# PhucNguyenAH/tacotron2_subword

Measured on AMD Instinct MI355X. Metric: mel_frames_per_sec_train, higher is better.
Workload: dtype bf16; 1 GPU; BERT_Tacotron2 default hparams (SMA), full training iteration fwd+loss+bwd+clip+Adam, B=64/GPU, 100 phones, 60 sub-word tokens, 400 frames, 80-mel; global_batch=64, frames_per_item=400, parallelism=dp1, torch_ops=loss reductions, cat/transpose copies, persistent_chains=True, recurrent_steps_bf16=True

## Files before the change

include/t2amd.h:

```cpp
#ifndef T2AMD_H
#define T2AMD_H
#include <stddef.h>
#include <stdint.h>

#ifdef __cplusplus
extern "C" {
#endif

#define T2_ATTN_SMA 0
#define T2_ATTN_LSA 1
#define T2_ATTN_DCA 4
#define T2_ATTN_GMM 3
#define T2_ATTN_FWD2 2

enum {
    T2_SITE_PRENET1 = 1, T2_SITE_PRENET2 = 2, T2_SITE_PRENET1_SUB = 3, T2_SITE_PRENET2_SUB = 4,
    T2_SITE_ATT_H = 5, T2_SITE_ATT_C = 6, T2_SITE_ATT_H_SUB = 7, T2_SITE_ATT_C_SUB = 8,
    T2_SITE_DEC_H = 9, T2_SITE_DEC_C = 10, T2_SITE_NOISE = 11, T2_SITE_NOISE_SUB = 12,
    T2_SITE_ENC0 = 16,
    T2_SITE_ENCSUB0 = 20,
    T2_SITE_POSTNET0 = 24
};

const char* t2_last_error(void);
#define T2_ABI_VERSION 4
int t2_version(void);
int t2_chain_status(uint32_t* out_host );
int t2_chain_status_clear(void);
int t2_debug_report_abort(uint32_t code, void* stream);
int t2_debug_occupy(int workgroups, int milliseconds, void* stream);
int t2_chain_claimed(void);
int t2_set_precision(int mode);
int t2_get_precision(void);
int t2_gemm_counts(uint64_t* out_host , int reset);
int t2_set_gemm_split_min_mflop(int mflop);
int t2_set_overlap(int on);
int t2_set_chain(int on);
int t2_get_chain(void);
int t2_set_chain_bwd(int on);
int t2_set_gemm_staging(int on);
int t2_side_join(void* stream);

typedef struct t2_dims {
    int n_mel;
    int prenet_dim;
    int enc_dim;
    int att_rnn_dim;
    int dec_rnn_dim;
    int att_dim;
    int loc_filters;
    int loc_kernel;
    int attention_kind;
    float p_att_dropout, p_dec_dropout, p_prenet_dropout;
    int n_streams;
    float score_mask_value, score_mask_value_sub;
    int score_mask_given;
} t2_dims;

typedef struct t2_attention_weights {
    const float* wq;
    const float* wm;
    const float* v;
    const float* loc_conv;
    const float* loc_dense;
    const float* mlp_b1;
    const float* mlp_w2;
    const float* mlp_b2;
    const float* dca_T;
    const float* dca_bT;
    const float* dca_P;
} t2_attention_weights;
typedef struct t2_lstm_weights { const float *w_ih, *w_hh, *b_ih, *b_hh; } t2_lstm_weights;
typedef struct t2_decoder_weights {
    const float *prenet_w1, *prenet_w2;
    const float *prenet_sub_w1, *prenet_sub_w2;
    t2_lstm_weights att, att_sub;
    t2_attention_weights attn, attn_sub;
    t2_lstm_weights dec;
    const float *proj_w, *proj_b;
    const float *gate_w, *gate_b;
} t2_decoder_weights;

typedef struct t2_decoder_layout {
    size_t total_floats;
    size_t x, p1, p2, p1s, p2s;
    size_t pm, pms;
    size_t prea, preas;
    size_t ga, gas;
    size_t cna, cnas, ca, cas;
    size_t din;
    size_t psel, psels;
    size_t wcum, wcums;
    size_t pred, gd, cnd, cd;
    size_t dout;
    size_t qs, qss;
    size_t qpart;
    size_t w1t;
    size_t w16a, w16as, w16d, wt16a, wt16as, wt16d, din16, dh16;
    size_t gemm_ws; size_t gemm_ws_floats;
    size_t chain; size_t chain_floats;
    size_t usave, usaves;
    size_t locsave, locsaves;
} t2_decoder_layout;

int t2_decoder_layout_query(const t2_dims* dims, int B, int T, int Tin, int Tsub, t2_decoder_layout* out);

typedef struct t2_decoder_fwd_args {
    int B, T, Tin, Tsub;
    const float* memory;
    const float* memory_sub;
    const int32_t* mem_lengths;
    const int32_t* sub_lengths;
    const float* mels;
    float* mel_out;
    float* gate_out;
    float* align;
    float* align_sub;
    float* ws;
    int training;
    int prenet_dropout;
    uint64_t seed;
    int phase;
} t2_decoder_fwd_args;
int t2_decoder_forward(const t2_dims* dims, const t2_decoder_weights* w, const t2_decoder_fwd_args* a, void* stream);

typedef struct t2_lstm_grads { float *w_ih, *w_hh, *b_ih, *b_hh; } t2_lstm_grads;
typedef struct t2_attention_grads { float *wq, *wm, *v, *loc_conv, *loc_dense, *mlp_b1, *mlp_w2, *mlp_b2, *dca_T, *dca_bT, *dca_P; } t2_attention_grads;
typedef struct t2_decoder_grads {
    float *prenet_w1, *prenet_w2, *prenet_sub_w1, *prenet_sub_w2;
    t2_lstm_grads att, att_sub;
    t2_attention_grads attn, attn_sub;
    t2_lstm_grads dec;
    float *proj_w, *proj_b, *gate_w, *gate_b;
} t2_decoder_grads;
typedef struct t2_decoder_bwd_layout {
    size_t total_floats;
    size_t ddout, ddin, dgd, dga, dgas, dctx, dctxs, dq, dqs, dv, dvs, dpm, dpms, carry, carrys;
    size_t carryc, carrycs, dlconv, dlconvs, dldense, dldenses;
    size_t dcd, dca, dcas, partd, parta, dp2, dp2s, dp1, dmel_t, dgate_t, dg16a, dg16d, colsum_ws, gemm_ws, gemm_ws_floats;
    size_t chain, chain_floats;
} t2_decoder_bwd_layout;
int t2_decoder_bwd_layout_query(const t2_dims* dims, int B, int T, int Tin, int Tsub, t2_decoder_bwd_layout* out);
typedef struct t2_decoder_bwd_args {
    int B, T, Tin, Tsub;
    const float* memory; const float* memory_sub;
    const float* align; const float* align_sub;
    const float* d_mel;
    const float* d_gate;
    const float* d_align;
    const float* d_align_sub;
    float* d_memory;
    float* d_memory_sub;
    const float* ws;
    float* bws;
    int training; int prenet_dropout; uint64_t seed;
    int defer_weight_grads;
} t2_decoder_bwd_args;
int t2_decoder_backward(const t2_dims* dims, const t2_decoder_weights* w, const t2_decoder_grads* g,
                        const t2_decoder_bwd_args* a, void* stream);

typedef struct t2_decoder_infer_args {
    int B, Tin, Tsub, max_steps, poll_every;
    float gate_threshold;
    const float* memory; const float* memory_sub;
    const int32_t* mem_lengths; const int32_t* sub_lengths;
    float* mel_out;
    float* gate_out;
    float* align;
    float* align_sub;
    int32_t* stop_index;
    int32_t* done_count;
    float* ws;
    int prenet_dropout; uint64_t seed;
    int* steps_run_host;
} t2_decoder_infer_args;
int t2_decoder_infer(const t2_dims* dims, const t2_decoder_weights* w, const t2_decoder_infer_args* a, void* stream);

int t2_finalize_bct(const float* in_btc, float* out_bct, int B, int T, int C, const int32_t* lengths, float fill, void* stream);
int t2_mask_bt(float* x, int B, int T, const int32_t* lengths, float fill, void* stream);

typedef struct t2_conv_bn_args {
    int B, T, Cin, Cout, K;
    const float* x;
    const float* w; const float* bias;
    const float* gamma; const float* beta;
    float* run_mean; float* run_var;
    int training; float eps; int act; float drop_p; uint64_t seed; uint32_t site;
    const float* residual;
    float* z; float* mean; float* invstd; float* var;
    float* y;
    float* ws; size_t ws_floats;
} t2_conv_bn_args;
int t2_conv_bn_forward(const t2_conv_bn_args* a, void* stream);
typedef struct t2_conv_bn_bwd_args {
    int B, T, Cin, Cout, K;
    const float* x; const float* w; const float* gamma; const float* beta;
    const float* z; const float* mean; const float* invstd;
    int training; float eps; int act; float drop_p; uint64_t seed; uint32_t site;
    const float* dy;
    float* dw; float* dbias; float* dgamma; float* dbeta;
    float* dx; int dx_accumulate;
    float* ws; size_t ws_floats;
} t2_conv_bn_bwd_args;
int t2_conv_bn_backward(const t2_conv_bn_bwd_args* a, void* stream);

int t2_embedding_forward(const int64_t* ids, const float* table, float* out, int rows, int dim, void* stream);
int t2_embedding_backward(const int64_t* ids, const float* dout, float* dtable, int rows, int dim, int vocab, void* stream);

typedef struct t2_lstm_seq_args {
    int nstreams, B, T, H;
    const float* pre[4];
    const float* w_hh[4];
    int reverse[4];
    const int32_t* lengths;
    float* h[4]; long ldh;
    float* c[4];
    float* gates[4];
    float* ws; size_t ws_floats;
} t2_lstm_seq_args;
size_t t2_lstm_seq_chain_ws_floats(int nstreams, int B, int H, int backward);
int t2_lstm_seq_forward(const t2_lstm_seq_args* a, void* stream);
typedef struct t2_lstm_seq_bwd_args {
    int nstreams, B, T, H;
    const float* w_hh[4]; int reverse[4];
    const float* h[4]; long ldh; const float* c[4]; const float* gates[4];
    const float* dh[4]; long lddh;
    float* dpre[4];
    float* dw_hh[4];
    float* ws; size_t ws_floats;
} t2_lstm_seq_bwd_args;
int t2_lstm_seq_backward(const t2_lstm_seq_bwd_args* a, void* stream);

typedef struct t2_gemm_args {
    const float* A; const float* B; float* C; int M, N, K;
    long sam, sak, sbn, sbk, ldc; int batch; long bsA, bsB, bsC;
    float alpha, beta; const float* bias; int act; int crow_mod; long crow_mul;
    float* ws; size_t ws_bytes; int splitk;
} t2_gemm_args;
int t2_gemm_ex(const t2_gemm_args* a, void* stream);
int t2_prof_gemm(const t2_gemm_args* a, int reps, float* ms_total, float* ms_kernel, void* stream);
enum { T2_GEMM_F32_64 = 0, T2_GEMM_F32_128, T2_GEMM_BF16CONV, T2_GEMM_SRC128, T2_GEMM_SRC256, T2_GEMM_SRC256KM };
enum { T2_GEMM_OPERAND_FP32 = 0, T2_GEMM_OPERAND_STAGED, T2_GEMM_OPERAND_CALLER };
typedef struct t2_gemm_plan_opts {
    int conv_a, conv_b, conv_T, conv_C, fp32_only;
    int a16, b16; long lda16, ldb16; int a16_kmajor, b16_kmajor, split16;
} t2_gemm_plan_opts;
typedef struct t2_gemm_plan_info {
    int kernel; const char* name;
    int split;
    int splitk, kchunks;
    int a_src, b_src;
    size_t stage_bytes_a, stage_bytes_b;
} t2_gemm_plan_info;
int t2_gemm_plan(const t2_gemm_args* a, const t2_gemm_plan_opts* opts, t2_gemm_plan_info* out);
int t2_colsum(const float* x, long ld, int M, int N, float* out, float* scratch, void* stream);
int t2_mask_btc(float* x, int B, int T, int C, const int32_t* lengths, float fill, void* stream);

typedef struct t2_adam_tensor { float* p; const float* g; float* m; float* v; long numel; int first_chunk; int pad_; } t2_adam_tensor;
int t2_adam_chunks(long numel);
int t2_adam_step(const t2_adam_tensor* table, int n_tensors, int n_chunks, float* partial, float* norm_out, float max_norm,
                 float lr, float beta1, float beta2, float eps, float weight_decay, int step, void* stream);
int t2_adam_norm(const t2_adam_tensor* table, int n_tensors, int n_chunks, float* partial, float* norm_out, float max_norm, void* stream);

int t2_prof_enable(int max_launches);
int t2_prof_collect(int n_kinds, double* total_ms_host, int* launches_host);

int t2_gemm(const float* A, const float* B, float* C, int M, int N, int K,
            long sam, long sak, long sbn, long sbk, long ldc,
            const float* bias, int act, float alpha, float beta,
            float* ws, size_t ws_bytes, int splitk, void* stream);
int t2_rng_keep_mask(uint64_t seed, uint32_t site, uint32_t n, float p, uint8_t* out, void* stream);
int t2_rng_normal(uint64_t seed, uint32_t site, uint32_t n, float* out, void* stream);

#ifdef __cplusplus
}
#endif
#endif
```

tacotron2_subword_amd/_lib.py:

```python
from __future__ import annotations

import ctypes as C
import os

import torch

_HERE = os.path.dirname(os.path.abspath(__file__))
LIB_PATH = os.environ.get("T2AMD_LIB") or os.path.join(_HERE, "libt2amd.so")

ATTN_SMA, ATTN_LSA, ATTN_FWD2, ATTN_GMM, ATTN_DCA = 0, 1, 2, 3, 4

SITE = dict(PRENET1=1, PRENET2=2, PRENET1_SUB=3, PRENET2_SUB=4, ATT_H=5, ATT_C=6, ATT_H_SUB=7, ATT_C_SUB=8,
            DEC_H=9, DEC_C=10, NOISE=11, NOISE_SUB=12, ENC0=16, ENCSUB0=20, POSTNET0=24)

_fp = C.POINTER(C.c_float)
_ip = C.POINTER(C.c_int32)


class Dims(C.Structure):
    _fields_ = [("n_mel", C.c_int), ("prenet_dim", C.c_int), ("enc_dim", C.c_int), ("att_rnn_dim", C.c_int),
                ("dec_rnn_dim", C.c_int), ("att_dim", C.c_int), ("loc_filters", C.c_int), ("loc_kernel", C.c_int),
                ("attention_kind", C.c_int), ("p_att_dropout", C.c_float), ("p_dec_dropout", C.c_float),
                ("p_prenet_dropout", C.c_float), ("n_streams", C.c_int),
                ("score_mask_value", C.c_float), ("score_mask_value_sub", C.c_float), ("score_mask_given", C.c_int)]


class AttentionWeights(C.Structure):
    _fields_ = [("wq", C.c_void_p), ("wm", C.c_void_p), ("v", C.c_void_p), ("loc_conv", C.c_void_p), ("loc_dense", C.c_void_p),
                ("mlp_b1", C.c_void_p), ("mlp_w2", C.c_void_p), ("mlp_b2", C.c_void_p),
                ("dca_T", C.c_void_p), ("dca_bT", C.c_void_p), ("dca_P", C.c_void_p)]


class LstmWeights(C.Structure):
    _fields_ = [("w_ih", C.c_void_p), ("w_hh", C.c_void_p), ("b_ih", C.c_void_p), ("b_hh", C.c_void_p)]


class DecoderWeights(C.Structure):
    _fields_ = [("prenet_w1", C.c_void_p), ("prenet_w2", C.c_void_p), ("prenet_sub_w1", C.c_void_p), ("prenet_sub_w2", C.c_void_p),
                ("att", LstmWeights), ("att_sub", LstmWeights), ("attn", AttentionWeights), ("attn_sub", AttentionWeights),
                ("dec", LstmWeights), ("proj_w", C.c_void_p), ("proj_b", C.c_void_p), ("gate_w", C.c_void_p), ("gate_b", C.c_void_p)]


_LAYOUT_FIELDS = ["total_floats", "x", "p1", "p2", "p1s", "p2s", "pm", "pms", "prea", "preas", "ga", "gas",
                  "cna", "cnas", "ca", "cas", "din", "psel", "psels", "wcum", "wcums", "pred", "gd", "cnd", "cd",
                  "dout", "qs", "qss", "qpart", "w1t", "w16a", "w16as", "w16d", "wt16a", "wt16as", "wt16d", "din16", "dh16",
                  "gemm_ws", "gemm_ws_floats", "chain", "chain_floats", "usave", "usaves", "locsave", "locsaves"]


class DecoderLayout(C.Structure):
    _fields_ = [(n, C.c_size_t) for n in _LAYOUT_FIELDS]


class DecoderFwdArgs(C.Structure):
    _fields_ = [("B", C.c_int), ("T", C.c_int), ("Tin", C.c_int), ("Tsub", C.c_int),
                ("memory", C.c_void_p), ("memory_sub", C.c_void_p), ("mem_lengths", C.c_void_p), ("sub_lengths", C.c_void_p),
                ("mels", C.c_void_p), ("mel_out", C.c_void_p), ("gate_out", C.c_void_p), ("align", C.c_void_p),
                ("align_sub", C.c_void_p), ("ws", C.c_void_p), ("training", C.c_int), ("prenet_dropout", C.c_int),
                ("seed", C.c_uint64), ("phase", C.c_int)]


class DecoderInferArgs(C.Structure):
    _fields_ = [("B", C.c_int), ("Tin", C.c_int), ("Tsub", C.c_int), ("max_steps", C.c_int), ("poll_every", C.c_int),
                ("gate_threshold", C.c_float),
                ("memory", C.c_void_p), ("memory_sub", C.c_void_p), ("mem_lengths", C.c_void_p), ("sub_lengths", C.c_void_p),
                ("mel_out", C.c_void_p), ("gate_out", C.c_void_p), ("align", C.c_void_p), ("align_sub", C.c_void_p),
                ("stop_index", C.c_void_p), ("done_count", C.c_void_p), ("ws", C.c_void_p),
                ("prenet_dropout", C.c_int), ("seed", C.c_uint64), ("steps_run_host", C.POINTER(C.c_int))]


class LstmGrads(C.Structure):
    _fields_ = LstmWeights._fields_


class AttentionGrads(C.Structure):
    _fields_ = AttentionWeights._fields_


class DecoderGrads(C.Structure):
    _fields_ = [("prenet_w1", C.c_void_p), ("prenet_w2", C.c_void_p), ("prenet_sub_w1", C.c_void_p), ("prenet_sub_w2", C.c_void_p),
                ("att", LstmGrads), ("att_sub", LstmGrads), ("attn", AttentionGrads), ("attn_sub", AttentionGrads),
                ("dec", LstmGrads), ("proj_w", C.c_void_p), ("proj_b", C.c_void_p), ("gate_w", C.c_void_p), ("gate_b", C.c_void_p)]


_BWD_LAYOUT_FIELDS = ["total_floats", "ddout", "ddin", "dgd", "dga", "dgas", "dctx", "dctxs", "dq", "dqs", "dv", "dvs",
                      "dpm", "dpms", "carry", "carrys", "carryc", "carrycs", "dlconv", "dlconvs", "dldense", "dldenses", "dcd", "dca", "dcas", "partd", "parta", "dp2", "dp2s", "dp1",
                      "dmel_t", "dgate_t", "dg16a", "dg16d", "colsum_ws", "gemm_ws", "gemm_ws_floats", "chain", "chain_floats"]


class DecoderBwdLayout(C.Structure):
    _fields_ = [(n, C.c_size_t) for n in _BWD_LAYOUT_FIELDS]


class DecoderBwdArgs(C.Structure):
    _fields_ = [("B", C.c_int), ("T", C.c_int), ("Tin", C.c_int), ("Tsub", C.c_int),
                ("memory", C.c_void_p), ("memory_sub", C.c_void_p), ("align", C.c_void_p), ("align_sub", C.c_void_p),
                ("d_mel", C.c_void_p), ("d_gate", C.c_void_p), ("d_align", C.c_void_p), ("d_align_sub", C.c_void_p),
                ("d_memory", C.c_void_p), ("d_memory_sub", C.c_void_p), ("ws", C.c_void_p), ("bws", C.c_void_p),
                ("training", C.c_int), ("prenet_dropout", C.c_int), ("seed", C.c_uint64), ("defer_weight_grads", C.c_int)]


class ConvBnArgs(C.Structure):
    _fields_ = [("B", C.c_int), ("T", C.c_int), ("Cin", C.c_int), ("Cout", C.c_int), ("K", C.c_int),
                ("x", C.c_void_p), ("w", C.c_void_p), ("bias", C.c_void_p), ("gamma", C.c_void_p), ("beta", C.c_void_p),
                ("run_mean", C.c_void_p), ("run_var", C.c_void_p),
                ("training", C.c_int), ("eps", C.c_float), ("act", C.c_int), ("drop_p", C.c_float), ("seed", C.c_uint64),
                ("site", C.c_uint32), ("residual", C.c_void_p),
                ("z", C.c_void_p), ("mean", C.c_void_p), ("invstd", C.c_void_p), ("var", C.c_void_p), ("y", C.c_void_p),
                ("ws", C.c_void_p), ("ws_floats", C.c_size_t)]


class ConvBnBwdArgs(C.Structure):
    _fields_ = [("B", C.c_int), ("T", C.c_int), ("Cin", C.c_int), ("Cout", C.c_int), ("K", C.c_int),
                ("x", C.c_void_p), ("w", C.c_void_p), ("gamma", C.c_void_p), ("beta", C.c_void_p),
                ("z", C.c_void_p), ("mean", C.c_void_p), ("invstd", C.c_void_p),
                ("training", C.c_int), ("eps", C.c_float), ("act", C.c_int), ("drop_p", C.c_float), ("seed", C.c_uint64),
                ("site", C.c_uint32), ("dy", C.c_void_p),
                ("dw", C.c_void_p), ("dbias", C.c_void_p), ("dgamma", C.c_void_p), ("dbeta", C.c_void_p),
                ("dx", C.c_void_p), ("dx_accumulate", C.c_int), ("ws", C.c_void_p), ("ws_floats", C.c_size_t)]


_P4 = C.c_void_p * 4
_I4 = C.c_int * 4


class LstmSeqArgs(C.Structure):
    _fields_ = [("nstreams", C.c_int), ("B", C.c_int), ("T", C.c_int), ("H", C.c_int),
                ("pre", _P4), ("w_hh", _P4), ("reverse", _I4), ("lengths", C.c_void_p),
                ("h", _P4), ("ldh", C.c_long), ("c", _P4), ("gates", _P4), ("ws", C.c_void_p), ("ws_floats", C.c_size_t)]


class LstmSeqBwdArgs(C.Structure):
    _fields_ = [("nstreams", C.c_int), ("B", C.c_int), ("T", C.c_int), ("H", C.c_int),
                ("w_hh", _P4), ("reverse", _I4), ("h", _P4), ("ldh", C.c_long), ("c", _P4), ("gates", _P4),
                ("dh", _P4), ("lddh", C.c_long), ("dpre", _P4), ("dw_hh", _P4), ("ws", C.c_void_p), ("ws_floats", C.c_size_t)]


class GemmArgs(C.Structure):
    _fields_ = [("A", C.c_void_p), ("B", C.c_void_p), ("C", C.c_void_p), ("M", C.c_int), ("N", C.c_int), ("K", C.c_int),
                ("sam", C.c_long), ("sak", C.c_long), ("sbn", C.c_long), ("sbk", C.c_long), ("ldc", C.c_long),
                ("batch", C.c_int), ("bsA", C.c_long), ("bsB", C.c_long), ("bsC", C.c_long),
                ("alpha", C.c_float), ("beta", C.c_float), ("bias", C.c_void_p), ("act", C.c_int),
                ("crow_mod", C.c_int), ("crow_mul", C.c_long), ("ws", C.c_void_p), ("ws_bytes", C.c_size_t), ("splitk", C.c_int)]


class GemmPlanOpts(C.Structure):
    _fields_ = [("conv_a", C.c_int), ("conv_b", C.c_int), ("conv_T", C.c_int), ("conv_C", C.c_int), ("fp32_only", C.c_int),
                ("a16", C.c_int), ("b16", C.c_int), ("lda16", C.c_long), ("ldb16", C.c_long),
                ("a16_kmajor", C.c_int), ("b16_kmajor", C.c_int), ("split16", C.c_int)]


class GemmPlanInfo(C.Structure):
    _fields_ = [("kernel", C.c_int), ("name", C.c_char_p), ("split", C.c_int), ("splitk", C.c_int), ("kchunks", C.c_int),
                ("a_src", C.c_int), ("b_src", C.c_int), ("stage_bytes_a", C.c_size_t), ("stage_bytes_b", C.c_size_t)]


ABI_VERSION = 4

EXPORTS = ["t2_last_error", "t2_version", "t2_chain_status", "t2_chain_status_clear", "t2_debug_report_abort", "t2_debug_occupy", "t2_chain_claimed", "t2_set_precision", "t2_get_precision", "t2_gemm_counts", "t2_set_gemm_split_min_mflop", "t2_set_overlap", "t2_set_chain", "t2_get_chain", "t2_set_chain_bwd", "t2_set_gemm_staging", "t2_side_join", "t2_decoder_layout_query", "t2_decoder_forward", "t2_decoder_infer",
           "t2_decoder_bwd_layout_query", "t2_decoder_backward", "t2_prof_enable", "t2_prof_collect", "t2_adam_chunks", "t2_adam_step", "t2_adam_norm",
           "t2_conv_bn_forward", "t2_conv_bn_backward", "t2_embedding_forward", "t2_embedding_backward",
           "t2_lstm_seq_forward", "t2_lstm_seq_backward", "t2_lstm_seq_chain_ws_floats", "t2_gemm_ex", "t2_prof_gemm", "t2_gemm_plan", "t2_colsum", "t2_mask_btc",
           "t2_finalize_bct", "t2_mask_bt", "t2_gemm", "t2_rng_keep_mask", "t2_rng_normal"]

_lib = None


def lib() -> C.CDLL:
    global _lib
    if _lib is None:
        if not os.path.exists(LIB_PATH):
            raise RuntimeError(f"{LIB_PATH} is missing: the HIP extension must be built (see __graft_entry__.build); "
                               "there is no CPU fallback for the product path")
        L = C.CDLL(LIB_PATH)
        L.t2_last_error.restype = C.c_char_p
        if L.t2_version() != ABI_VERSION:
            raise RuntimeError(f"{LIB_PATH} speaks ABI version {L.t2_version()}, this binding {ABI_VERSION}: rebuild the library "
                               "(the argument structs differ in size between versions)")
        L.t2_chain_status.argtypes = [C.POINTER(C.c_uint32)]
        L.t2_debug_report_abort.argtypes = [C.c_uint32, C.c_void_p]
        L.t2_debug_occupy.argtypes = [C.c_int, C.c_int, C.c_void_p]
        L.t2_gemm.argtypes = [C.c_void_p, C.c_void_p, C.c_void_p, C.c_int, C.c_int, C.c_int, C.c_long, C.c_long, C.c_long,
                              C.c_long, C.c_long, C.c_void_p, C.c_int, C.c_float, C.c_float, C.c_void_p, C.c_size_t,
                              C.c_int, C.c_void_p]
        L.t2_rng_keep_mask.argtypes = [C.c_uint64, C.c_uint32, C.c_uint32, C.c_float, C.c_void_p, C.c_void_p]
        L.t2_rng_normal.argtypes = [C.c_uint64, C.c_uint32, C.c_uint32, C.c_void_p, C.c_void_p]
        L.t2_decoder_layout_query.argtypes = [C.POINTER(Dims), C.c_int, C.c_int, C.c_int, C.c_int, C.POINTER(DecoderLayout)]
        L.t2_decoder_forward.argtypes = [C.POINTER(Dims), C.POINTER(DecoderWeights), C.POINTER(DecoderFwdArgs), C.c_void_p]
        L.t2_decoder_infer.argtypes = [C.POINTER(Dims), C.POINTER(DecoderWeights), C.POINTER(DecoderInferArgs), C.c_void_p]
        L.t2_decoder_bwd_layout_query.argtypes = [C.POINTER(Dims), C.c_int, C.c_int, C.c_int, C.c_int, C.POINTER(DecoderBwdLayout)]
        L.t2_decoder_backward.argtypes = [C.POINTER(Dims), C.POINTER(DecoderWeights), C.POINTER(DecoderGrads),
                                          C.POINTER(DecoderBwdArgs), C.c_void_p]
        L.t2_conv_bn_forward.argtypes = [C.POINTER(ConvBnArgs), C.c_void_p]
        L.t2_conv_bn_backward.argtypes = [C.POINTER(ConvBnBwdArgs), C.c_void_p]
        L.t2_embedding_forward.argtypes = [C.c_void_p, C.c_void_p, C.c_void_p, C.c_int, C.c_int, C.c_void_p]
        L.t2_embedding_backward.argtypes = [C.c_void_p, C.c_void_p, C.c_void_p, C.c_int, C.c_int, C.c_int, C.c_void_p]
        L.t2_lstm_seq_forward.argtypes = [C.POINTER(LstmSeqArgs), C.c_void_p]
        L.t2_lstm_seq_backward.argtypes = [C.POINTER(LstmSeqBwdArgs), C.c_void_p]
        L.t2_lstm_seq_chain_ws_floats.argtypes, L.t2_lstm_seq_chain_ws_floats.restype = [C.c_int, C.c_int, C.c_int, C.c_int], C.c_size_t
        L.t2_gemm_ex.argtypes = [C.POINTER(GemmArgs), C.c_void_p]
        L.t2_prof_gemm.argtypes = [C.POINTER(GemmArgs), C.c_int, C.POINTER(C.c_float), C.POINTER(C.c_float), C.c_void_p]
        L.t2_gemm_plan.argtypes = [C.POINTER(GemmArgs), C.POINTER(GemmPlanOpts), C.POINTER(GemmPlanInfo)]
        L.t2_colsum.argtypes = [C.c_void_p, C.c_long, C.c_int, C.c_int, C.c_void_p, C.c_void_p, C.c_void_p]
        L.t2_mask_btc.argtypes = [C.c_void_p, C.c_int, C.c_int, C.c_int, C.c_void_p, C.c_float, C.c_void_p]
        L.t2_prof_enable.argtypes = [C.c_int]
        L.t2_gemm_counts.argtypes = [C.POINTER(C.c_uint64), C.c_int]
        L.t2_set_gemm_split_min_mflop.argtypes = [C.c_int]
        L.t2_prof_collect.argtypes = [C.c_int, C.POINTER(C.c_double), C.POINTER(C.c_int)]
        L.t2_finalize_bct.argtypes = [C.c_void_p, C.c_void_p, C.c_int, C.c_int, C.c_int, C.c_void_p, C.c_float, C.c_void_p]
        L.t2_mask_bt.argtypes = [C.c_void_p, C.c_int, C.c_int, C.c_void_p, C.c_float, C.c_void_p]
        _lib = L
    return _lib


def check(rc: int) -> None:
    if rc != 0:
        raise RuntimeError(f"t2amd call failed ({rc}): {lib().t2_last_error().decode()}")


def ptr(t: torch.Tensor | None) -> int | None:
    if t is None:
        return None
    if not t.is_cuda:
        raise RuntimeError("t2amd: tensors must live on the GPU (no CPU fallback in the product path)")
    if not t.is_contiguous():
        raise RuntimeError("t2amd: tensor must be contiguous")
    return t.data_ptr()


def stream() -> int:
    return torch.cuda.current_stream().cuda_stream


def dims_from_hparams(hp, n_streams: int = 2) -> Dims:
    g = (lambda k: hp[k]) if isinstance(hp, dict) else (lambda k: getattr(hp, k))
    kind = {"StepwiseMonotonicAttention": ATTN_SMA, "ForwardAttentionV2": ATTN_FWD2, "GMMAttention": ATTN_GMM,
            "DynamicConvolutionAttention": ATTN_DCA}.get(g("attention"), ATTN_LSA)
    return Dims(int(g("n_mel_channels")) * int(g("n_frames_per_step")), int(g("prenet_dim")), int(g("encoder_embedding_dim")),
                int(g("attention_rnn_dim")), int(g("decoder_rnn_dim")), int(g("attention_dim")),
                int(g("attention_location_n_filters")), int(g("attention_location_kernel_size")), kind,
                float(g("p_attention_dropout")), float(g("p_decoder_dropout")), 0.5, n_streams)


def decoder_weights(P: dict, kind: int, prefix: str = "decoder.", single: bool = False) -> DecoderWeights:
    p = lambda k: ptr(P[prefix + k])
    lstm = lambda n: LstmWeights(p(n + ".weight_ih"), p(n + ".weight_hh"), p(n + ".bias_ih"), p(n + ".bias_hh"))

    def attn(n):
        if kind == ATTN_SMA:
            return AttentionWeights(p(n + ".query_layer.linear_layer.weight"), p(n + ".memory_layer.linear_layer.weight"),
                                    p(n + ".v.weight"), None, None)
        if kind == ATTN_DCA:
            return AttentionWeights(p(n + ".W.weight"), None, p(n + ".v.weight"), p(n + ".F.weight"), p(n + ".U.weight"),
                                    p(n + ".W.bias"), p(n + ".V.weight"), None, p(n + ".T.weight"), p(n + ".T.bias"), p(n + ".P"))
        if kind == ATTN_GMM:
            return AttentionWeights(p(n + ".mlp.0.weight"), None, None, None, None,
                                    p(n + ".mlp.0.bias"), p(n + ".mlp.2.weight"), p(n + ".mlp.2.bias"))
        return AttentionWeights(p(n + ".query_layer.linear_layer.weight"), p(n + ".memory_layer.linear_layer.weight"),
                                p(n + ".v.linear_layer.weight"), p(n + ".location_layer.location_conv.conv.weight"),
                                p(n + ".location_layer.location_dense.linear_layer.weight"))
    none_l, none_a = LstmWeights(None, None, None, None), AttentionWeights()
    return DecoderWeights(p("prenet.layers.0.linear_layer.weight"), p("prenet.layers.1.linear_layer.weight"),
                          None if single else p("prenet_bert.layers.0.linear_layer.weight"),
                          None if single else p("prenet_bert.layers.1.linear_layer.weight"),
                          lstm("attention_rnn"), none_l if single else lstm("attention_rnn_bert"),
                          attn("attention_layer"), none_a if single else attn("attention_layer_bert"),
                          lstm("decoder_rnn"), p("linear_projection.linear_layer.weight"), p("linear_projection.linear_layer.bias"),
                          p("gate_layer.linear_layer.weight"), p("gate_layer.linear_layer.bias"))


DECODER_PARAM_KEYS_SMA = [
    "prenet.layers.0.linear_layer.weight", "prenet.layers.1.linear_layer.weight",
    "prenet_bert.layers.0.linear_layer.weight", "prenet_bert.layers.1.linear_layer.weight",
    "attention_rnn.weight_ih", "attention_rnn.weight_hh", "attention_rnn.bias_ih", "attention_rnn.bias_hh",
    "attention_rnn_bert.weight_ih", "attention_rnn_bert.weight_hh", "attention_rnn_bert.bias_ih", "attention_rnn_bert.bias_hh",
    "attention_layer.query_layer.linear_layer.weight", "attention_layer.memory_layer.linear_layer.weight", "attention_layer.v.weight",
    "attention_layer_bert.query_layer.linear_layer.weight", "attention_layer_bert.memory_layer.linear_layer.weight",
    "attention_layer_bert.v.weight",
    "decoder_rnn.weight_ih", "decoder_rnn.weight_hh", "decoder_rnn.bias_ih", "decoder_rnn.bias_hh",
    "linear_projection.linear_layer.weight", "linear_projection.linear_layer.bias",
    "gate_layer.linear_layer.weight", "gate_layer.linear_layer.bias"]


def _lsa_keys():
    out = []
    for k in DECODER_PARAM_KEYS_SMA:
        if k.endswith(".v.weight"):
            n = k[:-len(".v.weight")]
            out += [n + ".v.linear_layer.weight", n + ".location_layer.location_conv.conv.weight",
                    n + ".location_layer.location_dense.linear_layer.weight"]
        else:
            out.append(k)
    return out


DECODER_PARAM_KEYS_LSA = _lsa_keys()


def _gmm_keys():
    out = []
    for k in DECODER_PARAM_KEYS_SMA:
        if ".query_layer." in k:
            n = k[:k.index(".query_layer.")]
            out += [n + ".mlp.0.weight", n + ".mlp.0.bias", n + ".mlp.2.weight", n + ".mlp.2.bias"]
        elif ".memory_layer." in k or k.endswith(".v.weight"):
            continue
        else:
            out.append(k)
    return out


DECODER_PARAM_KEYS_GMM = _gmm_keys()


def _dca_keys():
    out = []
    for k in DECODER_PARAM_KEYS_SMA:
        if ".query_layer." in k:
            n = k[:k.index(".query_layer.")]
            out += [n + s for s in (".W.weight", ".W.bias", ".V.weight", ".F.weight", ".U.weight", ".T.weight", ".T.bias", ".v.weight")]
        elif ".memory_layer." in k or k.endswith(".v.weight"):
            continue
        else:
            out.append(k)
    return out


DECODER_PARAM_KEYS_DCA = _dca_keys()


def decoder_param_keys(kind: int, single: bool = False):
    keys = {ATTN_SMA: DECODER_PARAM_KEYS_SMA, ATTN_GMM: DECODER_PARAM_KEYS_GMM, ATTN_DCA: DECODER_PARAM_KEYS_DCA}.get(kind, DECODER_PARAM_KEYS_LSA)
    return [k for k in keys if "_bert" not in k] if single else keys


def decoder_grads(G: dict, prefix: str = "decoder.", single: bool = False, kind: int = ATTN_SMA) -> DecoderGrads:
    p = lambda k: ptr(G[prefix + k])
    lstm = lambda n: LstmGrads(p(n + ".weight_ih"), p(n + ".weight_hh"), p(n + ".bias_ih"), p(n + ".bias_hh"))

    def attn(n):
        if kind == ATTN_SMA:
            return AttentionGrads(p(n + ".query_layer.linear_layer.weight"), p(n + ".memory_layer.linear_layer.weight"),
                                  p(n + ".v.weight"), None, None)
        if kind == ATTN_DCA:
            return AttentionGrads(p(n + ".W.weight"), None, p(n + ".v.weight"), p(n + ".F.weight"), p(n + ".U.weight"),
                                  p(n + ".W.bias"), p(n + ".V.weight"), None, p(n + ".T.weight"), p(n + ".T.bias"), None)
        if kind == ATTN_GMM:
            return AttentionGrads(p(n + ".mlp.0.weight"), None, None, None, None,
                                  p(n + ".mlp.0.bias"), p(n + ".mlp.2.weight"), p(n + ".mlp.2.bias"))
        return AttentionGrads(p(n + ".query_layer.linear_layer.weight"), p(n + ".memory_layer.linear_layer.weight"),
                              p(n + ".v.linear_layer.weight"), p(n + ".location_layer.location_conv.conv.weight"),
                              p(n + ".location_layer.location_dense.linear_layer.weight"))
    none_l, none_a = LstmGrads(None, None, None, None), AttentionGrads()
    return DecoderGrads(p("prenet.layers.0.linear_layer.weight"), p("prenet.layers.1.linear_layer.weight"),
                        None if single else p("prenet_bert.layers.0.linear_layer.weight"),
                        None if single else p("prenet_bert.layers.1.linear_layer.weight"),
                        lstm("attention_rnn"), none_l if single else lstm("attention_rnn_bert"),
                        attn("attention_layer"), none_a if single else attn("attention_layer_bert"),
                        lstm("decoder_rnn"), p("linear_projection.linear_layer.weight"), p("linear_projection.linear_layer.bias"),
                        p("gate_layer.linear_layer.weight"), p("gate_layer.linear_layer.bias"))


def decoder_bwd_layout(dims: Dims, B: int, T: int, Tin: int, Tsub: int) -> DecoderBwdLayout:
    L = DecoderBwdLayout()
    check(lib().t2_decoder_bwd_layout_query(C.byref(dims), B, T, Tin, Tsub, C.byref(L)))
    return L


def decoder_layout(dims: Dims, B: int, T: int, Tin: int, Tsub: int) -> DecoderLayout:
    L = DecoderLayout()
    check(lib().t2_decoder_layout_query(C.byref(dims), B, T, Tin, Tsub, C.byref(L)))
    return L


PROF_KINDS = ["att_lstm_fwd", "attention_fwd", "dec_lstm_fwd", "attention_bwd", "att_lstm_bwd_pointwise",
              "att_lstm_bwd_gemm", "dec_lstm_bwd_pointwise", "dec_lstm_bwd_gemm", "chain_a_fwd", "chain_b_fwd", "chain_b_bwd", "chain_a_bwd", "chain_dec"]


def prof_enable(max_launches: int) -> None:
    check(lib().t2_prof_enable(max_launches))


def prof_collect() -> dict:
    n = len(PROF_KINDS)
    ms, cnt = (C.c_double * n)(), (C.c_int * n)()
    check(lib().t2_prof_collect(n, ms, cnt))
    return {k: (ms[i], cnt[i]) for i, k in enumerate(PROF_KINDS)}


def set_chain(on: bool) -> None:
    check(lib().t2_set_chain(int(bool(on))))


def set_chain_bwd(on: bool) -> None:
    check(lib().t2_set_chain_bwd(int(bool(on))))


def get_chain() -> bool:
    return bool(lib().t2_get_chain())


PRECISION_MODES = {"f32": 0, "fp32": 0, "bf16": 1, "bf16x3": 2}


def set_precision(mode: str) -> None:
    check(lib().t2_set_precision(PRECISION_MODES[mode]))


def get_precision() -> str:
    return {0: "f32", 1: "bf16", 2: "bf16x3"}[lib().t2_get_precision()]


def gemm_counts(reset: bool = False):
    out = (C.c_uint64 * 4)()
    check(lib().t2_gemm_counts(out, int(bool(reset))))
    return tuple(int(v) for v in out)


def gemm_plan(args: GemmArgs, **opts) -> dict:
    o, info = GemmPlanOpts(**opts), GemmPlanInfo()
    check(lib().t2_gemm_plan(C.byref(args), C.byref(o), C.byref(info)))
    return dict(kernel=info.kernel, name=info.name.decode(), split=bool(info.split), splitk=info.splitk, kchunks=info.kchunks,
                a_src=info.a_src, b_src=info.b_src, stage_bytes_a=info.stage_bytes_a, stage_bytes_b=info.stage_bytes_b)


def set_gemm_split_min_mflop(mflop: int = -1) -> None:
    check(lib().t2_set_gemm_split_min_mflop(int(mflop)))
```

tacotron2_subword_amd/blocks.py:

```python
from __future__ import annotations

import ctypes as C

import torch

from . import _lib as L

ACT_NONE, ACT_RELU, ACT_TANH = 0, 1, 2
_WS = {}


def _scratch(dev, n_floats: int) -> torch.Tensor:
    key = (dev, torch.cuda.current_stream(dev).cuda_stream if dev.type == "cuda" else 0)
    t = _WS.get(key)
    if t is None or t.numel() < n_floats:
        t = torch.empty(int(n_floats * 1.25) + 1024, dtype=torch.float32, device=dev)
        _WS[key] = t
    return t


def _stage_terms() -> int:
    return 3 if L.get_precision() == "bf16x3" else 1


def gemm_ex(A, Bm, out, M, N, K, sam, sak, sbn, sbk, ldc, *, bias=None, act=0, alpha=1.0, beta=0.0, crow_mod=0, crow_mul=0,
            batch=1, bsA=0, bsB=0, bsC=0, splitk_ws=True):
    ws = _scratch(out.device, (8 << 20) * _stage_terms()) if splitk_ws and beta == 0.0 else None
    a = L.GemmArgs(L.ptr(A), L.ptr(Bm), L.ptr(out), M, N, K, sam, sak, sbn, sbk, ldc, batch, bsA, bsB, bsC, alpha, beta,
                   L.ptr(bias), act, crow_mod, crow_mul, L.ptr(ws), 0 if ws is None else ws.numel() * 4, 0)
    L.check(L.lib().t2_gemm_ex(C.byref(a), L.stream()))
    return out


def colsum(x2d: torch.Tensor) -> torch.Tensor:
    M, N = x2d.shape
    out = torch.empty(N, dtype=torch.float32, device=x2d.device)
    sc = torch.empty(64 * N, dtype=torch.float32, device=x2d.device)
    L.check(L.lib().t2_colsum(L.ptr(x2d), x2d.stride(0), M, N, L.ptr(out), L.ptr(sc), L.stream()))
    return out


class _LinearFn(torch.autograd.Function):

    @staticmethod
    def forward(ctx, x, W, b):
        shape = x.shape
        x2 = x.reshape(-1, shape[-1]).contiguous()
        M, K = x2.shape
        N = W.shape[0]
        y = torch.empty(M, N, dtype=torch.float32, device=x.device)
        gemm_ex(x2, W, y, M, N, K, K, 1, W.stride(0), 1, N, bias=b)
        ctx.save_for_backward(x2, W)
        ctx.has_bias, ctx.shape = b is not None, shape
        return y.view(*shape[:-1], N)

    @staticmethod
    def backward(ctx, dy):
        x2, W = ctx.saved_tensors
        M, K = x2.shape
        N = W.shape[0]
        dy2 = dy.reshape(M, N).contiguous()
        dx = dW = db = None
        if ctx.needs_input_grad[0]:
            dx = torch.empty(M, K, dtype=torch.float32, device=dy.device)
            gemm_ex(dy2, W, dx, M, K, N, N, 1, 1, W.stride(0), K)
            dx = dx.view(ctx.shape)
        if ctx.needs_input_grad[1]:
            dW = torch.empty(N, K, dtype=torch.float32, device=dy.device)
            gemm_ex(dy2, x2, dW, N, K, M, 1, N, 1, K, K)
        if ctx.has_bias and ctx.needs_input_grad[2]:
            db = colsum(dy2)
        return dx, dW, db


def linear(x, W, b=None):
    return _LinearFn.apply(x, W, b)


class _EmbeddingFn(torch.autograd.Function):
    @staticmethod
    def forward(ctx, ids, table):
        ids = ids.contiguous().long()
        rows, D = ids.numel(), table.shape[1]
        out = torch.empty(*ids.shape, D, dtype=torch.float32, device=table.device)
        L.check(L.lib().t2_embedding_forward(L.ptr(ids), L.ptr(table), L.ptr(out), rows, D, L.stream()))
        ctx.save_for_backward(ids)
        ctx.vocab = table.shape[0]
        return out

    @staticmethod
    def backward(ctx, dout):
        (ids,) = ctx.saved_tensors
        dout = dout.contiguous()
        D = dout.shape[-1]
        dtable = torch.empty(ctx.vocab, D, dtype=torch.float32, device=dout.device)
        L.check(L.lib().t2_embedding_backward(L.ptr(ids), L.ptr(dout), L.ptr(dtable), ids.numel(), D, ctx.vocab, L.stream()))
        return None, dtable


def embedding(ids, table):
    return _EmbeddingFn.apply(ids, table)


class _ConvStackFn(torch.autograd.Function):

    @staticmethod
    def forward(ctx, x, cfg, *params):
        x = x.contiguous()
        B, T, _ = x.shape
        n = len(cfg["acts"])
        dev = x.device
        saved, cur = [], x
        for i in range(n):
            w, bias, gamma, beta = params[4 * i:4 * i + 4]
            rm, rv = cfg["buffers"][i]
            Cout, Cin, K = w.shape
            M = B * T
            z = torch.empty(M, Cout, dtype=torch.float32, device=dev)
            y = torch.empty(B, T, Cout, dtype=torch.float32, device=dev)
            st = torch.empty(3, Cout, dtype=torch.float32, device=dev)
            nws = Cout * Cin * K + 4 + 128 * Cout + _stage_terms() * ((M * Cin + Cout * Cin * K) // 2) + 4096
            ws = _scratch(dev, nws)
            res = x if (cfg["residual"] and i == n - 1) else None
            a = L.ConvBnArgs(B, T, Cin, Cout, K, L.ptr(cur), L.ptr(w.detach()), L.ptr(bias.detach()), L.ptr(gamma.detach()),
                             L.ptr(beta.detach()), L.ptr(rm), L.ptr(rv), int(cfg["training"]), 1e-5, cfg["acts"][i],
                             cfg["drop_p"] if cfg["training"] else 0.0, cfg["seed"], cfg["site0"] + i, L.ptr(res),
                             L.ptr(z), L.ptr(st[0]), L.ptr(st[1]), L.ptr(st[2]), L.ptr(y), L.ptr(ws), ws.numel())
            L.check(L.lib().t2_conv_bn_forward(C.byref(a), L.stream()))
            saved.append((cur, z, st))
            cur = y
        ctx.cfg, ctx.saved_acts, ctx.params = cfg, saved, [p.detach() for p in params]
        return cur

    @staticmethod
    def backward(ctx, dy):
        cfg, params = ctx.cfg, ctx.params
        n = len(cfg["acts"])
        dev = dy.device
        dy = dy.contiguous()
        d_res = dy if cfg["residual"] else None
        grads = [None] * (4 * n)
        for i in range(n - 1, -1, -1):
            w, bias, gamma, beta = params[4 * i:4 * i + 4]
            xin, z, st = ctx.saved_acts[i]
            B, T, Cin = xin.shape
            Cout, _, K = w.shape
            M = B * T
            dw, db = torch.empty_like(w), torch.empty_like(bias)
            dg, dbt = torch.empty_like(gamma), torch.empty_like(beta)
            need_dx = i > 0 or ctx.needs_input_grad[0]
            dx = torch.empty(B, T, Cin, dtype=torch.float32, device=dev) if need_dx else None
            nws = M * Cout + Cout * Cin * K + 128 * Cout + 16 + (8 << 20) + _stage_terms() * ((M * (Cout + K * max(Cin, Cout))) // 2) + Cout * Cin * K
            ws = _scratch(dev, nws)
            a = L.ConvBnBwdArgs(B, T, Cin, Cout, K, L.ptr(xin), L.ptr(w), L.ptr(gamma), L.ptr(beta), L.ptr(z), L.ptr(st[0]), L.ptr(st[1]),
                                int(cfg["training"]), 1e-5, cfg["acts"][i], cfg["drop_p"] if cfg["training"] else 0.0, cfg["seed"],
                                cfg["site0"] + i, L.ptr(dy), L.ptr(dw), L.ptr(db), L.ptr(dg), L.ptr(dbt), L.ptr(dx), 0,
                                L.ptr(ws), ws.numel())
            L.check(L.lib().t2_conv_bn_backward(C.byref(a), L.stream()))
            grads[4 * i:4 * i + 4] = [dw, db, dg, dbt]
            dy = dx
        if dy is not None and d_res is not None:
            dy = dy + d_res
        ctx.saved_acts = None
        return (dy, None) + tuple(grads)


def conv_bn_stack(x, layers, acts, *, training, drop_p, seed, site0, residual=False):
    params, buffers = [], []
    for conv, bn in layers:
        params += [conv.weight, conv.bias, bn.weight, bn.bias]
        buffers.append((bn.running_mean, bn.running_var))
        if training:
            bn.num_batches_tracked += 1
    cfg = dict(acts=list(acts), buffers=buffers, training=bool(training), drop_p=float(drop_p), seed=int(seed), site0=int(site0),
               residual=bool(residual))
    return _ConvStackFn.apply(x, cfg, *params)


class _BiLstmFn(torch.autograd.Function):

    @staticmethod
    def forward(ctx, x, lengths, w_ih, w_hh, b_ih, b_hh, w_ih_r, w_hh_r, b_ih_r, b_hh_r):
        B, T, E = x.shape
        H = w_hh.shape[1]
        dev = x.device
        xt = x.transpose(0, 1).contiguous()
        pre = torch.empty(2, T * B, 4 * H, dtype=torch.float32, device=dev)
        bsum = torch.stack((b_ih.detach() + b_hh.detach(), b_ih_r.detach() + b_hh_r.detach()))
        for d, W in enumerate((w_ih, w_ih_r)):
            gemm_ex(xt, W.detach(), pre[d], T * B, 4 * H, E, E, 1, W.stride(0), 1, 4 * H, bias=bsum[d])
        out = torch.empty(T, B, 2 * H, dtype=torch.float32, device=dev)
        cells = torch.empty(2, T, B, H, dtype=torch.float32, device=dev)
        gates = torch.empty(2, T, B, 4 * H, dtype=torch.float32, device=dev)
        a = L.LstmSeqArgs()
        a.nstreams, a.B, a.T, a.H = 2, B, T, H
        a.pre[0], a.pre[1] = pre[0].data_ptr(), pre[1].data_ptr()
        a.w_hh[0], a.w_hh[1] = L.ptr(w_hh.detach()), L.ptr(w_hh_r.detach())
        a.reverse[0], a.reverse[1] = 0, 1
        a.lengths = L.ptr(lengths)
        a.h[0], a.h[1] = out.data_ptr(), out.data_ptr() + 4 * H
        a.ldh = 2 * H
        a.c[0], a.c[1] = cells[0].data_ptr(), cells[1].data_ptr()
        a.gates[0], a.gates[1] = gates[0].data_ptr(), gates[1].data_ptr()
        xws = torch.empty(int(L.lib().t2_lstm_seq_chain_ws_floats(2, B, H, 0)), dtype=torch.float32, device=dev)
        a.ws, a.ws_floats = L.ptr(xws), xws.numel()
        L.check(L.lib().t2_lstm_seq_forward(C.byref(a), L.stream()))
        ctx.save_for_backward(xt, out, cells, gates, w_ih, w_hh, w_ih_r, w_hh_r)
        ctx.dims = (B, T, E, H)
        return out.transpose(0, 1).contiguous()

    @staticmethod
    def backward(ctx, dout):
        xt, out, cells, gates, w_ih, w_hh, w_ih_r, w_hh_r = ctx.saved_tensors
        B, T, E, H = ctx.dims
        dev = dout.device
        dh = dout.transpose(0, 1).contiguous()
        dpre = torch.empty(2, T * B, 4 * H, dtype=torch.float32, device=dev)
        dwhh = torch.empty(2, 4 * H, H, dtype=torch.float32, device=dev)
        nws = max(2 * (B * H + 8 * B * H) + 64, int(L.lib().t2_lstm_seq_chain_ws_floats(2, B, H, 1))) + (8 << 20) * _stage_terms()
        ws = _scratch(dev, nws)
        a = L.LstmSeqBwdArgs()
        a.nstreams, a.B, a.T, a.H = 2, B, T, H
        a.w_hh[0], a.w_hh[1] = L.ptr(w_hh), L.ptr(w_hh_r)
        a.reverse[0], a.reverse[1] = 0, 1
        a.h[0], a.h[1] = out.data_ptr(), out.data_ptr() + 4 * H
        a.ldh = 2 * H
        a.c[0], a.c[1] = cells[0].data_ptr(), cells[1].data_ptr()
        a.gates[0], a.gates[1] = gates[0].data_ptr(), gates[1].data_ptr()
        a.dh[0], a.dh[1] = dh.data_ptr(), dh.data_ptr() + 4 * H
        a.lddh = 2 * H
        a.dpre[0], a.dpre[1] = dpre[0].data_ptr(), dpre[1].data_ptr()
        a.dw_hh[0], a.dw_hh[1] = dwhh[0].data_ptr(), dwhh[1].data_ptr()
        a.ws, a.ws_floats = L.ptr(ws), ws.numel()
        L.check(L.lib().t2_lstm_seq_backward(C.byref(a), L.stream()))
        TB = T * B
        dxt = torch.empty(TB, E, dtype=torch.float32, device=dev)
        res = []
        for d, W in enumerate((w_ih, w_ih_r)):
            gemm_ex(dpre[d], W, dxt, TB, E, 4 * H, 4 * H, 1, 1, W.stride(0), E, beta=float(d))
            dW = torch.empty(4 * H, E, dtype=torch.float32, device=dev)
            gemm_ex(dpre[d], xt, dW, 4 * H, E, TB, 1, 4 * H, 1, E, E)
            db = colsum(dpre[d])
            res.append((dW, dwhh[d], db, db))
        dx = dxt.view(T, B, E).transpose(0, 1).contiguous()
        return (dx, None) + res[0] + res[1]


def bilstm(x, lengths, lstm):
    ln = None if lengths is None else lengths.to(dtype=torch.int32).contiguous()
    return _BiLstmFn.apply(x, ln, lstm.weight_ih_l0, lstm.weight_hh_l0, lstm.bias_ih_l0, lstm.bias_hh_l0,
                           lstm.weight_ih_l0_reverse, lstm.weight_hh_l0_reverse, lstm.bias_ih_l0_reverse, lstm.bias_hh_l0_reverse)
```

tacotron2_subword_amd/csrc/c_api.hip:

```cpp
#include <fcntl.h>
#include <stdarg.h>
#include <stdio.h>
#include <sys/file.h>
#include <unistd.h>
#include <stdlib.h>
#include <string.h>

#include "../../include/t2amd.h"
#include "kernels.h"

static thread_local char g_err[512] = "";

void t2_set_error(const char* fmt, ...) {
    va_list ap;
    va_start(ap, fmt);
    vsnprintf(g_err, sizeof(g_err), fmt, ap);
    va_end(ap);
}

#define T2_TRY(expr)                \
    do {                            \
        int rc_ = (expr);           \
        if (rc_ != 0) return rc_;   \
    } while (0)
// ... 1064 lines not shown
    if (overlap) {
        T2_TRY(side_get(&side)); c.sd = side->s;
        T2_TRY(stream_edge(*side, ne++, c.s, side->s));
    }
    const std::vector<int> bounds = chunk_bounds(z.T, overlap);
    const float* DGd = c.S(BL.dgd);
    unsigned char* const ws8 = reinterpret_cast<unsigned char*>(c.gemm_ws());
    const size_t wt_bytes = ((size_t)4 * z.Hd * z.WD * sizeof(__bf16) + 255) & ~(size_t)255;
    const bool pre16 = get_precision() == 1 && (4 * z.Hd) % 64 == 0 && z.WD % 64 == 0 && c.gemm_ws_bytes() > 2 * wt_bytes;
    if (pre16) T2_TRY(stage_bf16(w->dec.w_ih, false, z.WD, reinterpret_cast<__bf16*>(ws8), z.WD, 4 * z.Hd, overlap ? side->s : c.s));
    const size_t dgt_bytes = ((size_t)4 * z.Hd * BT * sizeof(__bf16) + 255) & ~(size_t)255;
    const size_t dg16_off = pre16 ? wt_bytes : 0;
    const bool share = get_precision() == 1 && BT % 64 == 0 && z.B % 8 == 0 && (4 * z.Hd) % 128 == 0 && z.T > 1 &&
                       c.gemm_ws_bytes() >= dg16_off + dgt_bytes + ((size_t)z.WD * BT * sizeof(__bf16) + 256);
    __bf16* const dg16 = reinterpret_cast<__bf16*>(ws8 + dg16_off);
    bool chunk_cast = share && pre16;
    for (size_t ci = 1; ci < bounds.size(); ++ci) if (((bounds[ci] - bounds[ci - 1]) * z.B) % 64 != 0) chunk_cast = false;
    ChainBwdDesc cbb{};
    const bool chain_b = chain_a && chain_b_bwd_desc(c, &cbb);
    for (size_t ci = bounds.size() - 1; ci > 0; --ci) {
        const int t0 = bounds[ci - 1], t1 = bounds[ci];
        hipStream_t sb = overlap ? side->s : c.s;
        if (chain_b) {
            cbb.t0 = t0; cbb.t1 = t1;
            ProfScope ps(PK_CHAIN_B_BWD, sb);
            T2_TRY(chain_bwd(cbb, c.S(BL.chain), BL.chain_floats, sb));
        } else {
            for (int t = t1 - 1; t >= t0; --t) T2_TRY(dec_bwd_step(c, t));
        }
        GemmDesc dd = matmul_nn(DGd + c.R(t0) * 4 * z.Hd, 4 * z.Hd, w->dec.w_ih, z.WD, c.S(BL.ddin) + c.R(t0) * z.WD, z.WD,
                                (t1 - t0) * z.B, z.WD, 4 * z.Hd);
        dd.ws = c.gemm_ws(); dd.ws_bytes = c.gemm_ws_bytes();
        if (pre16) {
            dd.B16 = reinterpret_cast<const __bf16*>(ws8); dd.ldb16 = 4 * z.Hd;
            dd.ws = reinterpret_cast<float*>(ws8 + wt_bytes); dd.ws_bytes -= wt_bytes;
        }
        if (chunk_cast) {
            T2_TRY(stage_bf16(DGd + c.R(t0) * 4 * z.Hd, true, 4 * z.Hd, dg16 + c.R(t0) * 4 * z.Hd, (t1 - t0) * z.B, 4 * z.Hd, sb));
            dd.A16 = dg16 + c.R(t0) * 4 * z.Hd; dd.lda16 = 4 * z.Hd;
            dd.ws = reinterpret_cast<float*>(ws8 + dg16_off + dgt_bytes); dd.ws_bytes = c.gemm_ws_bytes() - dg16_off - dgt_bytes;
        }
        T2_TRY(gemm(dd, sb));
        if (overlap) T2_TRY(stream_edge(*side, ne++, sb, c.s));
        if (t0 == 0) {
            const float* DG = DGd;
            if (share && !chunk_cast) T2_TRY(stage_bf16(DG, true, 4 * z.Hd, dg16, BT, 4 * z.Hd, sb));
            auto with_dg16 = [&](GemmDesc m, long row0) {
                if (share) {
                    m.A16 = dg16 + row0 * 4 * z.Hd; m.lda16 = 4 * z.Hd; m.a16_kmajor = 1;
                    m.ws = reinterpret_cast<float*>(ws8 + dg16_off + dgt_bytes); m.ws_bytes = c.gemm_ws_bytes() - dg16_off - dgt_bytes;
                }
                return m;
            };
            GemmDesc mih = with_dg16(matmul_tn(c, DG, 4 * z.Hd, c.W(L.din), z.WD, g->dec.w_ih, z.WD, 4 * z.Hd, z.WD, BT), 0);
            if (share && c.use16) { mih.B16 = c.W16(L.din16); mih.ldb16 = z.WD; mih.b16_kmajor = 1; }
            T2_TRY(gemm(mih, sb));
            if (z.T > 1) T2_TRY(gemm(with_dg16(matmul_tn(c, DG + (long)z.B * 4 * z.Hd, 4 * z.Hd, c.W(L.dout), z.WO, g->dec.w_hh, z.Hd, 4 * z.Hd, z.Hd, BT - z.B), z.B), sb));
            else T2_TRY(fill_f32(g->dec.w_hh, 0.f, (size_t)4 * z.Hd * z.Hd, sb));
            if (chain_b) {
                T2_TRY(batch_sum(cbb.st[0].dbias_part, (z.B + 31) / 32, 4 * z.Hd, g->dec.b_ih, sb));
                T2_CHECK_HIP(hipMemcpyAsync(g->dec.b_hh, g->dec.b_ih, (size_t)4 * z.Hd * sizeof(float), hipMemcpyDeviceToDevice, sb));
            } else T2_TRY(colsum(DG, 4 * z.Hd, BT, 4 * z.Hd, g->dec.b_ih, g->dec.b_hh, cws, sb));
        }
        if (chain_a) {
            cab.t0 = t0; cab.t1 = t1;
            ProfScope ps(PK_CHAIN_A_BWD, c.s);
            T2_TRY(chain_bwd(cab, c.S(BL.chain), BL.chain_floats, c.s));
        } else {
            for (int t = t1 - 1; t >= t0; --t) T2_TRY(att_bwd_step(c, t));
        }
    }
    const bool defer = overlap && a->defer_weight_grads != 0;
    hipStream_t ts = c.s;
    if (defer) {
        T2_TRY(stream_edge(*side, ne++, c.s, side->s));
        ts = side->s;
    } else if (overlap) {
        T2_TRY(stream_edge(*side, ne++, side->s, c.s));
    }
    for (int s = 0; s < z.NS; ++s) {
        const t2_lstm_weights& lw = s ? w->att_sub : w->att;
        const t2_lstm_grads& lg = s ? g->att_sub : g->att;
        const t2_attention_weights& aw = s ? w->attn_sub : w->attn;
        const t2_attention_grads& ag = s ? g->attn_sub : g->attn;
        const int hoff = s ? z.Ha + z.E : 0, coff = hoff + z.Ha;
        const int Tin = s ? z.Tsub : z.Tin;
        const float* DG = c.S(s ? BL.dgas : BL.dga);
        const float* DIN = c.W(L.din);
        const float* P1 = c.W(s ? L.p1s : L.p1); const float* P2 = c.W(s ? L.p2s : L.p2);
        float* dP2 = c.S(s ? BL.dp2s : BL.dp2); float* dP1 = c.S(BL.dp1);
        const long ldw = z.P + z.E;
        const size_t dgt_bytes = ((size_t)4 * z.Ha * BT * sizeof(__bf16) + 255) & ~(size_t)255;
        const bool share = get_precision() == 1 && BT % 64 == 0 && z.B % 8 == 0 && (4 * z.Ha) % 128 == 0 && z.T > 1 &&
                           c.gemm_ws_bytes() >= 2 * dgt_bytes;
        __bf16* dg16 = reinterpret_cast<__bf16*>(c.gemm_ws());
        float* const ws_rest = reinterpret_cast<float*>(reinterpret_cast<unsigned char*>(c.gemm_ws()) + dgt_bytes);
        if (share) T2_TRY(stage_bf16(DG, true, 4 * z.Ha, dg16, BT, 4 * z.Ha, ts));
        const __bf16* DIN16 = share && c.use16 ? c.W16(L.din16) : nullptr;
        auto dw_gemm = [&](const float* G, long row0, const float* X, const __bf16* X16, long ldx, float* Y, long ldy, int N, int K) -> int {
            GemmDesc m = matmul_tn(c, G, 4 * z.Ha, X, ldx, Y, ldy, 4 * z.Ha, N, K);
            if (share) {
                m.A16 = dg16 + row0 * 4 * z.Ha; m.lda16 = 4 * z.Ha; m.a16_kmajor = 1;
                if (X16) { m.B16 = X16; m.ldb16 = ldx; m.b16_kmajor = 1; }
                m.ws = ws_rest; m.ws_bytes = c.gemm_ws_bytes() - dgt_bytes;
            }
            return gemm(m, ts);
        };
        T2_TRY(dw_gemm(DG, 0, P2, nullptr, z.P, lg.w_ih, ldw, z.P, BT));
        if (z.T > 1) {
            const float* DG1 = DG + (long)z.B * 4 * z.Ha;
            T2_TRY(dw_gemm(DG1, z.B, DIN + coff, DIN16 ? DIN16 + coff : nullptr, z.WD, lg.w_ih + z.P, ldw, z.E, BT - z.B));
            T2_TRY(dw_gemm(DG1, z.B, DIN + hoff, DIN16 ? DIN16 + hoff : nullptr, z.WD, lg.w_hh, z.Ha, z.Ha, BT - z.B));
        } else {
            GemmDesc zc = matmul_tn(c, DG, 4 * z.Ha, DIN + coff, z.WD, lg.w_ih + z.P, ldw, 4 * z.Ha, z.E, BT);
            zc.alpha = 0.f;
            T2_TRY(gemm(zc, ts));
            T2_TRY(fill_f32(lg.w_hh, 0.f, (size_t)4 * z.Ha * z.Ha, ts));
        }
        if (chain_a) {
            T2_TRY(batch_sum(cab.st[s].dbias_part, (z.B + 31) / 32, 4 * z.Ha, lg.b_ih, ts));
            T2_CHECK_HIP(hipMemcpyAsync(lg.b_hh, lg.b_ih, (size_t)4 * z.Ha * sizeof(float), hipMemcpyDeviceToDevice, ts));
        } else T2_TRY(colsum(DG, 4 * z.Ha, BT, 4 * z.Ha, lg.b_ih, lg.b_hh, cws, ts));
        const float scale = a->prenet_dropout ? 1.0f / (1.0f - dims->p_prenet_dropout) : 1.0f;
        GemmDesc gp = matmul_nn(DG, 4 * z.Ha, lw.w_ih, ldw, dP2, z.P, BT, z.P, 4 * z.Ha);
        gp.ws = c.gemm_ws(); gp.ws_bytes = c.gemm_ws_bytes();
        if (share) { gp.A16 = dg16; gp.lda16 = 4 * z.Ha; gp.ws = ws_rest; gp.ws_bytes -= dgt_bytes; }
        T2_TRY(gemm(gp, ts));
        T2_TRY(relu_drop_bwd(dP2, P2, dP2, scale, (size_t)BT * z.P, ts));
        T2_TRY(gemm(matmul_tn(c, dP2, z.P, P1, z.P, s ? g->prenet_sub_w2 : g->prenet_w2, z.P, z.P, z.P, BT), ts));
        T2_TRY(gemm(matmul_nn(dP2, z.P, s ? w->prenet_sub_w2 : w->prenet_w2, z.P, dP1, z.P, BT, z.P, z.P), ts));
        T2_TRY(relu_drop_bwd(dP1, P1, dP1, scale, (size_t)BT * z.P, ts));
        T2_TRY(gemm(matmul_tn(c, dP1, z.P, c.W(L.x), z.M, s ? g->prenet_sub_w1 : g->prenet_w1, z.M, z.P, z.M, BT), ts));
        const bool lsa_chain = chain_a && cab.kind == CHAIN_LSA;
        const int nsp = lsa_chain ? 2 : attn_bwd_nsplit(*dims, z);
        float* DQ = c.S(s ? BL.dqs : BL.dq);
        if (nsp == 2) T2_TRY(fold_halves(DQ, BT, z.A, ts));
        T2_TRY(gemm(matmul_tn(c, DQ, 2 * z.A, DIN + hoff, z.WD, ag.wq, z.Ha, z.A, z.Ha, BT), ts));
        const bool dcak = dims->attention_kind == T2_ATTN_DCA;
        const bool gmm = dims->attention_kind == T2_ATTN_GMM || dcak;
        if (dcak) {
            T2_REQUIRE(ag.mlp_b1 && ag.mlp_w2 && ag.loc_conv && ag.loc_dense && ag.dca_T && ag.dca_bT && ag.v, "t2_decoder_backward: DCA gradient buffers missing");
            T2_TRY(colsum(DQ, 2 * z.A, BT, z.A, ag.mlp_b1, nullptr, cws, ts));
            const size_t na = dca_acc_floats(z.A);
            float* full = c.gemm_ws();
            T2_REQUIRE(na * sizeof(float) <= c.gemm_ws_bytes(), "t2_decoder_backward: scratch too small");
            T2_TRY(batch_sum(c.S(s ? BL.dldenses : BL.dldense), z.B, (int)na, full, ts));
            auto cp = [&](float* dst, size_t off, size_t n) { return hipMemcpyAsync(dst, full + off, n * sizeof(float), hipMemcpyDeviceToDevice, ts); };
            size_t off = 0;
            T2_CHECK_HIP(cp(ag.v, off, z.A)); off += z.A;
            T2_CHECK_HIP(cp(ag.dca_bT, off, z.A)); off += z.A;
            T2_CHECK_HIP(cp(ag.loc_dense, off, (size_t)z.A * kDcaC)); off += (size_t)z.A * kDcaC;
            T2_CHECK_HIP(cp(ag.dca_T, off, (size_t)z.A * kDcaC)); off += (size_t)z.A * kDcaC;
            T2_CHECK_HIP(cp(ag.loc_conv, off, kDcaC * kDcaK)); off += kDcaC * kDcaK;
            T2_CHECK_HIP(cp(ag.mlp_w2, off, (size_t)kDcaC * kDcaK * z.A));
        } else if (gmm) {
            T2_REQUIRE(ag.mlp_b1 && ag.mlp_w2 && ag.mlp_b2, "t2_decoder_backward: GMM needs mlp_b1 / mlp_w2 / mlp_b2 gradient buffers");
            T2_TRY(colsum(DQ, 2 * z.A, BT, z.A, ag.mlp_b1, nullptr, cws, ts));
            T2_TRY(batch_sum(c.S(s ? BL.dldenses : BL.dldense), z.B, 3 * kGmmK * z.A, ag.mlp_w2, ts));
            float* b2tmp = cws;
            T2_TRY(batch_sum(c.S(s ? BL.dlconvs : BL.dlconv), z.B, 16, b2tmp, ts));
            T2_CHECK_HIP(hipMemcpyAsync(ag.mlp_b2, b2tmp, 3 * kGmmK * sizeof(float), hipMemcpyDeviceToDevice, ts));
        } else {
            T2_TRY(batch_sum(c.S(s ? BL.dvs : BL.dv), nsp * z.B, z.A, ag.v, ts));
        }
        if (dims->attention_kind == T2_ATTN_LSA) {
            T2_REQUIRE(ag.loc_conv && ag.loc_dense, "t2_decoder_backward: LSA needs loc_conv / loc_dense gradient buffers");
            T2_TRY(batch_sum(c.S(s ? BL.dlconvs : BL.dlconv), (lsa_chain ? 2 : 1) * z.B, dims->loc_filters * 2 * dims->loc_kernel, ag.loc_conv, ts));
            T2_TRY(batch_sum(c.S(s ? BL.dldenses : BL.dldense), (lsa_chain ? 2 : 1) * z.B, z.A * dims->loc_filters, ag.loc_dense, ts));
        }
        const float* mem = s ? a->memory_sub : a->memory;
        float* dmem = s ? a->d_memory_sub : a->d_memory;
        if (!gmm) {
            const float* DPM = c.S(s ? BL.dpms : BL.dpm);
            T2_TRY(gemm(matmul_tn(c, DPM, z.A, mem, z.E, ag.wm, z.E, z.A, z.E, z.B * Tin), ts));
            T2_TRY(gemm(matmul_nn(DPM, z.A, aw.wm, z.E, dmem, z.E, z.B * Tin, z.E, z.A), c.s));
        }
        GemmDesc dm = gemm_desc();
        dm.A = s ? a->align_sub : a->align; dm.sam = 1; dm.sak = Tin; dm.bsA = (long)z.T * Tin;
        dm.B = c.S(s ? BL.dctxs : BL.dctx); dm.sbk = (long)z.B * z.E; dm.sbn = 1; dm.bsB = z.E;
        dm.C = dmem; dm.ldc = z.E; dm.bsC = (long)Tin * z.E;
        dm.M = Tin; dm.N = z.E; dm.K = z.T; dm.batch = z.B; dm.beta = gmm ? 0.f : 1.f;
        T2_TRY(gemm(dm, c.s));
    }
    return 0;
}

int t2_decoder_infer(const t2_dims* dims_in, const t2_decoder_weights* w, const t2_decoder_infer_args* a, void* stream) {
    T2_REQUIRE(dims_in && w && a && a->steps_run_host, "null argument");
    T2_TRY(check_dims(*dims_in));
    int max_pos = 0;
    const t2_dims dd = canon_dims(*dims_in, &max_pos);
    const t2_dims* dims = &dd;
    (void)max_pos;
    T2_REQUIRE(a->B >= 1 && a->B <= 256 && a->max_steps >= 1, "bad shape B=%d max_steps=%d", a->B, a->max_steps);
    Dec c{*dims, *w, sizes_of(*dims, a->B, a->max_steps, a->Tin, a->Tsub), {}, a->ws,
          a->memory, a->memory_sub, a->mem_lengths, a->sub_lengths,
          a->mel_out, a->gate_out, a->align, a->align_sub,
          false, a->prenet_dropout != 0, false, a->seed, (hipStream_t)stream};
    c.max_pos = max_pos;
    layout_of(*dims, c.z, &c.L);
    const Sizes& z = c.z; const t2_decoder_layout& L = c.L;
    const int T = z.T;
    int poll = a->poll_every > 0 ? a->poll_every : 16;

    hipLaunchKernelGGL(init_stop_kernel, dim3((z.B + 63) / 64), dim3(64), 0, c.s, a->stop_index, a->done_count, z.B);
    T2_LAUNCH_CHECK();
    T2_TRY(processed_memory(c));
    for (int s = 0; s < z.NS; ++s)
        T2_TRY(permute_rows(s ? w->prenet_sub_w1 : w->prenet_w1, c.P(L.w1t) + (size_t)s * z.M * z.P, z.P, z.M, 1, c.s));
    c.I = infer_shadows(z, L.w16a);
    c.use16 = get_precision() == 1 && z.B <= 128 && c.I.Ka % 256 == 0 && c.I.Kd % 256 == 0;
    if (c.use16) {
        const long ldi = z.P + z.E;
        for (int s = 0; s < z.NS; ++s) {
            const t2_lstm_weights& lw = s ? w->att_sub : w->att;
            __bf16* f = c.P16(c.I.wa[s]);
            T2_TRY(cast_rows_bf16(lw.w_hh, z.Ha, f, c.I.Ka, 4 * z.Ha, z.Ha, c.s));
            T2_TRY(cast_rows_bf16(lw.w_ih + z.P, ldi, f + z.Ha, c.I.Ka, 4 * z.Ha, z.E, c.s));
            T2_TRY(cast_rows_bf16(lw.w_ih, ldi, f + z.Ha + z.E, c.I.Ka, 4 * z.Ha, z.P, c.s));
        }
        T2_TRY(cast_rows_bf16(w->dec.w_ih, z.WD, c.P16(c.I.wd), c.I.Kd, 4 * z.Hd, z.WD, c.s));
        T2_TRY(cast_rows_bf16(w->dec.w_hh, z.Hd, c.P16(c.I.wd) + z.WD, c.I.Kd, 4 * z.Hd, z.Hd, c.s));
        T2_CHECK_HIP(hipMemsetAsync(c.RowA(0, 0), 0, (size_t)2 * 2 * z.B * c.I.Ka * sizeof(__bf16), c.s));
        T2_CHECK_HIP(hipMemsetAsync(c.RowD(0), 0, (size_t)2 * z.B * c.I.Kd * sizeof(__bf16), c.s));
    }
    auto tail = [&](int t, bool proj) -> int {
        StepTailDesc d{};
        d.B = z.B; d.M = z.M; d.P = z.P; d.WO = z.WO; d.NS = z.NS; d.t = t;
        d.do_proj = proj; d.do_prenet = proj ? (t + 1 < T) : 1;
        const int tn = proj ? t + 1 : 0;
        if (proj) {
            d.dout = c.P(L.dout) + c.R(t) * z.WO; d.lddout = z.WO;
            d.proj_w = w->proj_w; d.proj_b = w->proj_b; d.gate_w = w->gate_w; d.gate_b = w->gate_b;
            d.mel_out = a->mel_out + (long)t * z.M; d.ldmel = (long)T * z.M;
            d.gate_out = a->gate_out + t; d.ldgate = T;
            d.thr = a->gate_threshold; d.stop_index = a->stop_index; d.done = a->done_count;
        }
        for (int s = 0; s < z.NS; ++s) {
            d.w1t[s] = c.P(L.w1t) + (size_t)s * z.M * z.P; d.w2[s] = s ? w->prenet_sub_w2 : w->prenet_w2;
            d.p1[s] = c.P(s ? L.p1s : L.p1) + c.R(tn) * z.P; d.p2[s] = c.P(s ? L.p2s : L.p2) + c.R(tn) * z.P;
            d.site1[s] = s ? T2_SITE_PRENET1_SUB : T2_SITE_PRENET1; d.site2[s] = s ? T2_SITE_PRENET2_SUB : T2_SITE_PRENET2;
        }
        d.ldp = z.P;
        if (c.use16) { for (int s = 0; s < z.NS; ++s) d.p2_16[s] = c.RowA(tn & 1, s) + z.Ha + z.E; d.ldp16 = c.I.Ka; }
        d.drop_p = c.prenet_dropout ? dims->p_prenet_dropout : 0.f; d.seed = c.seed;
        d.drop_base = (uint32_t)(c.R(tn) * z.P); d.drop_mstride = (uint32_t)z.P;
        return step_tail(d, c.s);
    };
    int steps = 0;
    StopPoll* pl = nullptr;
    T2_TRY(stop_poll_get(&pl));
    ChainDesc cdec{};
    const bool chain = g_chain && chain_dec_desc(c, *w, *a, &cdec);
    if (chain && a->poll_every <= 0) poll = 32;
    T2_TRY(chain_fwd_ws_clear(c.P(L.chain), L.chain_floats, chain ? CHAIN_WS_DECODE : CHAIN_WS_STATUS, c.s));
    if (!chain) T2_TRY(tail(0, false));
    for (int t = 0; t < T; ++t) {
        if (chain) {
            if (t % poll == 0) {
                cdec.t0 = t; cdec.t1 = std::min(T, t + poll);
                ProfScope ps(PK_CHAIN_DEC, c.s);
                T2_TRY(chain_fwd(cdec, c.P(L.chain), L.chain_floats, c.s));
            }
        } else {
            T2_TRY(att_lstm_step(c, t));
            T2_TRY(attention_step(c, t));
            T2_TRY(dec_lstm_step(c, t));
            T2_TRY(tail(t, true));
        }
        steps = t + 1;
        if (steps % poll == 0 && steps < T) {
            const int k = steps / poll, slot = k & 3;
            T2_CHECK_HIP(hipMemcpyAsync(pl->host + slot, a->done_count, sizeof(int32_t), hipMemcpyDeviceToHost, c.s));
            T2_CHECK_HIP(hipEventRecord(pl->ev[slot], c.s));
            if (k >= 3) {
                const int prev = (k - 2) & 3;
                T2_CHECK_HIP(hipEventSynchronize(pl->ev[prev]));
                if (pl->host[prev] >= z.B) break;
            }
        }
    }
    *a->steps_run_host = steps;
    if (chain) {
        hipLaunchKernelGGL(poison_if_aborted_kernel, dim3(64), dim3(256), 0, c.s, status_words(a->ws, L), CHAIN_STATUS_FWD_ATT + 1,
                           a->mel_out, (size_t)z.B * T * z.M, a->gate_out, (size_t)z.B * T);
        T2_LAUNCH_CHECK();
    }
    return 0;
}


int t2_conv_bn_forward(const t2_conv_bn_args* a, void* stream) {
    T2_REQUIRE(a, "null argument");
    const size_t nw = (size_t)a->Cout * a->Cin * a->K;
    T2_REQUIRE(a->ws_floats >= nw + 128 * (size_t)a->Cout, "t2_conv_bn_forward: workspace too small");
    ConvBnFwd f{};
    f.x = a->x; f.B = a->B; f.T = a->T; f.Cin = a->Cin; f.Cout = a->Cout; f.K = a->K;
    f.w = a->w; f.bias = a->bias; f.gamma = a->gamma; f.beta = a->beta; f.run_mean = a->run_mean; f.run_var = a->run_var;
    f.training = a->training; f.eps = a->eps; f.act = a->act; f.drop_p = a->drop_p; f.seed = a->seed; f.site = a->site;
    f.residual = a->residual; f.z = a->z; f.mean = a->mean; f.invstd = a->invstd; f.var = a->var; f.y = a->y;
    f.wperm = a->ws; f.scratch = a->ws + align4(nw);
    const size_t used = align4(nw) + 128 * (size_t)a->Cout;
    if (a->ws_floats > used) { f.gemm_ws = a->ws + used; f.gemm_ws_bytes = (a->ws_floats - used) * sizeof(float); }
    return conv_bn_fwd(f, (hipStream_t)stream);
}

int t2_conv_bn_backward(const t2_conv_bn_bwd_args* a, void* stream) {
    T2_REQUIRE(a, "null argument");
    const size_t nw = align4((size_t)a->Cout * a->Cin * a->K), ndz = align4((size_t)a->B * a->T * a->Cout), nsc = 128 * (size_t)a->Cout;
    T2_REQUIRE(a->ws_floats >= nw + ndz + nsc, "t2_conv_bn_backward: workspace too small");
    ConvBnBwd f{};
    f.x = a->x; f.B = a->B; f.T = a->T; f.Cin = a->Cin; f.Cout = a->Cout; f.K = a->K;
    f.w = a->w; f.gamma = a->gamma; f.beta = a->beta; f.z = a->z; f.mean = a->mean; f.invstd = a->invstd;
    f.training = a->training; f.eps = a->eps; f.act = a->act; f.drop_p = a->drop_p; f.seed = a->seed; f.site = a->site;
    f.dy = a->dy; f.dw = a->dw; f.dbias = a->dbias; f.dgamma = a->dgamma; f.dbeta = a->dbeta;
    f.dx = a->dx; f.dx_accumulate = a->dx_accumulate;
    f.dz = a->ws; f.wperm = a->ws + ndz; f.scratch = a->ws + ndz + nw;
    f.gemm_ws = a->ws + ndz + nw + nsc; f.gemm_ws_bytes = (a->ws_floats - (ndz + nw + nsc)) * sizeof(float);
    return conv_bn_bwd(f, (hipStream_t)stream);
}

int t2_embedding_forward(const int64_t* ids, const float* table, float* out, int rows, int dim, void* stream) {
    return embedding_fwd(reinterpret_cast<const long*>(ids), table, out, rows, dim, (hipStream_t)stream);
}
int t2_embedding_backward(const int64_t* ids, const float* dout, float* dtable, int rows, int dim, int vocab, void* stream) {
    return embedding_bwd(reinterpret_cast<const long*>(ids), dout, dtable, rows, dim, vocab, (hipStream_t)stream);
}

int t2_lstm_seq_forward(const t2_lstm_seq_args* a, void* stream) {
    T2_REQUIRE(a && a->nstreams >= 1 && a->nstreams <= kMaxLstmStreams, "t2_lstm_seq_forward: bad nstreams");
    T2_REQUIRE(a->H % 64 == 0, "t2_lstm_seq_forward: H=%d must be a multiple of 64", a->H);
    const int B = a->B, T = a->T, H = a->H;
    if (g_chain && a->ws && a->ws_floats >= enc_chain_ws_floats(a->nstreams, B, H, 0) && enc_chain_covers(a->nstreams, B, H)) {
        EncChainDesc d{};
        d.ND = a->nstreams; d.B = B; d.T = T; d.H = H; d.lengths = a->lengths; d.ldh = a->ldh;
        for (int s = 0; s < a->nstreams; ++s) {
            d.pre[s] = a->pre[s]; d.w_hh[s] = a->w_hh[s]; d.reverse[s] = a->reverse[s];
            d.h[s] = a->h[s]; d.c[s] = a->c[s]; d.gates[s] = a->gates[s];
        }
        return enc_chain_fwd(d, a->ws, a->ws_floats, (hipStream_t)stream);
    }
    for (int step = 0; step < T; ++step) {
        LstmStepDesc d{};
        d.nstreams = a->nstreams; d.B = B; d.H = H; d.drop_p = 0.f;
        for (int s = 0; s < a->nstreams; ++s) {
            LstmStream& st = d.st[s];
            const int t = a->reverse[s] ? T - 1 - step : step;
            const int tp = a->reverse[s] ? t + 1 : t - 1;
            st.pre = a->pre[s] + (long)t * B * 4 * H; st.ldpre = 4 * H;
            if (step > 0) {
                st.seg[0] = LstmSeg{a->h[s] + (long)tp * B * a->ldh, a->ldh, a->w_hh[s], (long)H, H};
                st.nseg = 1;
                st.c_prev = a->c[s] + (long)tp * B * H; st.ldc_prev = H;
            }
            st.gates = a->gates[s] + (long)t * B * 4 * H; st.ldgates = 4 * H;
            st.c_out = a->c[s] + (long)t * B * H; st.ldc_out = H;
            st.h_out = a->h[s] + (long)t * B * a->ldh; st.ldh_out = a->ldh;
            st.lengths = a->lengths; st.t = t;
        }
        T2_TRY(lstm_step_fwd(d, (hipStream_t)stream));
    }
    return 0;
}

size_t t2_lstm_seq_chain_ws_floats(int nstreams, int B, int H, int backward) { return enc_chain_ws_floats(nstreams, B, H, backward); }

int t2_lstm_seq_backward(const t2_lstm_seq_bwd_args* a, void* stream) {
    T2_REQUIRE(a && a->nstreams >= 1 && a->nstreams <= kMaxLstmStreams, "t2_lstm_seq_backward: bad nstreams");
    const int B = a->B, T = a->T, H = a->H, ns = a->nstreams;
    const int ks = lstm_bwd_ksplit(4 * H);
    hipStream_t s = (hipStream_t)stream;
    float* dc = a->ws;
    float* part = dc + align4((size_t)ns * B * H);
    float* gws = part + align4((size_t)ns * ks * B * H);
    T2_REQUIRE(a->ws_floats >= (size_t)(gws - a->ws), "t2_lstm_seq_backward: workspace too small");
    const size_t gws_bytes = (a->ws_floats - (size_t)(gws - a->ws)) * sizeof(float);
    const bool chain = g_chain && g_chain_bwd && a->ws_floats >= enc_chain_ws_floats(ns, B, H, 1) && enc_chain_covers(ns, B, H);
    if (chain) {
        EncChainBwdDesc d{};
        d.ND = ns; d.B = B; d.T = T; d.H = H; d.lddh = a->lddh;
        for (int i = 0; i < ns; ++i) {
            d.w_hh[i] = a->w_hh[i]; d.reverse[i] = a->reverse[i]; d.c[i] = a->c[i]; d.gates[i] = a->gates[i];
            d.dh[i] = a->dh[i]; d.dpre[i] = a->dpre[i];
        }
        T2_TRY(enc_chain_bwd(d, a->ws, a->ws_floats, s));
    }
    for (int step = 0; step < (chain ? 0 : T); ++step) {
        LstmBwdPointDesc p{};
        p.nstreams = ns; p.B = B; p.H = H; p.drop_p = 0.f; p.first = step == 0;
        LstmBwdGemmDesc g{};
        g.nstreams = ns; g.B = B; g.H4 = 4 * H; g.KS = ks; g.NC = H;
        for (int i = 0; i < ns; ++i) {
            const int t = a->reverse[i] ? step : T - 1 - step;
            const int tprev = a->reverse[i] ? t + 1 : t - 1;
            const bool has_prev = a->reverse[i] ? (t + 1 < T) : (t > 0);
            LstmBwdStream& st = p.st[i];
            st.dh1 = a->dh[i] + (long)t * B * a->lddh; st.lddh1 = a->lddh;
            st.part = part + (size_t)i * ks * B * H; st.nparts = ks; st.part_stride = (long)B * H; st.ldpart = H; st.part_col = 0;
            st.gates = a->gates[i] + (long)t * B * 4 * H; st.ldgates = 4 * H;
            st.c_new = a->c[i] + (long)t * B * H; st.ldc_new = H;
            if (has_prev) { st.c_prev = a->c[i] + (long)tprev * B * H; st.ldc_prev = H; }
            st.dc_state = dc + (size_t)i * B * H;
            st.dg = a->dpre[i] + (long)t * B * 4 * H; st.lddg = 4 * H;
            g.st[i].dg = st.dg; g.st[i].lddg = 4 * H;
            g.st[i].seg[0] = LstmBwdSeg{a->w_hh[i], (long)H, H}; g.st[i].nseg = 1;
            g.st[i].part = part + (size_t)i * ks * B * H;
        }
        T2_TRY(lstm_bwd_pointwise(p, s));
        if (step + 1 < T) T2_TRY(lstm_bwd_gemm(g, s));
    }
    for (int i = 0; i < ns; ++i) {
        if (T < 2) { T2_TRY(fill_f32(a->dw_hh[i], 0.f, (size_t)4 * H * H, s)); continue; }
        GemmDesc w = gemm_desc();
        const long rowsB = (long)B;
        w.A = a->reverse[i] ? a->dpre[i] : a->dpre[i] + rowsB * 4 * H; w.sam = 1; w.sak = 4 * H;
        w.B = a->reverse[i] ? a->h[i] + rowsB * a->ldh : a->h[i]; w.sbk = a->ldh; w.sbn = 1;
        w.C = a->dw_hh[i]; w.ldc = H; w.M = 4 * H; w.N = H; w.K = (T - 1) * B;
        w.ws = gws; w.ws_bytes = gws_bytes;
        T2_TRY(gemm(w, s));
    }
    return 0;
}

static GemmDesc desc_of(const t2_gemm_args& a) {
    GemmDesc g = gemm_desc();
    g.A = a.A; g.B = a.B; g.C = a.C; g.M = a.M; g.N = a.N; g.K = a.K;
    g.sam = a.sam; g.sak = a.sak; g.sbn = a.sbn; g.sbk = a.sbk; g.ldc = a.ldc;
    g.batch = a.batch > 0 ? a.batch : 1; g.bsA = a.bsA; g.bsB = a.bsB; g.bsC = a.bsC;
    g.alpha = a.alpha; g.beta = a.beta; g.bias1 = a.bias; g.act = a.act;
    g.crow_mod = a.crow_mod; g.crow_mul = a.crow_mul;
    g.ws = a.ws; g.ws_bytes = a.ws_bytes; g.splitk = a.splitk;
    return g;
}
int t2_gemm_ex(const t2_gemm_args* a, void* stream) {
    T2_REQUIRE(a, "null argument");
    return gemm(desc_of(*a), (hipStream_t)stream);
}
int t2_gemm_plan(const t2_gemm_args* a, const t2_gemm_plan_opts* o, t2_gemm_plan_info* out) {
    T2_REQUIRE(a && out, "null argument");
    GemmDesc g = desc_of(*a);
    if (o) {
        g.conv_a = o->conv_a; g.conv_b = o->conv_b; g.conv_T = o->conv_T; g.conv_C = o->conv_C; g.fp32_only = o->fp32_only;
        const __bf16* copy = reinterpret_cast<const __bf16*>(uintptr_t(256));
        if (o->a16) { g.A16 = copy; g.lda16 = o->lda16; g.a16_kmajor = o->a16_kmajor; }
        if (o->b16) { g.B16 = copy; g.ldb16 = o->ldb16; g.b16_kmajor = o->b16_kmajor; }
        g.split16 = o->split16;
    }
    GemmPlan p;
    T2_TRY(gemm_plan(g, &p));
    *out = t2_gemm_plan_info{(int)p.kernel, gemm_plan_name(p), p.split, p.splitk, p.kchunks, (int)p.a.src, (int)p.b.src, p.a.bytes, p.b.bytes};
    return 0;
}
static int time_gemm(const GemmDesc& g, int reps, float* ms, hipStream_t s) {
    hipEvent_t e0, e1;
    T2_CHECK_HIP(hipEventCreate(&e0)); T2_CHECK_HIP(hipEventCreate(&e1));
    int rc = gemm(g, s);
    T2_CHECK_HIP(hipEventRecord(e0, s));
    for (int i = 0; i < reps && rc == 0; ++i) rc = gemm(g, s);
    T2_CHECK_HIP(hipEventRecord(e1, s));
    T2_CHECK_HIP(hipEventSynchronize(e1));
    T2_CHECK_HIP(hipEventElapsedTime(ms, e0, e1));
    *ms /= reps;
    hipEventDestroy(e0); hipEventDestroy(e1);
    return rc;
}
int t2_prof_gemm(const t2_gemm_args* a, int reps, float* ms_total, float* ms_kernel, void* stream) {
    T2_REQUIRE(a && reps > 0 && ms_total && ms_kernel, "t2_prof_gemm: bad arguments");
    T2_REQUIRE(get_precision() != 0 && a->M % 128 == 0 && a->N % 128 == 0 && a->K % 64 == 0 && (a->batch <= 1) && a->ws,
               "t2_prof_gemm: bf16 or split-bf16 mode, whole-tile shapes and scratch only");
    hipStream_t s = (hipStream_t)stream;
    GemmDesc g = desc_of(*a);
    GemmPlan p, q;
    T2_TRY(gemm_plan(g, &p));
    T2_REQUIRE(p.a.src == GemmSrc::staged && p.b.src == GemmSrc::staged, "t2_prof_gemm: refused, gemm() runs this product on kernel %s, which stages no bf16 copies", gemm_plan_name(p));
    T2_TRY(time_gemm(g, reps, ms_total, s));
    unsigned char* w8 = reinterpret_cast<unsigned char*>(a->ws);
    __bf16* a16 = reinterpret_cast<__bf16*>(w8); __bf16* b16 = reinterpret_cast<__bf16*>(w8 + p.a.bytes);
    T2_TRY(stage_planned(g.A, p.a, p.split, a16, s));
    T2_TRY(stage_planned(g.B, p.b, p.split, b16, s));
    g.A16 = a16; g.lda16 = p.a.ld; g.B16 = b16; g.ldb16 = p.b.ld;
    g.a16_kmajor = g.b16_kmajor = p.kernel == GemmKernel::src256km; g.split16 = p.split;
    g.ws = reinterpret_cast<float*>(w8 + p.a.bytes + p.b.bytes); g.ws_bytes = a->ws_bytes - p.a.bytes - p.b.bytes;
    T2_TRY(gemm_plan(g, &q));
    T2_REQUIRE(q.kernel == p.kernel && q.split == p.split && q.a.src == GemmSrc::caller && q.b.src == GemmSrc::caller,
               "t2_prof_gemm: refused, with both copies handed over gemm() would run kernel %s and not read both", gemm_plan_name(q));
    return time_gemm(g, reps, ms_kernel, s);
}
int t2_colsum(const float* x, long ld, int M, int N, float* out, float* scratch, void* stream) {
    return colsum(x, ld, M, N, out, nullptr, scratch, (hipStream_t)stream);
}
int t2_mask_btc(float* x, int B, int T, int C, const int32_t* lengths, float fill, void* stream) {
    T2_REQUIRE(lengths, "t2_mask_btc: lengths is null");
    return mask_btc(x, B, T, C, lengths, fill, (hipStream_t)stream);
}

int t2_prof_enable(int max_launches) {
    if (max_launches <= 0) { g_prof.on = false; return 0; }
    const size_t need = (size_t)max_launches * 2;
    while (g_prof.ev.size() < need) {
        hipEvent_t e;
        T2_CHECK_HIP(hipEventCreate(&e));
        g_prof.ev.push_back(e);
    }
    g_prof.kind.assign(g_prof.ev.size() / 2, 0);
    g_prof.used = 0;
    g_prof.on = true;
    return 0;
}

int t2_prof_collect(int n_kinds, double* total_ms_host, int* launches_host) {
    T2_REQUIRE(n_kinds >= PK_COUNT, "t2_prof_collect: need %d kinds", (int)PK_COUNT);
    g_prof.on = false;
    for (int i = 0; i < n_kinds; ++i) { total_ms_host[i] = 0.0; launches_host[i] = 0; }
    if (g_prof.used == 0) return 0;
    T2_CHECK_HIP(hipDeviceSynchronize());
    for (size_t i = 0; i + 1 < g_prof.used; i += 2) {
        float ms = 0.f;
        T2_CHECK_HIP(hipEventElapsedTime(&ms, g_prof.ev[i], g_prof.ev[i + 1]));
        total_ms_host[g_prof.kind[i / 2]] += ms;
        launches_host[g_prof.kind[i / 2]] += 1;
    }
    g_prof.used = 0;
    return 0;
}

int t2_adam_chunks(long numel) { return adam_chunks(numel); }
int t2_adam_step(const t2_adam_tensor* table, int n_tensors, int n_chunks, float* partial, float* norm_out, float max_norm,
                 float lr, float beta1, float beta2, float eps, float weight_decay, int step, void* stream) {
    static_assert(sizeof(t2_adam_tensor) == sizeof(AdamTensor), "table row layout");
    return adam_step(reinterpret_cast<const AdamTensor*>(table), n_tensors, n_chunks, partial, norm_out, max_norm, lr, beta1, beta2, eps,
                     weight_decay, step, (hipStream_t)stream);
}

int t2_adam_norm(const t2_adam_tensor* table, int n_tensors, int n_chunks, float* partial, float* norm_out, float max_norm, void* stream) {
    return adam_norm(reinterpret_cast<const AdamTensor*>(table), n_tensors, n_chunks, partial, norm_out, max_norm, (hipStream_t)stream);
}

int t2_finalize_bct(const float* in_btc, float* out_bct, int B, int T, int C, const int32_t* lengths, float fill, void* stream) {
    return transpose_btc_to_bct(in_btc, out_bct, B, T, C, lengths, fill, (hipStream_t)stream);
}
int t2_mask_bt(float* x, int B, int T, const int32_t* lengths, float fill, void* stream) {
    T2_REQUIRE(lengths, "t2_mask_bt: lengths is null");
    return mask_bt(x, B, T, lengths, fill, (hipStream_t)stream);
}

int t2_gemm(const float* A, const float* B, float* C, int M, int N, int K, long sam, long sak, long sbn, long sbk, long ldc,
            const float* bias, int act, float alpha, float beta, float* ws, size_t ws_bytes, int splitk, void* stream) {
    GemmDesc g = gemm_desc();
    g.A = A; g.B = B; g.C = C; g.M = M; g.N = N; g.K = K;
    g.sam = sam; g.sak = sak; g.sbn = sbn; g.sbk = sbk; g.ldc = ldc;
    g.bias1 = bias; g.act = act; g.alpha = alpha; g.beta = beta;
    g.ws = ws; g.ws_bytes = ws_bytes; g.splitk = splitk;
    return gemm(g, (hipStream_t)stream);
}
int t2_rng_keep_mask(uint64_t seed, uint32_t site, uint32_t n, float p, uint8_t* out, void* stream) {
    return rng_keep_mask(seed, site, n, p, out, (hipStream_t)stream);
}
int t2_rng_normal(uint64_t seed, uint32_t site, uint32_t n, float* out, void* stream) {
    return rng_normal(seed, site, n, out, (hipStream_t)stream);
}

}
```

tacotron2_subword_amd/csrc/common.h:

```cpp
#pragma once
#include <hip/hip_runtime.h>
#include <stdint.h>
#include <math.h>

namespace t2 {

typedef float f32x4 __attribute__((ext_vector_type(4)));
typedef float f32x16 __attribute__((ext_vector_type(16)));

constexpr int kWave = 64;

__host__ __device__ __forceinline__ uint32_t mix32(uint32_t x) {
    x ^= x >> 16; x *= 0x7feb352du; x ^= x >> 15; x *= 0x846ca68bu; x ^= x >> 16;
    return x;
}
struct RngKey { uint32_t k0, k1; };
__host__ __device__ __forceinline__ RngKey rng_key(uint64_t seed, uint32_t site) {
    RngKey k;
    k.k0 = mix32((uint32_t)seed ^ mix32(site * 0x9E3779B9u + 0x85ebca6bu));
    k.k1 = mix32((uint32_t)(seed >> 32) + site * 0xc2b2ae35u + 0x27d4eb2fu);
    return k;
}
__host__ __device__ __forceinline__ uint32_t rng_u32(RngKey k, uint32_t idx) {
    return mix32((idx ^ k.k0) * 0x9E3779B1u + k.k1);
}
__host__ __device__ __forceinline__ float rng_uniform(RngKey k, uint32_t idx) {
    return (float)(rng_u32(k, idx) >> 8) * (1.0f / 16777216.0f);
}
__host__ __device__ __forceinline__ bool rng_keep(RngKey k, uint32_t idx, float p) {
    return rng_uniform(k, idx) >= p;
}
__device__ __forceinline__ float rng_normal(RngKey k, uint32_t idx) {
    uint32_t a = rng_u32(k, idx);
    uint32_t b = mix32(a ^ 0x68bc21ebu) + k.k0;
    float u1 = ((float)(a >> 8) + 1.0f) * (1.0f / 16777216.0f);
    float u2 = (float)(b >> 8) * (1.0f / 16777216.0f);
    return sqrtf(-2.0f * logf(u1)) * cosf(6.28318530717958647692f * u2);
}

__device__ __forceinline__ float sigmoidf_(float x) { return 1.0f / (1.0f + expf(-x)); }

__device__ __forceinline__ float wave_sum(float v) {
#pragma unroll
    for (int o = 32; o > 0; o >>= 1) v += __shfl_xor(v, o, 64);
    return v;
}
__device__ __forceinline__ float wave_max(float v) {
#pragma unroll
    for (int o = 32; o > 0; o >>= 1) v = fmaxf(v, __shfl_xor(v, o, 64));
    return v;
}

}

void t2_set_error(const char* fmt, ...);
#define T2_CHECK_HIP(expr)                                                                   \
    do {                                                                                     \
        hipError_t e_ = (expr);                                                              \
        if (e_ != hipSuccess) {                                                              \
            t2_set_error("%s:%d: %s -> %s", __FILE__, __LINE__, #expr, hipGetErrorString(e_)); \
            return -2;                                                                       \
        }                                                                                    \
    } while (0)
#define T2_REQUIRE(cond, ...)                                                                \
    do {                                                                                     \
        if (!(cond)) {                                                                       \
            t2_set_error(__VA_ARGS__);                                                       \
            return -1;                                                                       \
        }                                                                                    \
    } while (0)
#define T2_LAUNCH_CHECK() T2_CHECK_HIP(hipGetLastError())
#define T2_TRY_RC(expr)             \
    do {                            \
        int rc__ = (expr);          \
        if (rc__ != 0) return rc__; \
    } while (0)

#include <mutex>
#include <tuple>
#include <vector>
inline int t2_allow_dynamic_lds(const void* fn, size_t smem) {
    if (smem <= 64 * 1024) return 0;
    int dev = 0;
    T2_CHECK_HIP(hipGetDevice(&dev));
    static std::mutex mu;
    static std::vector<std::tuple<int, const void*, size_t>> done;
    std::lock_guard<std::mutex> lock(mu);
    for (auto& e : done)
        if (std::get<0>(e) == dev && std::get<1>(e) == fn) {
            if (std::get<2>(e) >= smem) return 0;
            T2_CHECK_HIP(hipFuncSetAttribute(fn, hipFuncAttributeMaxDynamicSharedMemorySize, (int)smem));
            std::get<2>(e) = smem;
            return 0;
        }
    T2_CHECK_HIP(hipFuncSetAttribute(fn, hipFuncAttributeMaxDynamicSharedMemorySize, (int)smem));
    done.emplace_back(dev, fn, smem);
    return 0;
}
```

tacotron2_subword_amd/csrc/conv.hip:

```cpp
#include "kernels.h"

namespace t2 {

namespace {

inline int grid_for(size_t n, int block = 256, int cap = 8192) {
    size_t g = (n + block - 1) / block;
    return (int)(g < 1 ? 1 : (g > (size_t)cap ? cap : g));
}

__global__ void permute_w_fwd_kernel(const float* __restrict__ w, float* __restrict__ wp, int Co, int Ci, int K) {
    const size_t n = (size_t)Co * Ci * K;
    for (size_t i = blockIdx.x * (size_t)blockDim.x + threadIdx.x; i < n; i += (size_t)gridDim.x * blockDim.x) {
        const int ci = (int)(i % Ci); const size_t r = i / Ci; const int dk = (int)(r % K), co = (int)(r / K);
        wp[i] = w[((size_t)co * Ci + ci) * K + dk];
    }
}
__global__ void permute_w_bwd_kernel(const float* __restrict__ w, float* __restrict__ wt, int Co, int Ci, int K) {
    const size_t n = (size_t)Co * Ci * K;
    for (size_t i = blockIdx.x * (size_t)blockDim.x + threadIdx.x; i < n; i += (size_t)gridDim.x * blockDim.x) {
        const int co = (int)(i % Co); const size_t r = i / Co; const int dk = (int)(r % K), ci = (int)(r / K);
        wt[i] = w[((size_t)co * Ci + ci) * K + (K - 1 - dk)];
    }
}
__global__ void unpermute_dw_kernel(const float* __restrict__ dwp, float* __restrict__ dw, int Co, int Ci, int K) {
    const size_t n = (size_t)Co * Ci * K;
    for (size_t i = blockIdx.x * (size_t)blockDim.x + threadIdx.x; i < n; i += (size_t)gridDim.x * blockDim.x) {
        const int dk = (int)(i % K); const size_t r = i / K; const int ci = (int)(r % Ci), co = (int)(r / Ci);
        dw[i] = dwp[((size_t)co * K + dk) * Ci + ci];
    }
}

struct BnElem {
    const float* z; const float* mean; const float* invstd; const float* gamma; const float* beta;
    int C; int act; float drop_p; RngKey key;
};
__device__ __forceinline__ float act_fwd(float u, int act) {
    return act == ACT_RELU ? fmaxf(u, 0.f) : (act == ACT_TANH ? tanhf(u) : u);
}

template <int MODE>
__global__ void colreduce_stage1_kernel(BnElem e, const float* __restrict__ dy, float* __restrict__ du, int M, int slabs,
                                        float* __restrict__ scratch) {
    const int C = e.C;
    const int c = blockIdx.x * 64 + (threadIdx.x & 63);
    const int sub = threadIdx.x >> 6;
    const int rows = (M + slabs - 1) / slabs;
    const int m0 = blockIdx.y * rows, m1 = min(M, m0 + rows);
    __shared__ float p0[4][64], p1[4][64];
    float a0 = 0.f, a1 = 0.f;
    if (c < C) {
        const float mean = MODE >= 1 ? e.mean[c] : 0.f;
        const float inv = MODE == 2 ? e.invstd[c] : 0.f, ga = MODE == 2 ? e.gamma[c] : 0.f, be = MODE == 2 ? e.beta[c] : 0.f;
        const float scale = e.drop_p > 0.f ? 1.0f / (1.0f - e.drop_p) : 1.0f;
        for (int m = m0 + sub; m < m1; m += 4) {
            const size_t i = (size_t)m * C + c;
            const float z = e.z[i];
            if (MODE == 0) a0 += z;
            else if (MODE == 1) { const float d = z - mean; a0 += d * d; }
            else {
                const float xh = (z - mean) * inv, u = xh * ga + be;
                float g = dy[i];
                if (e.drop_p > 0.f) g = rng_keep(e.key, (uint32_t)i, e.drop_p) ? g * scale : 0.f;
                if (e.act == ACT_RELU) g = u > 0.f ? g : 0.f;
                else if (e.act == ACT_TANH) { const float t = tanhf(u); g *= 1.0f - t * t; }
                du[i] = g;
                a0 += g; a1 += g * xh;
            }
        }
    }
    p0[sub][threadIdx.x & 63] = a0; p1[sub][threadIdx.x & 63] = a1;
    __syncthreads();
    if (sub == 0 && c < C) {
        const int l = threadIdx.x;
        scratch[(size_t)blockIdx.y * C + c] = p0[0][l] + p0[1][l] + p0[2][l] + p0[3][l];
        if (MODE == 2) scratch[(size_t)(slabs + blockIdx.y) * C + c] = p1[0][l] + p1[1][l] + p1[2][l] + p1[3][l];
    }
}
__global__ void colreduce_stage2_kernel(const float* __restrict__ scratch, int C, int slabs, int M, int mode, float eps,
                                        float* out0, float* out1) {
    const int c = blockIdx.x * blockDim.x + threadIdx.x;
    if (c >= C) return;
    auto ordered_sum = [&](const float* __restrict__ p) {
        float acc = 0.f;
        int s = 0;
        for (; s + 16 <= slabs; s += 16) {
            float v[16];
#pragma unroll
            for (int j = 0; j < 16; ++j) v[j] = p[(size_t)(s + j) * C];
#pragma unroll
            for (int j = 0; j < 16; ++j) acc += v[j];
        }
        for (; s < slabs; ++s) acc += p[(size_t)s * C];
        return acc;
    };
    const float s0 = ordered_sum(scratch + c);
    const float s1 = mode == 2 ? ordered_sum(scratch + (size_t)slabs * C + c) : 0.f;
    if (mode == 0) out0[c] = s0 / (float)M;
    else if (mode == 1) { const float var = s0 / (float)M; out0[c] = 1.0f / sqrtf(var + eps); if (out1) out1[c] = var; }
    else { out0[c] = s0; out1[c] = s1; }
}

__global__ void bn_apply_kernel(BnElem e, const float* __restrict__ residual, float* __restrict__ y, size_t n) {
    const float scale = e.drop_p > 0.f ? 1.0f / (1.0f - e.drop_p) : 1.0f;
    for (size_t i = blockIdx.x * (size_t)blockDim.x + threadIdx.x; i < n; i += (size_t)gridDim.x * blockDim.x) {
        const int c = (int)(i % e.C);
        float v = act_fwd((e.z[i] - e.mean[c]) * e.invstd[c] * e.gamma[c] + e.beta[c], e.act);
        if (e.drop_p > 0.f) v = rng_keep(e.key, (uint32_t)i, e.drop_p) ? v * scale : 0.f;
        if (residual) v += residual[i];
        y[i] = v;
    }
}
__global__ void bn_bwd_dz_kernel(BnElem e, const float* __restrict__ du, const float* __restrict__ sdu, const float* __restrict__ sduxh,
                                 int M, int training, float* __restrict__ dz, size_t n) {
    const float invM = 1.0f / (float)M;
    for (size_t i = blockIdx.x * (size_t)blockDim.x + threadIdx.x; i < n; i += (size_t)gridDim.x * blockDim.x) {
        const int c = (int)(i % e.C);
        const float inv = e.invstd[c], ga = e.gamma[c];
        float g = du[i];
        if (training) {
            const float xh = (e.z[i] - e.mean[c]) * inv;
            g = g - sdu[c] * invM - xh * sduxh[c] * invM;
        }
        dz[i] = g * ga * inv;
    }
}
__global__ void bn_running_kernel(const float* mean, const float* var, int C, int M, float momentum, float* rm, float* rv) {
    const int c = blockIdx.x * blockDim.x + threadIdx.x;
    if (c >= C) return;
    const float unb = var[c] * ((float)M / (float)(M > 1 ? M - 1 : 1));
    rm[c] = (1.0f - momentum) * rm[c] + momentum * mean[c];
    rv[c] = (1.0f - momentum) * rv[c] + momentum * unb;
}
__global__ void invstd_from_var_kernel(const float* var, int C, float eps, float* invstd) {
    const int c = blockIdx.x * blockDim.x + threadIdx.x;
    if (c < C) invstd[c] = 1.0f / sqrtf(var[c] + eps);
}

__global__ void embedding_fwd_kernel(const long* __restrict__ ids, const float* __restrict__ table, float* __restrict__ out, int rows, int D) {
    const size_t n = (size_t)rows * (D / 4);
    for (size_t i = blockIdx.x * (size_t)blockDim.x + threadIdx.x; i < n; i += (size_t)gridDim.x * blockDim.x) {
        const int r = (int)(i / (D / 4)), q = (int)(i % (D / 4));
        reinterpret_cast<f32x4*>(out)[i] = reinterpret_cast<const f32x4*>(table + ids[r] * (long)D)[q];
    }
}
__global__ void embedding_bwd_kernel(const long* __restrict__ ids, const float* __restrict__ dout, float* __restrict__ dtable, int rows, int D) {
    const int v = blockIdx.x;
    extern __shared__ int hits[];
    __shared__ int wave_cnt[2][16];
    const int wave = threadIdx.x >> 6, lane = threadIdx.x & 63, nw = blockDim.x >> 6;
    int run = 0;
    long idn = (int)threadIdx.x < rows ? ids[threadIdx.x] : -1;
    for (int r0 = 0, it = 0; r0 < rows; r0 += blockDim.x, ++it) {
        const int r = r0 + threadIdx.x, rn = r + blockDim.x;
        const long id = idn;
        idn = rn < rows ? ids[rn] : -1;
        const bool hit = r < rows && id == v;
        const unsigned long long m = __ballot(hit);
        int* wc = wave_cnt[it & 1];
        if (lane == 0) wc[wave] = __popcll(m);
        __syncthreads();
        int base = run, tot = 0;
        for (int w = 0; w < nw; ++w) { const int cw = wc[w]; if (w < wave) base += cw; tot += cw; }
        if (hit) hits[base + __popcll(m & ((1ull << lane) - 1ull))] = r;
        run += tot;
    }
    __syncthreads();
    const int nhit = run;
    for (int c = threadIdx.x; c < D; c += blockDim.x) {
        float acc = 0.f;
        int h = 0;
        for (; h + 8 <= nhit; h += 8) {
            float x[8];
#pragma unroll
            for (int j = 0; j < 8; ++j) x[j] = dout[(size_t)hits[h + j] * D + c];
#pragma unroll
            for (int j = 0; j < 8; ++j) acc += x[j];
        }
        for (; h < nhit; ++h) acc += dout[(size_t)hits[h] * D + c];
        dtable[(size_t)v * D + c] = acc;
    }
}

template <int MODE>
int colreduce(const BnElem& e, const float* dy, float* du, int M, float eps, float* out0, float* out1, float* scratch, hipStream_t s) {
    const int slabs = M >= 64 * 64 ? 64 : (M >= 64 ? M / 64 : 1);
    hipLaunchKernelGGL(colreduce_stage1_kernel<MODE>, dim3((e.C + 63) / 64, slabs), dim3(256), 0, s, e, dy, du, M, slabs, scratch);
    T2_LAUNCH_CHECK();
    hipLaunchKernelGGL(colreduce_stage2_kernel, dim3((e.C + 255) / 256), dim3(256), 0, s, scratch, e.C, slabs, M, MODE, eps, out0, out1);
    T2_LAUNCH_CHECK();
    return 0;
}

}

int conv_bn_fwd(const ConvBnFwd& a, hipStream_t s) {
    const int M = a.B * a.T;
    T2_REQUIRE(a.Cin % 4 == 0 && a.K % 2 == 1, "conv_bn_fwd: Cin=%d must be a multiple of 4 and the kernel size odd (%d)", a.Cin, a.K);
    T2_REQUIRE((size_t)M * a.Cout < (1ull << 32), "conv_bn_fwd: B*T*Cout too large for 32-bit RNG indices");
    const size_t nw = (size_t)a.Cout * a.Cin * a.K;
    hipLaunchKernelGGL(permute_w_fwd_kernel, dim3(grid_for(nw)), dim3(256), 0, s, a.w, a.wperm, a.Cout, a.Cin, a.K);
    T2_LAUNCH_CHECK();
    GemmDesc g = gemm_desc();
    g.A = a.x; g.conv_a = 1; g.conv_T = a.T; g.conv_C = a.Cin; g.conv_pad = (a.K - 1) / 2;
    g.B = a.wperm; g.sbn = (long)a.K * a.Cin; g.sbk = 1;
    g.C = a.z; g.ldc = a.Cout; g.M = M; g.N = a.Cout; g.K = a.K * a.Cin; g.bias1 = a.bias;
    g.ws = a.gemm_ws; g.ws_bytes = a.gemm_ws_bytes;
    T2_TRY_RC(gemm(g, s));
    BnElem e{a.z, a.mean, a.invstd, a.gamma, a.beta, a.Cout, a.act, a.drop_p, rng_key(a.seed, a.site)};
    if (a.training) {
        T2_TRY_RC(colreduce<0>(e, nullptr, nullptr, M, a.eps, a.mean, nullptr, a.scratch, s));
        T2_TRY_RC(colreduce<1>(e, nullptr, nullptr, M, a.eps, a.invstd, a.var, a.scratch, s));
        if (a.run_mean) {
            hipLaunchKernelGGL(bn_running_kernel, dim3((a.Cout + 255) / 256), dim3(256), 0, s, a.mean, a.var, a.Cout, M, 0.1f, a.run_mean, a.run_var);
            T2_LAUNCH_CHECK();
        }
    } else {
        T2_CHECK_HIP(hipMemcpyAsync(a.mean, a.run_mean, sizeof(float) * a.Cout, hipMemcpyDeviceToDevice, s));
        hipLaunchKernelGGL(invstd_from_var_kernel, dim3((a.Cout + 255) / 256), dim3(256), 0, s, a.run_var, a.Cout, a.eps, a.invstd);
        T2_LAUNCH_CHECK();
    }
    const size_t n = (size_t)M * a.Cout;
    hipLaunchKernelGGL(bn_apply_kernel, dim3(grid_for(n)), dim3(256), 0, s, e, a.residual, a.y, n);
    T2_LAUNCH_CHECK();
    return 0;
}

int conv_bn_bwd(const ConvBnBwd& a, hipStream_t s) {
    const int M = a.B * a.T;
    const size_t n = (size_t)M * a.Cout;
    BnElem e{a.z, a.mean, a.invstd, a.gamma, a.beta, a.Cout, a.act, a.drop_p, rng_key(a.seed, a.site)};
    T2_TRY_RC(colreduce<2>(e, a.dy, a.dz, M, a.eps, a.dbeta, a.dgamma, a.scratch, s));
    hipLaunchKernelGGL(bn_bwd_dz_kernel, dim3(grid_for(n)), dim3(256), 0, s, e, a.dz, a.dbeta, a.dgamma, M, a.training, a.dz, n);
    T2_LAUNCH_CHECK();
    T2_TRY_RC(colsum(a.dz, a.Cout, M, a.Cout, a.dbias, nullptr, a.scratch, s));
    GemmDesc g = gemm_desc();
    g.A = a.dz; g.sam = 1; g.sak = a.Cout;
    g.B = a.x; g.conv_b = 1; g.conv_T = a.T; g.conv_C = a.Cin; g.conv_pad = (a.K - 1) / 2;
    g.C = a.wperm; g.ldc = (long)a.K * a.Cin; g.M = a.Cout; g.N = a.K * a.Cin; g.K = M;
    g.ws = a.gemm_ws; g.ws_bytes = a.gemm_ws_bytes;
    T2_TRY_RC(gemm(g, s));
    const size_t nw = (size_t)a.Cout * a.Cin * a.K;
    hipLaunchKernelGGL(unpermute_dw_kernel, dim3(grid_for(nw)), dim3(256), 0, s, a.wperm, a.dw, a.Cout, a.Cin, a.K);
    T2_LAUNCH_CHECK();
    if (a.dx) {
        T2_REQUIRE(a.Cout % 4 == 0, "conv_bn_bwd: Cout=%d must be a multiple of 4", a.Cout);
        hipLaunchKernelGGL(permute_w_bwd_kernel, dim3(grid_for(nw)), dim3(256), 0, s, a.w, a.wperm, a.Cout, a.Cin, a.K);
        T2_LAUNCH_CHECK();
        GemmDesc h = gemm_desc();
        h.A = a.dz; h.conv_a = 1; h.conv_T = a.T; h.conv_C = a.Cout; h.conv_pad = (a.K - 1) / 2;
        h.B = a.wperm; h.sbn = (long)a.K * a.Cout; h.sbk = 1;
        h.C = a.dx; h.ldc = a.Cin; h.M = M; h.N = a.Cin; h.K = a.K * a.Cout;
        h.beta = a.dx_accumulate ? 1.f : 0.f;
        h.ws = a.gemm_ws; h.ws_bytes = a.gemm_ws_bytes;
        T2_TRY_RC(gemm(h, s));
    }
    return 0;
}

int embedding_fwd(const long* ids, const float* table, float* out, int rows, int D, hipStream_t s) {
    T2_REQUIRE(D % 4 == 0, "embedding: dim %d must be a multiple of 4", D);
    hipLaunchKernelGGL(embedding_fwd_kernel, dim3(grid_for((size_t)rows * (D / 4))), dim3(256), 0, s, ids, table, out, rows, D);
    T2_LAUNCH_CHECK();
    return 0;
}
int embedding_bwd(const long* ids, const float* dout, float* dtable, int rows, int D, int vocab, hipStream_t s) {
    const size_t smem = (size_t)rows * sizeof(int);
    T2_REQUIRE(smem <= 150 * 1024, "embedding_bwd: %d tokens do not fit the LDS hit list", rows);
    T2_TRY_RC(t2_allow_dynamic_lds(reinterpret_cast<const void*>(embedding_bwd_kernel), smem));
    hipLaunchKernelGGL(embedding_bwd_kernel, dim3(vocab), dim3(256), smem, s, ids, dout, dtable, rows, D);
    T2_LAUNCH_CHECK();
    return 0;
}

}
```

tacotron2_subword_amd/csrc/elementwise.hip:

```cpp
#include "kernels.h"

namespace t2 {

namespace {

inline int grid_for(size_t n, int block = 256, int cap = 4096) {
    size_t g = (n + block - 1) / block;
    return (int)(g < 1 ? 1 : (g > (size_t)cap ? cap : g));
}

__global__ void rng_keep_mask_kernel(RngKey k, uint32_t n, float p, uint8_t* out) {
    for (uint32_t i = blockIdx.x * blockDim.x + threadIdx.x; i < n; i += gridDim.x * blockDim.x)
        out[i] = rng_keep(k, i, p) ? 1 : 0;
}
__global__ void rng_normal_kernel(RngKey k, uint32_t n, float* out) {
    for (uint32_t i = blockIdx.x * blockDim.x + threadIdx.x; i < n; i += gridDim.x * blockDim.x)
        out[i] = rng_normal(k, i);
}

__global__ void teacher_inputs_kernel(const float* __restrict__ mel, float* __restrict__ X, int B, int M, int T) {
    __shared__ float tile[32][33];
    const int b = blockIdx.z, t0 = blockIdx.x * 32, m0 = blockIdx.y * 32;
    const int tx = threadIdx.x & 31, ty = threadIdx.x >> 5;
    for (int i = ty; i < 32; i += 8) {
        const int m = m0 + i, ts = t0 + tx - 1;
        float v = 0.f;
        if (m < M && ts >= 0 && ts < T) v = mel[((long)b * M + m) * T + ts];
        tile[i][tx] = v;
    }
    __syncthreads();
    for (int i = ty; i < 32; i += 8) {
        const int t = t0 + i, m = m0 + tx;
        if (t < T && m < M) X[((long)t * B + b) * M + m] = tile[tx][i];
    }
}

__global__ void transpose_btc_kernel(const float* __restrict__ in, float* __restrict__ out, int B, int T, int C,
                                     const int* __restrict__ lengths, float fill) {
    __shared__ float tile[32][33];
    const int b = blockIdx.z, t0 = blockIdx.x * 32, c0 = blockIdx.y * 32;
    const int tx = threadIdx.x & 31, ty = threadIdx.x >> 5;
    for (int i = ty; i < 32; i += 8) {
        const int t = t0 + i, c = c0 + tx;
        tile[i][tx] = (t < T && c < C) ? in[((long)b * T + t) * C + c] : 0.f;
    }
    __syncthreads();
    const int len = lengths ? lengths[b] : T;
    for (int i = ty; i < 32; i += 8) {
        const int c = c0 + i, t = t0 + tx;
        if (c < C && t < T) out[((long)b * C + c) * T + t] = t < len ? tile[tx][i] : fill;
    }
}

__global__ void mask_bt_kernel(float* x, int B, int T, const int* __restrict__ lengths, float fill) {
    const long n = (long)B * T;
    for (long i = blockIdx.x * (long)blockDim.x + threadIdx.x; i < n; i += (long)gridDim.x * blockDim.x) {
        const int b = (int)(i / T), t = (int)(i % T);
        if (t >= lengths[b]) x[i] = fill;
    }
}

__global__ void mask_btc_kernel(float* x, int B, int T, int C, const int* __restrict__ lengths, float fill) {
    const size_t n = (size_t)B * T * C;
    for (size_t i = blockIdx.x * (size_t)blockDim.x + threadIdx.x; i < n; i += (size_t)gridDim.x * blockDim.x) {
        const size_t r = i / C;
        if ((int)(r % T) >= lengths[r / T]) x[i] = fill;
    }
}

__global__ void fill_kernel(float* p, float v, size_t n) {
    for (size_t i = blockIdx.x * (size_t)blockDim.x + threadIdx.x; i < n; i += (size_t)gridDim.x * blockDim.x) p[i] = v;
}

__global__ void permute_rows_kernel(const float* __restrict__ in, float* __restrict__ out, int R1, int R2, int W) {
    const size_t n = (size_t)R1 * R2 * W;
    for (size_t i = blockIdx.x * (size_t)blockDim.x + threadIdx.x; i < n; i += (size_t)gridDim.x * blockDim.x) {
        const int w = (int)(i % W);
        const size_t r = i / W;
        const int r1 = (int)(r % R1), r2 = (int)(r / R1);
        out[i] = in[((size_t)r1 * R2 + r2) * W + w];
    }
}

__global__ void relu_drop_bwd_kernel(const float* __restrict__ dy, const float* __restrict__ y, float* dz, float scale, size_t n) {
    for (size_t i = blockIdx.x * (size_t)blockDim.x + threadIdx.x; i < n; i += (size_t)gridDim.x * blockDim.x)
        dz[i] = y[i] > 0.f ? dy[i] * scale : 0.f;
}

__global__ void colsum_stage1_kernel(const float* __restrict__ X, long ld, int M, int N, int slabs, float* scratch) {
    const int n = blockIdx.x * 64 + (threadIdx.x & 63);
    const int sub = threadIdx.x >> 6;
    const int rows = (M + slabs - 1) / slabs;
    const int m0 = blockIdx.y * rows, m1 = min(M, m0 + rows);
    __shared__ float part[4][64];
    float acc = 0.f;
    if (n < N) for (int m = m0 + sub; m < m1; m += 4) acc += X[(long)m * ld + n];
    part[sub][threadIdx.x & 63] = acc;
    __syncthreads();
    if (sub == 0 && n < N) scratch[(long)blockIdx.y * N + n] = part[0][threadIdx.x] + part[1][threadIdx.x] + part[2][threadIdx.x] + part[3][threadIdx.x];
}
__device__ __forceinline__ float ordered_sum16(const float* __restrict__ p, int count, long stride) {
    float acc = 0.f;
    int s = 0;
    for (; s + 16 <= count; s += 16) {
        float v[16];
#pragma unroll
        for (int j = 0; j < 16; ++j) v[j] = p[(long)(s + j) * stride];
#pragma unroll
        for (int j = 0; j < 16; ++j) acc += v[j];
    }
    for (; s < count; ++s) acc += p[(long)s * stride];
    return acc;
}
__global__ void colsum_stage2_kernel(const float* __restrict__ scratch, int N, int slabs, float* out, float* out2) {
    const int n = blockIdx.x * blockDim.x + threadIdx.x;
    if (n >= N) return;
    const float acc = ordered_sum16(scratch + n, slabs, N);
    out[n] = acc;
    if (out2) out2[n] = acc;
}
__global__ void fold_halves_kernel(float* __restrict__ X, size_t rows, int A) {
    const size_t n = rows * A;
    for (size_t i = blockIdx.x * (size_t)blockDim.x + threadIdx.x; i < n; i += (size_t)gridDim.x * blockDim.x) {
        float* r = X + (i / A) * 2 * A + (i % A);
        r[0] += r[A];
    }
}
__global__ void batch_sum_kernel(const float* __restrict__ X, int B, int n, float* out) {
    const int i = blockIdx.x * blockDim.x + threadIdx.x;
    if (i >= n) return;
    out[i] = ordered_sum16(X + i, B, n);
}

}

int permute_rows(const float* in, float* out, int R1, int R2, int W, hipStream_t s) {
    const size_t n = (size_t)R1 * R2 * W;
    hipLaunchKernelGGL(permute_rows_kernel, dim3(grid_for(n)), dim3(256), 0, s, in, out, R1, R2, W);
    T2_LAUNCH_CHECK();
    return 0;
}
int relu_drop_bwd(const float* dy, const float* y, float* dz, float scale, size_t n, hipStream_t s) {
    hipLaunchKernelGGL(relu_drop_bwd_kernel, dim3(grid_for(n)), dim3(256), 0, s, dy, y, dz, scale, n);
    T2_LAUNCH_CHECK();
    return 0;
}
int colsum(const float* X, long ld, int M, int N, float* out, float* out2, float* scratch, hipStream_t s) {
    const int slabs = M >= 64 * 64 ? 64 : (M >= 64 ? M / 64 : 1);
    hipLaunchKernelGGL(colsum_stage1_kernel, dim3((N + 63) / 64, slabs), dim3(256), 0, s, X, ld, M, N, slabs, scratch);
    T2_LAUNCH_CHECK();
    hipLaunchKernelGGL(colsum_stage2_kernel, dim3((N + 255) / 256), dim3(256), 0, s, scratch, N, slabs, out, out2);
    T2_LAUNCH_CHECK();
    return 0;
}
int fold_halves(float* X, size_t rows, int A, hipStream_t s) {
    hipLaunchKernelGGL(fold_halves_kernel, dim3(grid_for(rows * A)), dim3(256), 0, s, X, rows, A);
    T2_LAUNCH_CHECK();
    return 0;
}
int batch_sum(const float* X, int B, int n, float* out, hipStream_t s) {
    hipLaunchKernelGGL(batch_sum_kernel, dim3((n + 255) / 256), dim3(256), 0, s, X, B, n, out);
    T2_LAUNCH_CHECK();
    return 0;
}

int rng_keep_mask(uint64_t seed, uint32_t site, uint32_t n, float p, uint8_t* out, hipStream_t s) {
    hipLaunchKernelGGL(rng_keep_mask_kernel, dim3(grid_for(n)), dim3(256), 0, s, rng_key(seed, site), n, p, out);
    T2_LAUNCH_CHECK();
    return 0;
}
int rng_normal(uint64_t seed, uint32_t site, uint32_t n, float* out, hipStream_t s) {
    hipLaunchKernelGGL(rng_normal_kernel, dim3(grid_for(n)), dim3(256), 0, s, rng_key(seed, site), n, out);
    T2_LAUNCH_CHECK();
    return 0;
}
int teacher_inputs(const float* mel, float* X, int B, int M, int T, hipStream_t s) {
    dim3 grid((T + 31) / 32, (M + 31) / 32, B);
    hipLaunchKernelGGL(teacher_inputs_kernel, grid, dim3(256), 0, s, mel, X, B, M, T);
    T2_LAUNCH_CHECK();
    return 0;
}
int transpose_btc_to_bct(const float* in, float* out, int B, int T, int C, const int* lengths, float fill, hipStream_t s) {
    dim3 grid((T + 31) / 32, (C + 31) / 32, B);
    hipLaunchKernelGGL(transpose_btc_kernel, grid, dim3(256), 0, s, in, out, B, T, C, lengths, fill);
    T2_LAUNCH_CHECK();
    return 0;
}
int mask_bt(float* x, int B, int T, const int* lengths, float fill, hipStream_t s) {
    hipLaunchKernelGGL(mask_bt_kernel, dim3(grid_for((size_t)B * T)), dim3(256), 0, s, x, B, T, lengths, fill);
    T2_LAUNCH_CHECK();
    return 0;
}
int mask_btc(float* x, int B, int T, int C, const int* lengths, float fill, hipStream_t s) {
    hipLaunchKernelGGL(mask_btc_kernel, dim3(grid_for((size_t)B * T * C)), dim3(256), 0, s, x, B, T, C, lengths, fill);
    T2_LAUNCH_CHECK();
    return 0;
}
int fill_f32(float* p, float v, size_t n, hipStream_t s) {
    hipLaunchKernelGGL(fill_kernel, dim3(grid_for(n)), dim3(256), 0, s, p, v, n);
    T2_LAUNCH_CHECK();
    return 0;
}

}
```

tacotron2_subword_amd/csrc/gemm.hip:

```cpp
#include "kernels.h"
#include <cstdlib>
#include <algorithm>
#include <type_traits>

namespace t2 {

static int g_precision = 0;
static int env_int(const char* name, int dflt) { const char* v = getenv(name); return v && *v ? atoi(v) : dflt; }
static int g_stage = env_int("T2_GEMM_STAGE", 1);
void set_gemm_staging(int on) { g_stage = on != 0; }
constexpr int kStageMin = 256;
constexpr int kSplitMinMflopDefault = 2147;
static double g_split_min_flop = 1e6 * kSplitMinMflopDefault;
void set_gemm_split_min_mflop(int mflop) { g_split_min_flop = 1e6 * (mflop < 0 ? kSplitMinMflopDefault : mflop); }
void set_precision(int p) { g_precision = p; }
int get_precision() { return g_precision; }
static uint64_t g_counts[4] = {0, 0, 0, 0};
void gemm_counts(uint64_t* out, int reset) {
    for (int i = 0; i < 4; ++i) { out[i] = g_counts[i]; if (reset) g_counts[i] = 0; }
}

namespace {

constexpr int BK = 16;
// ... 905 lines not shown
    using I0 = std::integral_constant<int, 0>; using I1 = std::integral_constant<int, 1>; using I2 = std::integral_constant<int, 2>;

    stage(0, 0); stage(2, 0); stage(3, 0); stage(1, 0); stage(0, 1); stage(2, 1);
    T2_G256_WAIT(8);
    __builtin_amdgcn_s_barrier();
    if (wr == 1) __builtin_amdgcn_s_barrier();
    int kt = 0;
    for (; kt + 2 < nkt2; kt += 2) { ktile(I0{}, I0{}, kt); ktile(I1{}, I0{}, kt + 1); }
    ktile(I0{}, I1{}, kt);
    ktile(I1{}, I2{}, kt + 1);
    if (wr == 0) __builtin_amdgcn_s_barrier();
#undef T2_G256_WAIT

    const RngKey key = rng_key(d.seed, d.site);
    float* ws = d.splitk > 1 ? d.ws + (long)split * (long)d.M * d.N : nullptr;
    float* stg = reinterpret_cast<float*>(smem16) + wave * 4096;
    const bool vec_ok = ws || ((reinterpret_cast<uintptr_t>(d.C) & 15) == 0 && d.ldc % 4 == 0);
    const float inv_keep = d.drop_p > 0.f ? 1.0f / (1.0f - d.drop_p) : 1.0f;
    const int c4 = (lane & 15) * 4, n = n0 + (KM ? (wc >> 1) * 128 + (c4 >> 5) * 64 + (wc & 1) * 32 + (c4 & 31) : wc * 64 + c4);
    f32x4 bias = {0.f, 0.f, 0.f, 0.f};
    if (!ws) {
#pragma unroll
        for (int c = 0; c < 4; ++c) bias[c] = (d.bias1 ? d.bias1[n + c] : 0.f) + (d.bias2 ? d.bias2[n + c] : 0.f);
    }
    __syncthreads();
#pragma unroll
    for (int p = 0; p < 2; ++p) {
#pragma unroll
        for (int ii = 0; ii < 2; ++ii)
#pragma unroll
            for (int j = 0; j < 2; ++j)
#pragma unroll
                for (int e = 0; e < 16; ++e) stg[(ii * 32 + (e & 3) + 8 * (e >> 2) + 4 * hk) * 64 + j * 32 + r] = acc[2 * p + ii][j][e];
        __syncthreads();
        for (int it = 0; it < 16; ++it) {
            const int row = it * 4 + (lane >> 4);
            const int m = m0 + wr * 128 + p * 64 + row;
            f32x4 v = *reinterpret_cast<const f32x4*>(stg + row * 64 + c4);
            if (ws) { *reinterpret_cast<f32x4*>(ws + (long)m * d.N + n) = v; continue; }
            const uint32_t ibase = d.drop_base + (uint32_t)m * d.drop_mstride + (uint32_t)n;
#pragma unroll
            for (int c = 0; c < 4; ++c) {
                float x = apply_act(d.alpha * v[c] + bias[c], d.act);
                if (d.drop_p > 0.f) x = rng_keep(key, ibase + c, d.drop_p) ? x * inv_keep : 0.f;
                v[c] = x;
            }
            const long mo = d.crow_mod ? (long)(m % d.crow_mod) * d.crow_mul + m / d.crow_mod : (long)m;
            float* pc = d.C + mo * d.ldc + n;
            if (vec_ok) {
                if (d.beta != 0.f) v += d.beta * *reinterpret_cast<const f32x4*>(pc);
                *reinterpret_cast<f32x4*>(pc) = v;
            } else {
#pragma unroll
                for (int c = 0; c < 4; ++c) pc[c] = d.beta != 0.f ? v[c] + d.beta * pc[c] : v[c];
            }
        }
        if (p == 0) __syncthreads();
    }
}

template <bool CONV_A, bool KM, bool CONV_B>
int launch_bf16src256(const GemmK& g, const __bf16* pa, long lda, const __bf16* pb, long ldb, dim3 grid, hipStream_t s) {
    constexpr size_t smem = 128 * 1024;
    T2_TRY_RC(t2_allow_dynamic_lds(reinterpret_cast<const void*>(gemm_bf16src256_kernel<CONV_A, KM, CONV_B>), smem));
    GemmK gk = g;
    gk.xcd_swizzle = (grid.x * grid.y) % 8 == 0 && grid.y >= 4;
    hipLaunchKernelGGL((gemm_bf16src256_kernel<CONV_A, KM, CONV_B>), grid, dim3(512), smem, s, gk, pa, lda, pb, ldb);
    T2_LAUNCH_CHECK();
    return 0;
}

__global__ void stage_kc_kernel(const float* __restrict__ src, long ld, __bf16* __restrict__ dst, int rows, int K) {
    const int k8 = K >> 3;
    const long total = (long)rows * k8;
    for (long t = blockIdx.x * (long)blockDim.x + threadIdx.x; t < total; t += (long)gridDim.x * blockDim.x) {
        const long row = t / k8; const int s = (int)(t - row * k8);
        const float* p = src + row * ld + s * 8;
        const f32x4 lo = *reinterpret_cast<const f32x4*>(p), hi = *reinterpret_cast<const f32x4*>(p + 4);
        *reinterpret_cast<bf16x8*>(dst + row * (long)K + s * 8) = pack8(lo, hi);
    }
}
__global__ __launch_bounds__(256) void stage_mc_kernel(const float* __restrict__ src, long ld, __bf16* __restrict__ dst, int rows, int K) {
    __shared__ float tile[64][65];
    const int r0 = blockIdx.x * 64, k0 = blockIdx.y * 64;
#pragma unroll
    for (int i = 0; i < 4; ++i) {
        const int k = (threadIdx.x >> 4) + 16 * i, r4 = (threadIdx.x & 15) * 4;
        const f32x4 v = *reinterpret_cast<const f32x4*>(src + (long)(k0 + k) * ld + r0 + r4);
#pragma unroll
        for (int j = 0; j < 4; ++j) tile[k][r4 + j] = v[j];
    }
    __syncthreads();
#pragma unroll
    for (int i = 0; i < 2; ++i) {
        const int kg = threadIdx.x & 7, row = (threadIdx.x >> 3) + 32 * i;
        bf16x8 o;
#pragma unroll
        for (int j = 0; j < 8; ++j) o[j] = (__bf16)tile[kg * 8 + j][row];
        *reinterpret_cast<bf16x8*>(dst + (long)(r0 + row) * K + k0 + kg * 8) = o;
    }
}

int stage_operand(const float* src, bool kc, long ld, __bf16* dst, int rows, int K, hipStream_t s) {
    if (kc) {
        long blocks = ((long)rows * (K >> 3) + 255) / 256;
        if (blocks > 8192) blocks = 8192;
        hipLaunchKernelGGL(stage_kc_kernel, dim3((unsigned)blocks), dim3(256), 0, s, src, ld, dst, rows, K);
    } else {
        hipLaunchKernelGGL(stage_mc_kernel, dim3(rows / 64, K / 64), dim3(256), 0, s, src, ld, dst, rows, K);
    }
    T2_LAUNCH_CHECK();
    return 0;
}

__device__ __forceinline__ void split8(const f32x4& lo4, const f32x4& hi4, bf16x8& h, bf16x8& l) {
#pragma unroll
    for (int j = 0; j < 8; ++j) {
        const float x = j < 4 ? lo4[j] : hi4[j - 4];
        const __bf16 xh = (__bf16)x;
        h[j] = xh; l[j] = (__bf16)(x - (float)xh);
    }
}
__global__ void stage_split_kc_kernel(const float* __restrict__ src, long ld, __bf16* __restrict__ dst, int rows, int K, int lo_slot, int row_group) {
    const int k8 = K >> 3;
    const long total = (long)rows * k8;
    for (long t = blockIdx.x * (long)blockDim.x + threadIdx.x; t < total; t += (long)gridDim.x * blockDim.x) {
        const long row = t / k8; const int k = (int)(t - row * k8) * 8;
        const float* p = src + row * ld + k;
        bf16x8 h, l;
        split8(*reinterpret_cast<const f32x4*>(p), *reinterpret_cast<const f32x4*>(p + 4), h, l);
        long o, step;
        if (row_group) { o = ((row / row_group) * 3 * row_group + row % row_group) * (long)K + k; step = (long)row_group * K; }
        else { o = row * 3 * (long)K + (k >> 6) * 192 + (k & 63); step = 64; }
#pragma unroll
        for (int slot = 0; slot < 3; ++slot) *reinterpret_cast<bf16x8*>(dst + o + slot * step) = slot == lo_slot ? l : h;
    }
}
__global__ __launch_bounds__(256) void stage_split_mc_kernel(const float* __restrict__ src, long ld, __bf16* __restrict__ dst, int rows, int K, int lo_slot) {
    __shared__ float tile[64][65];
    const int r0 = blockIdx.x * 64, k0 = blockIdx.y * 64;
#pragma unroll
    for (int i = 0; i < 4; ++i) {
        const int k = (threadIdx.x >> 4) + 16 * i, r4 = (threadIdx.x & 15) * 4;
        const f32x4 v = *reinterpret_cast<const f32x4*>(src + (long)(k0 + k) * ld + r0 + r4);
#pragma unroll
        for (int j = 0; j < 4; ++j) tile[k][r4 + j] = v[j];
    }
    __syncthreads();
#pragma unroll
    for (int i = 0; i < 2; ++i) {
        const int kg = threadIdx.x & 7, row = (threadIdx.x >> 3) + 32 * i;
        f32x4 a, b;
#pragma unroll
        for (int j = 0; j < 4; ++j) { a[j] = tile[kg * 8 + j][row]; b[j] = tile[kg * 8 + 4 + j][row]; }
        bf16x8 h, l;
        split8(a, b, h, l);
        __bf16* o = dst + (long)(r0 + row) * 3 * K + 3 * (long)k0 + kg * 8;
#pragma unroll
        for (int slot = 0; slot < 3; ++slot) *reinterpret_cast<bf16x8*>(o + slot * 64) = slot == lo_slot ? l : h;
    }
}
int stage_split_operand(const float* src, bool kc, long ld, __bf16* dst, int rows, int K, int lo_slot, int row_group, hipStream_t s) {
    if (kc) {
        long blocks = ((long)rows * (K >> 3) + 255) / 256;
        if (blocks > 8192) blocks = 8192;
        hipLaunchKernelGGL(stage_split_kc_kernel, dim3((unsigned)blocks), dim3(256), 0, s, src, ld, dst, rows, K, lo_slot, row_group);
    } else {
        hipLaunchKernelGGL(stage_split_mc_kernel, dim3(rows / 64, K / 64), dim3(256), 0, s, src, ld, dst, rows, K, lo_slot);
    }
    T2_LAUNCH_CHECK();
    return 0;
}

inline bool aligned16(const void* p) { return (reinterpret_cast<uintptr_t>(p) & 15) == 0; }
inline size_t round256(size_t n) { return (n + 255) & ~(size_t)255; }

int check_gemm(const GemmDesc& d) {
    T2_REQUIRE(d.M > 0 && d.N > 0 && d.K > 0 && d.batch > 0, "gemm: bad shape M=%d N=%d K=%d batch=%d", d.M, d.N, d.K, d.batch);
    if (d.conv_a || d.conv_b) {
        T2_REQUIRE(d.conv_T > 0 && d.conv_C > 0 && d.conv_C % 4 == 0 && !(d.conv_a && d.conv_b), "gemm: bad implicit-conv operand (T=%d C=%d)", d.conv_T, d.conv_C);
        T2_REQUIRE(d.batch == 1, "gemm: implicit-conv operands need batch == 1");
        if (d.conv_a) T2_REQUIRE(d.K % d.conv_C == 0 && aligned16(d.A), "gemm: conv A operand: K=%d C=%d", d.K, d.conv_C);
        if (d.conv_b) T2_REQUIRE(d.N % d.conv_C == 0 && aligned16(d.B), "gemm: conv B operand: N=%d C=%d", d.N, d.conv_C);
    }
    T2_REQUIRE(d.conv_a || d.sam == 1 || d.sak == 1, "gemm: A needs one unit stride (sam=%ld sak=%ld)", d.sam, d.sak);
    T2_REQUIRE(d.conv_b || d.sbn == 1 || d.sbk == 1, "gemm: B needs one unit stride (sbn=%ld sbk=%ld)", d.sbn, d.sbk);
    T2_REQUIRE(d.drop_p == 0.f || (d.batch == 1 && (long)d.M * d.N < (1l << 32)), "gemm: dropout epilogue needs batch==1 and M*N < 2^32");
    return 0;
}

int choose_splitk(const GemmDesc& d, bool tile256, long tiles, int kch, size_t ws_bytes) {
    if (!(d.ws && d.beta == 0.f)) return 1;
    int sp = 1;
    if (tile256) {
        const int nkt = kch / 4;
        if (d.splitk > 0) sp = std::min(d.splitk, std::max(1, nkt / 2));
        else if (tiles < 512) {
            double best = 0.0;
            for (int c = 1; c <= 16; ++c) {
                if (c > 1 && nkt / c < 16) break;
                const long wgs = tiles * c, rounds = (wgs + 255) / 256;
                const double eff = (double)wgs / (256.0 * rounds);
                if (eff > best * 1.05) { best = eff; sp = c; }
            }
        }
    } else if (d.splitk > 0) sp = d.splitk;
    else if (tiles < 512 && kch >= 64) sp = std::min((int)((1024 + tiles - 1) / tiles), kch / 16);
    const size_t per = (size_t)d.batch * d.M * d.N * sizeof(float);
    if ((size_t)sp * per > ws_bytes) sp = (int)(ws_bytes / per);
    return std::max(sp, 1);
}

int run_gemm(const GemmDesc& d, const GemmPlan& p, hipStream_t s) {
    GemmK g{};
    g.d = d;
    g.kchunks = p.kchunks; g.avec = p.avec; g.bvec = p.bvec;
    if (d.conv_a) { g.d.sam = 0; g.d.sak = 1; }
    if (d.conv_b) { g.d.sbk = 0; g.d.sbn = 1; }
    if (d.drop_mstride == 0) g.d.drop_mstride = (uint32_t)d.N;
    g.d.K = p.K; g.d.conv_C = p.conv_C; g.d.splitk = p.splitk;
    const size_t staged = p.a.bytes + p.b.bytes;
    if (staged) { g.d.ws = reinterpret_cast<float*>(reinterpret_cast<unsigned char*>(d.ws) + staged); g.d.ws_bytes = d.ws_bytes - staged; }
    const int tile = p.kernel == GemmKernel::f32_64 ? 64 : p.kernel >= GemmKernel::src256 ? 256 : 128;
    const dim3 grid((d.N + tile - 1) / tile, (d.M + tile - 1) / tile, d.batch * p.splitk);
    if (gemm_reads_bf16_copies(p.kernel)) {
        __bf16* a16 = reinterpret_cast<__bf16*>(d.ws), * b16 = reinterpret_cast<__bf16*>(reinterpret_cast<unsigned char*>(d.ws) + p.a.bytes);
        if (p.a.src == GemmSrc::staged) T2_TRY_RC(stage_planned(d.A, p.a, p.split, a16, s));
        if (p.b.src == GemmSrc::staged) T2_TRY_RC(stage_planned(d.B, p.b, p.split, b16, s));
        const __bf16* pa = p.a.src == GemmSrc::caller ? d.A16 : a16, * pb = p.b.src == GemmSrc::caller ? d.B16 : b16;
        if (p.kernel == GemmKernel::src256km && d.conv_b) T2_TRY_RC((launch_bf16src256<false, true, true>(g, pa, p.a.ld, pb, p.b.ld, grid, s)));
        else if (p.kernel == GemmKernel::src256km) T2_TRY_RC((launch_bf16src256<false, true, false>(g, pa, p.a.ld, pb, p.b.ld, grid, s)));
        else if (p.kernel == GemmKernel::src256 && d.conv_a) T2_TRY_RC((launch_bf16src256<true, false, false>(g, pa, p.a.ld, pb, p.b.ld, grid, s)));
        else if (p.kernel == GemmKernel::src256) T2_TRY_RC((launch_bf16src256<false, false, false>(g, pa, p.a.ld, pb, p.b.ld, grid, s)));
        else if (d.conv_a) T2_TRY_RC((launch_bf16src<true, 2, 2, 2, 2, 2>(g, pa, p.a.ld, pb, p.b.ld, grid, s)));
        else T2_TRY_RC((launch_bf16src<false, 2, 2, 2, 2, 2>(g, pa, p.a.ld, pb, p.b.ld, grid, s)));
    } else {
        using Kernel = void (*)(GemmK);
        static const Kernel bf16conv[] = {gemm_bf16_kernel<true, true>, gemm_bf16_kernel<true, false>, gemm_bf16_kernel<false, true>, gemm_bf16_kernel<false, false>};
        static const Kernel f32_64[] = {gemm_kernel<64, 64, true, true>, gemm_kernel<64, 64, true, false>, gemm_kernel<64, 64, false, true>, gemm_kernel<64, 64, false, false>};
        static const Kernel f32_128[] = {gemm_kernel<128, 128, true, true>, gemm_kernel<128, 128, true, false>, gemm_kernel<128, 128, false, true>, gemm_kernel<128, 128, false, false>};
        const bool conv16 = p.kernel == GemmKernel::bf16conv;
        const size_t smem = conv16 ? (size_t)4 * 128 * PK16 * sizeof(__bf16) : 0;
        const Kernel kernel = (conv16 ? bf16conv : p.kernel == GemmKernel::f32_64 ? f32_64 : f32_128)[(g.d.sak == 1 ? 0 : 2) + (g.d.sbk == 1 ? 0 : 1)];
        hipLaunchKernelGGL(kernel, grid, dim3(256), smem, s, g);
    }
    T2_LAUNCH_CHECK();
    if (p.splitk > 1) {
        const long total = (long)d.batch * d.M * d.N;
        int blocks = (int)((total + 255) / 256);
        if (blocks > 2048) blocks = 2048;
        hipLaunchKernelGGL(splitk_reduce_kernel, dim3(blocks), dim3(256), 0, s, g.d);
        T2_LAUNCH_CHECK();
    }
    return 0;
}

}

int stage_bf16(const float* src, bool kc, long ld, __bf16* dst, int rows, int K, hipStream_t s) {
    T2_REQUIRE(rows > 0 && K > 0 && rows % 64 == 0 && K % 64 == 0 && ld % 4 == 0 && aligned16(src) && aligned16(dst),
               "stage_bf16: rows=%d K=%d ld=%ld must be whole 64-tiles of 16-byte aligned rows", rows, K, ld);
    return stage_operand(src, kc, ld, dst, rows, K, s);
}

int stage_split_bf16(const float* src, bool kc, long ld, __bf16* dst, int rows, int K, int lo_slot, int row_group, hipStream_t s) {
    T2_REQUIRE(rows > 0 && K > 0 && rows % 64 == 0 && K % 64 == 0 && ld % 4 == 0 && aligned16(src) && aligned16(dst) &&
               (lo_slot == 1 || lo_slot == 2) && row_group >= 0 && (!row_group || (kc && rows % row_group == 0)),
               "stage_split_bf16: rows=%d K=%d ld=%ld must be whole 64-tiles of 16-byte aligned rows", rows, K, ld);
    return stage_split_operand(src, kc, ld, dst, rows, K, lo_slot, row_group, s);
}

int stage_planned(const float* src, const GemmOperandPlan& o, bool split, __bf16* dst, hipStream_t s) {
    return split ? stage_split_operand(src, o.kc, o.ld_src, dst, o.rows, o.K, o.lo_slot, o.row_group, s)
                 : stage_operand(src, o.kc, o.ld_src, dst, o.rows, o.K, s);
}

const char* gemm_plan_name(const GemmPlan& p) {
    static const char* const names[] = {"f32_64", "f32_128", "bf16conv", "src128", "src256", "src256km", "x3src128", "x3src256", "x3src256km"};
    return names[(int)p.kernel + (p.split ? 3 : 0)];
}

GemmPlan plan_gemm(const GemmDesc& d) {
    GemmPlan p{};
    const bool conv_any = d.conv_a || d.conv_b;
    const bool akc = d.conv_a || d.sak == 1, bkc = !d.conv_b && d.sbk == 1;
    const long lda = d.conv_a ? d.conv_C : akc ? d.sam : d.sak;
    const long ldb = d.conv_b ? d.conv_C : bkc ? d.sbn : d.sbk;
    p.avec = aligned16(d.A) && d.bsA % 4 == 0 && lda % 4 == 0;
    p.bvec = aligned16(d.B) && d.bsB % 4 == 0 && ldb % 4 == 0;
    p.K = d.K; p.conv_C = d.conv_C;

    const bool large = !d.fp32_only && d.M >= 64 && d.N >= 64 && d.K >= 64 && (!conv_any || d.conv_C % 8 == 0);
    const bool use_bf16 = g_precision == 1 && large;
    const bool want_split = g_precision == 2 && large && 2.0 * d.M * d.N * d.K >= g_split_min_flop;
    const int kmul = want_split ? 3 : 1;
    const bool copies = g_precision != 2 || (want_split && d.split16);
    bool a_caller = copies && d.A16, b_caller = copies && d.B16;
    static const int g_t256 = env_int("T2_GEMM_256", 1);
    const bool shape256 = g_t256 && d.M % 256 == 0 && d.N % 256 == 0 && d.K >= 128;
    const long ld_km = std::max(std::max((long)d.M, a_caller && d.a16_kmajor ? d.lda16 : 0l), std::max((long)(d.conv_b ? d.conv_C : d.N), b_caller && d.b16_kmajor ? d.ldb16 : 0l));
    const bool km = shape256 && !akc && !bkc && !d.conv_a && (!d.conv_b || d.conv_C % 256 == 0) && (long)d.K * kmul * ld_km * 2 < (1l << 31);
    a_caller = a_caller && (d.a16_kmajor != 0) == km;
    b_caller = b_caller && (d.b16_kmajor != 0) == km;
    const bool conv_ok = !conv_any || (d.conv_a && d.conv_C % 64 == 0 && !a_caller && !b_caller) || (d.conv_b && km && (!want_split || d.K % d.conv_T == 0));
    bool staged = false;
    size_t ws_bytes = d.ws_bytes;
    if ((use_bf16 || want_split) && g_stage && conv_ok && d.batch == 1 && d.M % 128 == 0 && d.N % 128 == 0 && d.K % 64 == 0) {
        const size_t a_elems = d.conv_a ? (size_t)d.M * d.conv_C : (size_t)d.M * d.K;
        const size_t b_elems = d.conv_b ? (size_t)d.K * d.conv_C : (size_t)d.N * d.K;
        const size_t need_a = a_caller ? 0 : round256(kmul * a_elems * sizeof(__bf16));
        const size_t need_b = b_caller ? 0 : round256(kmul * b_elems * sizeof(__bf16));
        const bool big = (a_caller || d.N >= kStageMin) && (b_caller || d.M >= kStageMin);
        const bool ok_src = (a_caller ? aligned16(d.A16) && d.lda16 % 8 == 0 : p.avec != 0) && (b_caller ? aligned16(d.B16) && d.ldb16 % 8 == 0 : p.bvec != 0);
        if (big && ok_src && (need_a + need_b == 0 || (d.ws && aligned16(d.ws) && d.ws_bytes >= need_a + need_b))) {
            staged = true;
            p.a.bytes = need_a; p.b.bytes = need_b;
            ws_bytes -= need_a + need_b;
        }
    }
    p.split = want_split && staged;
    if (p.split) { p.K = 3 * d.K; if (d.conv_a) p.conv_C = 3 * d.conv_C; }
    const int kch = (p.K + BK - 1) / BK;
    int splitk;
    if (staged) {
        const bool use256 = shape256 && (!d.conv_a || (long)d.M * p.conv_C * 2 < (1l << 31));
        p.kernel = !use256 ? GemmKernel::src128 : km ? GemmKernel::src256km : GemmKernel::src256;
        const int lo_grp = !p.split ? 0 : d.conv_b ? d.K : 64;
        const int lo = p.split ? 1 : 0;
        if (a_caller) p.a = {GemmSrc::caller, d.lda16};
        else if (d.conv_a) p.a = {GemmSrc::staged, p.conv_C, true, lda, d.M, d.conv_C, lo, 0, p.a.bytes};
        else if (km) p.a = {GemmSrc::staged, d.M, true, lda, d.K, d.M, lo, lo_grp, p.a.bytes};
        else p.a = {GemmSrc::staged, p.K, akc, lda, d.M, d.K, lo, 0, p.a.bytes};
        if (b_caller) p.b = {GemmSrc::caller, d.ldb16};
        else if (d.conv_b) p.b = {GemmSrc::staged, d.conv_C, true, ldb, d.K, d.conv_C, 2 * lo, lo_grp, p.b.bytes};
        else if (km) p.b = {GemmSrc::staged, d.N, true, ldb, d.K, d.N, 2 * lo, lo_grp, p.b.bytes};
        else p.b = {GemmSrc::staged, p.K, bkc, ldb, d.N, d.K, 2 * lo, 0, p.b.bytes};
        splitk = use256 ? choose_splitk(d, true, (long)(d.M / 256) * (d.N / 256), kch, ws_bytes) : choose_splitk(d, false, (long)(d.M / 128) * (d.N / 128), kch, ws_bytes);
    } else {
        const bool can_split = d.ws && d.beta == 0.f && kch >= 64;
        const long tiles128 = (long)((d.M + 127) / 128) * ((d.N + 127) / 128) * d.batch;
        const bool small = !use_bf16 && ((d.M <= 64 || d.N <= 64) || (tiles128 < 256 && !can_split));
        p.kernel = use_bf16 ? GemmKernel::bf16conv : small ? GemmKernel::f32_64 : GemmKernel::f32_128;
        splitk = choose_splitk(d, false, small ? (long)((d.M + 63) / 64) * ((d.N + 63) / 64) * d.batch : tiles128, kch, ws_bytes);
    }
    const int round = p.kernel >= GemmKernel::bf16conv ? 3 : 0;
    p.kchunks = ((kch + splitk - 1) / splitk + round) & ~round;
    p.splitk = (kch + p.kchunks - 1) / p.kchunks;
    if (p.kernel >= GemmKernel::src256 && p.splitk > 1 && kch - (p.splitk - 1) * p.kchunks < 8) {
        p.kchunks = ((kch + p.splitk - 2) / (p.splitk - 1) + 3) & ~3;
        p.splitk = (kch + p.kchunks - 1) / p.kchunks;
    }
    return p;
}

int gemm_plan(const GemmDesc& d, GemmPlan* out) {
    T2_TRY_RC(check_gemm(d));
    *out = plan_gemm(d);
    T2_REQUIRE((long)d.batch * out->splitk <= 65535, "gemm: batch*splitk too large (%d*%d)", d.batch, out->splitk);
    return 0;
}

int gemm(const GemmDesc& d, hipStream_t s) {
    GemmPlan p;
    T2_TRY_RC(gemm_plan(d, &p));
    static const int g_log = env_int("T2_GEMM_LOG", 0);
    if (g_log)
        fprintf(stderr, "t2gemm M=%d N=%d K=%d batch=%d %s%s kernel=%s splitk=%d stageA=%d stageB=%d convA=%d convB=%d beta=%g\n", d.M, d.N, d.K, d.batch,
                d.conv_a || d.sak == 1 ? "A[m][k]" : "A[k][m]", !d.conv_b && d.sbk == 1 ? " B[n][k]" : " B[k][n]", gemm_plan_name(p),
                p.splitk, p.a.src == GemmSrc::staged, p.b.src == GemmSrc::staged, d.conv_a, d.conv_b, (double)d.beta);
    ++g_counts[p.split ? 3 : gemm_reads_bf16_copies(p.kernel) ? 2 : p.kernel == GemmKernel::bf16conv ? 1 : 0];
    return run_gemm(d, p, s);
}

}
```

tacotron2_subword_amd/csrc/kernels.h:

```cpp
#pragma once
#include "common.h"

namespace t2 {

enum Act : int { ACT_NONE = 0, ACT_RELU = 1, ACT_TANH = 2 };

struct GemmDesc {
    const float* A; const float* B; float* C;
    int M, N, K;
    long sam, sak;
    long sbn, sbk;
    long ldc;
    int batch; long bsA, bsB, bsC;
    float alpha, beta;
    const float* bias1; const float* bias2;
    int act;
    float drop_p; uint64_t seed; uint32_t site;
    uint32_t drop_base, drop_mstride;
    float* ws; size_t ws_bytes;
    int splitk;
    int conv_a, conv_b, conv_T, conv_C, conv_pad;
    int fp32_only;
    const __bf16* A16; long lda16;
    const __bf16* B16; long ldb16;
    int a16_kmajor, b16_kmajor;
    int split16;
    int crow_mod; long crow_mul;
};
inline GemmDesc gemm_desc() {
    GemmDesc d{}; d.batch = 1; d.alpha = 1.f; d.beta = 0.f; d.act = ACT_NONE; d.drop_p = 0.f; return d;
}
int gemm(const GemmDesc& d, hipStream_t s);

enum class GemmKernel : int {
    f32_64, f32_128,
    bf16conv,
    src128,
    src256,
    src256km
};
inline bool gemm_reads_bf16_copies(GemmKernel k) { return k >= GemmKernel::src128; }
enum class GemmSrc : int { fp32, staged, caller };
struct GemmOperandPlan {
    GemmSrc src;
    long ld;
    bool kc; long ld_src; int rows, K, lo_slot, row_group;
    size_t bytes;
};
struct GemmPlan {
    GemmKernel kernel;
    bool split;
    int splitk, kchunks;
    int K, conv_C;
    GemmOperandPlan a, b;
    int avec, bvec;
};
GemmPlan plan_gemm(const GemmDesc& d);
int gemm_plan(const GemmDesc& d, GemmPlan* out);
const char* gemm_plan_name(const GemmPlan& p);
int stage_planned(const float* src, const GemmOperandPlan& o, bool split, __bf16* dst, hipStream_t s);
int stage_bf16(const float* src, bool kc, long ld, __bf16* dst, int rows, int K, hipStream_t s);
int stage_split_bf16(const float* src, bool kc, long ld, __bf16* dst, int rows, int K, int lo_slot, int row_group, hipStream_t s);
void set_precision(int p);
int get_precision();
void gemm_counts(uint64_t* out, int reset);
void set_gemm_split_min_mflop(int mflop);
void set_gemm_staging(int on);

constexpr int kMaxSeg = 6;
struct LstmSeg { const float* x; long ldx; const float* w; long ldw; int k; };
struct LstmStream {
    LstmSeg seg[kMaxSeg]; int nseg;
    const float* pre; long ldpre;
    const float* bias1; const float* bias2;
    const float* c_prev; long ldc_prev;
    float* gates; long ldgates;
    float* c_new; long ldc_new;
    float* h_out; long ldh_out;
    float* h_out2; long ldh_out2;
    float* c_out; long ldc_out;
    uint32_t site_h, site_c; uint32_t idx_base, idx_bstride;
    const int* lengths; int t;
    const float* wq; int A; float* qpart;
    const __bf16* x16; long ldx16; const __bf16* w16; long ldw16; int k16;
    __bf16* h16_out; long ldh16;
    __bf16* h16_out2; long ldh16_2;
};
constexpr int kMaxLstmStreams = 4;
struct LstmStepDesc { LstmStream st[kMaxLstmStreams]; int nstreams; int B, H; float drop_p; uint64_t seed; };
int lstm_step_fwd(const LstmStepDesc& d, hipStream_t s);

struct LstmBwdStream {
    const float* dh1; long lddh1;
    const float* dh2; long lddh2;
    const float* part; int nparts; long part_stride; long ldpart; int part_col;
    const float* dq; long lddq; const float* wq; int A;
    int dq_parts;
    const float* gates; long ldgates;
    const float* c_new; long ldc_new;
    const float* c_prev; long ldc_prev;
    float* dc_state;
    float* dg; long lddg;
    __bf16* dg16;
    uint32_t site_h, site_c, idx_base, idx_bstride;
};
struct LstmBwdPointDesc { LstmBwdStream st[kMaxLstmStreams]; int nstreams; int B, H; float drop_p; uint64_t seed; int first; };
int lstm_bwd_pointwise(const LstmBwdPointDesc& d, hipStream_t s);

struct LstmBwdSeg { const float* w; long ldw; int ncols; };
struct LstmBwdGemmStream {
    const float* dg; long lddg; LstmBwdSeg seg[3]; int nseg; float* part;
    const __bf16* dg16; const __bf16* wt16;
};
struct LstmBwdGemmDesc { LstmBwdGemmStream st[kMaxLstmStreams]; int nstreams; int B, H4, KS, NC; };
int lstm_bwd_gemm(const LstmBwdGemmDesc& d, hipStream_t s);
int lstm_bwd_ksplit(int H4);
int cast_rows_bf16(const float* src, long ld_src, __bf16* dst, long ld_dst, int R, int C, hipStream_t s);
int cast_transpose_bf16(const float* src, long ld_src, __bf16* dst, long ld_dst, int R, int C, hipStream_t s);

constexpr int kDcaC = 8, kDcaK = 21, kDcaP = 11, kDcaPad = (kDcaK - 1) / 2;
struct DcaWeights {
    const float* bW;
    const float* V;
    const float* F;
    const float* U;
    const float* T; const float* bT;
    const float* v;
    const float* P;
};
struct AttnStream {
    const float* query; long ldq;
    const float* qpart; int nparts;
    float* q_out; long ldq_out;
    const float* pm;
    const float* memory;
    const int* lengths;
    const float* a_prev; long lda_prev;
    float* a_out; long lda_out;
    float* p_out; long ldp_out;
    const float* wcum_prev; long ldwcum_prev;
    float* wcum_out; long ldwcum_out;
    float* ctx1; long ldctx1;
    float* ctx2; long ldctx2;
    __bf16* ctx16; long ldctx16;
    __bf16* ctx16b; long ldctx16b;
    const float* v;
    const float* loc_conv; const float* loc_dense;
    uint32_t site_noise; uint32_t idx_base, idx_bstride;
    int Tin;
    const float* gmm_b1; const float* gmm_w2; const float* gmm_b2;
    const float* mu_prev; float* mu_out;
    DcaWeights dca;
    float mask_value;
};
constexpr int kGmmK = 5, kGmmPad = 8;
struct AttnStepDesc {
    AttnStream st[2]; int nstreams; int B, A, E; int kind;
    int F, Kc; float noise_std; uint64_t seed; int first;
    int lsa_pa;
    int max_pos;
};
int attention_step_fwd(const AttnStepDesc& d, hipStream_t s);

struct AttnBwdStream {
    const float* dctx[3]; long lddctx[3];
    const float* part; int nparts; long part_stride; long ldpart; int part_col;
    const float* dalign; long lddalign;
    const float* q; long ldq;
    const float* pm; const float* memory;
    const float* p; long ldp;
    const float* a_prev; long lda_prev;
    const float* v;
    float* carry;
    float* carry_out;
    float* dctx_out; long lddctx_out;
    float* dq_out; long lddq_out;
    float* dv_acc;
    float* dpm_acc;
    int Tin;
    const float* w; long ldw;
    const float* wcum_prev; long ldwcum_prev;
    const float* loc_conv; const float* loc_dense;
    float* carry_cum;
    float* dconv_acc; float* ddense_acc;
    const float* gmm_w2; const float* gmm_b2;
    const float* mu; long ldmu;
    float* mu_carry;
    float* dw2_acc; float* db2_acc;
    DcaWeights dca;
    float* dca_acc;
};
__host__ __device__ inline size_t dca_acc_floats(int A) { return (size_t)2 * A + 2 * (size_t)A * kDcaC + kDcaC * kDcaK + (size_t)kDcaC * kDcaK * A; }
struct AttnBwdDesc { AttnBwdStream st[2]; int nstreams; int B, A, E; int first; int kind, F, Kc; int nsplit; };
int attention_step_bwd(const AttnBwdDesc& d, hipStream_t s);


enum ChainKind : int { CHAIN_LSTM = 0, CHAIN_SMA = 1, CHAIN_LSA = 2 };
struct ChainStream {
    const __bf16* w16; long ldw16;
    const float* pre;
    const float* wq;
    float* gates; float* c_new; float* c_out;
    float* h_out; long ldh;
    __bf16* h16_out; long ldh16;
    int coff, ctx2off;
    const float* pm; const float* memory; const int* lengths; int Tin;
    float* align; float* psel; float* wcum; float* qs;
    const float* v; const float* loc_conv; const float* loc_dense;
    float* usave; float* locsave;
    uint32_t site_h, site_c, site_noise;
    float mask_value;
};
struct ChainDesc {
    ChainStream st[2]; int NS, B, T, t0, t1;
    int H, E, A, WD, WO;
    float* din; __bf16* din16; float* dout;
    int kind, F, Kc, max_pos;
    float drop_p, noise_std; uint64_t seed;
    unsigned char* X; float* Q; unsigned* cnt; unsigned* err; unsigned q_bytes;
    int UT, RT, CS;
    int dec, P, M, Hd;
    const float* bias1[2]; const float* bias2[2];
    float* att_c[2];
    const __bf16* wd16; long ldwd;
    const float* dbias1; const float* dbias2; float* dec_c;
    const float* proj_w; const float* proj_b; const float* gate_w; const float* gate_b;
    const float* pw1[2]; const float* pw2[2];
    float* mel_out; long ldmel; float* gate_out; long ldgate;
    float thr; int32_t* stop_index; int32_t* done;
    float pdrop; uint32_t psite1[2], psite2[2];
    unsigned char* XD; unsigned char* XM;
    int lds_Tin, lds_Jp, lds_Jm; int Jp[2], Jm[2];
};
bool chain_plan(ChainDesc& d);
constexpr int kCntShards = 16;
enum ChainStatus : int { CHAIN_STATUS_FWD_ATT = 0, CHAIN_STATUS_FWD_LSTM = 1, CHAIN_STATUS_BWD_LSTM = 2, CHAIN_STATUS_BWD_ATT = 3 };
enum ChainWsClear : int { CHAIN_WS_STATUS = 0, CHAIN_WS_TEACHER = 1, CHAIN_WS_DECODE = 2 };
size_t chain_fwd_ws_floats(int NS, int B, int Ha, int E, int P, int Hd, int A);
int chain_fwd_ws_clear(float* ws, size_t ws_floats, ChainWsClear what, hipStream_t s);
int chain_fwd(ChainDesc d, float* ws, size_t ws_floats, hipStream_t s);
int chain_device_cus();
unsigned* chain_sticky_words();
bool chain_device_claim();

struct ChainBwdStream {
    const __bf16* wt16; long ldwt;
    const float* dh1; long lddh1;
    const float* gates; const float* c_new; const float* c_out;
    float* dg;
    float* dc_state;
    float* dbias_part;
    uint32_t site_h, site_c;
    const float* dctx_a; long lddctx_a;
    const float* dctx_b; long lddctx_b;
    const float* dalign;
    const float* qs;
    const float* pm; const float* memory; int Tin;
    const float* psel; const float* align;
    const float* v; const float* wq;
    float* dctx_out;
    float* dq_out;
    float* dv_acc;
    float* dpm_acc;
    const float* wcum;
    const float* usave; const float* locsave;
    const float* loc_conv; const float* loc_dense;
    float* dconv_acc; float* ddense_acc;
    const __bf16* wdt16;
};
struct ChainBwdDesc {
    ChainBwdStream st[2]; int NS, B, T, t0, t1, H, kind;
    int E, A, F, Kc;
    float drop_p; uint64_t seed;
    unsigned char* X; unsigned char* PB; unsigned* err; unsigned pb_bytes;
    unsigned char* PBC; unsigned pbc_bytes; float* DQX; float* CARRYX;
    int lds_Tc;
};
bool chain_bwd_plan(ChainBwdDesc& d);
size_t chain_bwd_ws_floats(int kind, int NS, int B, int Ha, int E, int A, int F, int Kc, int Hd);
int chain_bwd(ChainBwdDesc d, float* ws, size_t ws_floats, hipStream_t s);

struct EncChainDesc {
    int ND, B, T, H;
    const float* pre[2];
    const float* w_hh[2];
    int reverse[2];
    const int* lengths;
    float* h[2]; long ldh;
    float* c[2]; float* gates[2];
    float* X; unsigned* cnt; unsigned* err;
};
struct EncChainBwdDesc {
    int ND, B, T, H;
    const float* w_hh[2]; int reverse[2];
    const float* c[2]; const float* gates[2];
    const float* dh[2]; long lddh;
    float* dpre[2];
    float* X; float* PB; unsigned* cnt; unsigned* err;
};
bool enc_chain_covers(int ND, int B, int H);
size_t enc_chain_ws_floats(int ND, int B, int H, int backward);
int enc_chain_fwd(EncChainDesc d, float* ws, size_t ws_floats, hipStream_t s);
int enc_chain_bwd(EncChainBwdDesc d, float* ws, size_t ws_floats, hipStream_t s);

struct StepTailDesc {
    int B, M, P, WO, NS, t;
    int do_proj, do_prenet;
    const float* dout; long lddout;
    const float* proj_w; const float* proj_b; const float* gate_w; const float* gate_b;
    float* mel_out; long ldmel; float* gate_out; long ldgate;
    float thr; int32_t* stop_index; int32_t* done;
    const float* x_in; long ldx_in;
    const float* w1t[2]; const float* w2[2];
    float* p1[2]; float* p2[2]; long ldp;
    __bf16* p2_16[2]; long ldp16;
    float drop_p; uint64_t seed; uint32_t site1[2], site2[2]; uint32_t drop_base, drop_mstride;
};
int step_tail(const StepTailDesc& d, hipStream_t s);

struct ConvBnFwd {
    const float* x; int B, T, Cin, Cout, K;
    const float* w; const float* bias;
    const float* gamma; const float* beta; float* run_mean; float* run_var;
    int training; float eps; int act; float drop_p; uint64_t seed; uint32_t site;
    const float* residual;
    float* z; float* mean; float* invstd; float* var;
    float* y;
    float* wperm; float* scratch;
    float* gemm_ws; size_t gemm_ws_bytes;
};
int conv_bn_fwd(const ConvBnFwd& a, hipStream_t s);
struct ConvBnBwd {
    const float* x; int B, T, Cin, Cout, K;
    const float* w; const float* gamma; const float* beta;
    const float* z; const float* mean; const float* invstd;
    int training; float eps; int act; float drop_p; uint64_t seed; uint32_t site;
    const float* dy;
    float* dz;
    float* dw; float* dbias; float* dgamma; float* dbeta;
    float* dx; int dx_accumulate;
    float* wperm; float* scratch; float* gemm_ws; size_t gemm_ws_bytes;
};
int conv_bn_bwd(const ConvBnBwd& a, hipStream_t s);
int embedding_fwd(const long* ids, const float* table, float* out, int rows, int D, hipStream_t s);
int embedding_bwd(const long* ids, const float* dout, float* dtable, int rows, int D, int vocab, hipStream_t s);

struct AdamTensor { float* p; const float* g; float* m; float* v; long numel; int first_chunk; int pad_; };
int adam_chunks(long numel);
int adam_norm(const AdamTensor* table_dev, int n_tensors, int n_chunks, float* partial, float* norm_out, float max_norm, hipStream_t s);
int adam_step(const AdamTensor* table_dev, int n_tensors, int n_chunks, float* partial, float* norm_out, float max_norm,
              float lr, float b1, float b2, float eps, float wd, int step, hipStream_t s);

int rng_keep_mask(uint64_t seed, uint32_t site, uint32_t n, float p, uint8_t* out, hipStream_t s);
int rng_normal(uint64_t seed, uint32_t site, uint32_t n, float* out, hipStream_t s);
int teacher_inputs(const float* mel, float* X, int B, int M, int T, hipStream_t s);
int transpose_btc_to_bct(const float* in, float* out, int B, int T, int C, const int* lengths, float fill, hipStream_t s);
int mask_bt(float* x, int B, int T, const int* lengths, float fill, hipStream_t s);
int mask_btc(float* x, int B, int T, int C, const int* lengths, float fill, hipStream_t s);
int fill_f32(float* p, float v, size_t n, hipStream_t s);
int permute_rows(const float* in, float* out, int R1, int R2, int W, hipStream_t s);
int relu_drop_bwd(const float* dy, const float* y, float* dz, float scale, size_t n, hipStream_t s);
int colsum(const float* X, long ld, int M, int N, float* out, float* out2, float* scratch, hipStream_t s);
int fold_halves(float* X, size_t rows, int A, hipStream_t s);
int batch_sum(const float* X, int B, int n, float* out, hipStream_t s);

}
```

Baseline: 978,400 mel-frames/s.

## Hand off bf16 activations between conv-BN layers and vectorise column reductions

Conv-BN layers can now emit a bf16 copy of their output, which the next layer's GEMM reads directly instead of restaging the fp32 activation. Backward reuses the saved bf16 inputs, writes the weights in permuted bf16 and gives dz a bf16 copy, so the GEMMs can skip their staging kernels. Column-sum and BN column reductions are rewritten with 16-byte vector loads and multiple rows kept in flight. The cost is extra bf16 activation buffers held for backward, plus a more complex planning check that the GEMM route stays the same.

After: 1.002 million mel-frames/s (median of 6 runs). 1.02x the previous value.

```diff
diff --git a/include/t2amd.h b/include/t2amd.h
--- a/include/t2amd.h
+++ b/include/t2amd.h
@@ -190,6 +190,7 @@
     float* z; float* mean; float* invstd; float* var;
     float* y;
     float* ws; size_t ws_floats;
+    const void* x16; void* y16; int handoff;
 } t2_conv_bn_args;
 int t2_conv_bn_forward(const t2_conv_bn_args* a, void* stream);
 typedef struct t2_conv_bn_bwd_args {
@@ -201,6 +202,7 @@
     float* dw; float* dbias; float* dgamma; float* dbeta;
     float* dx; int dx_accumulate;
     float* ws; size_t ws_floats;
+    const void* x16; int handoff;
 } t2_conv_bn_bwd_args;
 int t2_conv_bn_backward(const t2_conv_bn_bwd_args* a, void* stream);
 
@@ -253,6 +255,7 @@
     size_t stage_bytes_a, stage_bytes_b;
 } t2_gemm_plan_info;
 int t2_gemm_plan(const t2_gemm_args* a, const t2_gemm_plan_opts* opts, t2_gemm_plan_info* out);
+int t2_conv_handoff_plan(const t2_gemm_args* a, const t2_gemm_plan_opts* opts, int* taken, t2_gemm_plan_info* out);
 int t2_colsum(const float* x, long ld, int M, int N, float* out, float* scratch, void* stream);
 int t2_mask_btc(float* x, int B, int T, int C, const int32_t* lengths, float fill, void* stream);
 
diff --git a/tacotron2_subword_amd/_lib.py b/tacotron2_subword_amd/_lib.py
--- a/tacotron2_subword_amd/_lib.py
+++ b/tacotron2_subword_amd/_lib.py
@@ -106,7 +106,8 @@
                 ("training", C.c_int), ("eps", C.c_float), ("act", C.c_int), ("drop_p", C.c_float), ("seed", C.c_uint64),
                 ("site", C.c_uint32), ("residual", C.c_void_p),
                 ("z", C.c_void_p), ("mean", C.c_void_p), ("invstd", C.c_void_p), ("var", C.c_void_p), ("y", C.c_void_p),
-                ("ws", C.c_void_p), ("ws_floats", C.c_size_t)]
+                ("ws", C.c_void_p), ("ws_floats", C.c_size_t),
+                ("x16", C.c_void_p), ("y16", C.c_void_p), ("handoff", C.c_int)]
 
 
 class ConvBnBwdArgs(C.Structure):
@@ -116,7 +117,8 @@
                 ("training", C.c_int), ("eps", C.c_float), ("act", C.c_int), ("drop_p", C.c_float), ("seed", C.c_uint64),
                 ("site", C.c_uint32), ("dy", C.c_void_p),
                 ("dw", C.c_void_p), ("dbias", C.c_void_p), ("dgamma", C.c_void_p), ("dbeta", C.c_void_p),
-                ("dx", C.c_void_p), ("dx_accumulate", C.c_int), ("ws", C.c_void_p), ("ws_floats", C.c_size_t)]
+                ("dx", C.c_void_p), ("dx_accumulate", C.c_int), ("ws", C.c_void_p), ("ws_floats", C.c_size_t),
+                ("x16", C.c_void_p), ("handoff", C.c_int)]
 
 
 _P4 = C.c_void_p * 4
@@ -159,7 +161,7 @@
 EXPORTS = ["t2_last_error", "t2_version", "t2_chain_status", "t2_chain_status_clear", "t2_debug_report_abort", "t2_debug_occupy", "t2_chain_claimed", "t2_set_precision", "t2_get_precision", "t2_gemm_counts", "t2_set_gemm_split_min_mflop", "t2_set_overlap", "t2_set_chain", "t2_get_chain", "t2_set_chain_bwd", "t2_set_gemm_staging", "t2_side_join", "t2_decoder_layout_query", "t2_decoder_forward", "t2_decoder_infer",
            "t2_decoder_bwd_layout_query", "t2_decoder_backward", "t2_prof_enable", "t2_prof_collect", "t2_adam_chunks", "t2_adam_step", "t2_adam_norm",
            "t2_conv_bn_forward", "t2_conv_bn_backward", "t2_embedding_forward", "t2_embedding_backward",
-           "t2_lstm_seq_forward", "t2_lstm_seq_backward", "t2_lstm_seq_chain_ws_floats", "t2_gemm_ex", "t2_prof_gemm", "t2_gemm_plan", "t2_colsum", "t2_mask_btc",
+           "t2_lstm_seq_forward", "t2_lstm_seq_backward", "t2_lstm_seq_chain_ws_floats", "t2_gemm_ex", "t2_prof_gemm", "t2_gemm_plan", "t2_conv_handoff_plan", "t2_colsum", "t2_mask_btc",
            "t2_finalize_bct", "t2_mask_bt", "t2_gemm", "t2_rng_keep_mask", "t2_rng_normal"]
 
 _lib = None
@@ -200,6 +202,7 @@
         L.t2_gemm_ex.argtypes = [C.POINTER(GemmArgs), C.c_void_p]
         L.t2_prof_gemm.argtypes = [C.POINTER(GemmArgs), C.c_int, C.POINTER(C.c_float), C.POINTER(C.c_float), C.c_void_p]
         L.t2_gemm_plan.argtypes = [C.POINTER(GemmArgs), C.POINTER(GemmPlanOpts), C.POINTER(GemmPlanInfo)]
+        L.t2_conv_handoff_plan.argtypes = [C.POINTER(GemmArgs), C.POINTER(GemmPlanOpts), C.POINTER(C.c_int), C.POINTER(GemmPlanInfo)]
         L.t2_colsum.argtypes = [C.c_void_p, C.c_long, C.c_int, C.c_int, C.c_void_p, C.c_void_p, C.c_void_p]
         L.t2_mask_btc.argtypes = [C.c_void_p, C.c_int, C.c_int, C.c_int, C.c_void_p, C.c_float, C.c_void_p]
         L.t2_prof_enable.argtypes = [C.c_int]
@@ -423,5 +426,12 @@
                 a_src=info.a_src, b_src=info.b_src, stage_bytes_a=info.stage_bytes_a, stage_bytes_b=info.stage_bytes_b)
 
 
+def conv_handoff_plan(args: GemmArgs, **opts) -> dict:
+    o, info, taken = GemmPlanOpts(**opts), GemmPlanInfo(), C.c_int(0)
+    check(lib().t2_conv_handoff_plan(C.byref(args), C.byref(o), C.byref(taken), C.byref(info)))
+    return dict(taken=bool(taken.value), kernel=info.kernel, name=info.name.decode(), split=bool(info.split), splitk=info.splitk,
+                kchunks=info.kchunks, a_src=info.a_src, b_src=info.b_src, stage_bytes_a=info.stage_bytes_a, stage_bytes_b=info.stage_bytes_b)
+
+
 def set_gemm_split_min_mflop(mflop: int = -1) -> None:
     check(lib().t2_set_gemm_split_min_mflop(int(mflop)))
diff --git a/tacotron2_subword_amd/blocks.py b/tacotron2_subword_amd/blocks.py
--- a/tacotron2_subword_amd/blocks.py
+++ b/tacotron2_subword_amd/blocks.py
@@ -7,6 +7,7 @@
 from . import _lib as L
 
 ACT_NONE, ACT_RELU, ACT_TANH = 0, 1, 2
+CONV_HANDOFF = True
 _WS = {}
 
 
@@ -110,7 +111,8 @@
         B, T, _ = x.shape
         n = len(cfg["acts"])
         dev = x.device
-        saved, cur = [], x
+        saved, cur, cur16 = [], x, None
+        handoff = CONV_HANDOFF and L.get_precision() == "bf16"
         for i in range(n):
             w, bias, gamma, beta = params[4 * i:4 * i + 4]
             rm, rv = cfg["buffers"][i]
@@ -122,14 +124,16 @@
             nws = Cout * Cin * K + 4 + 128 * Cout + _stage_terms() * ((M * Cin + Cout * Cin * K) // 2) + 4096
             ws = _scratch(dev, nws)
             res = x if (cfg["residual"] and i == n - 1) else None
+            y16 = torch.empty(B, T, Cout, dtype=torch.bfloat16, device=dev) if handoff and i + 1 < n else None
             a = L.ConvBnArgs(B, T, Cin, Cout, K, L.ptr(cur), L.ptr(w.detach()), L.ptr(bias.detach()), L.ptr(gamma.detach()),
                              L.ptr(beta.detach()), L.ptr(rm), L.ptr(rv), int(cfg["training"]), 1e-5, cfg["acts"][i],
                              cfg["drop_p"] if cfg["training"] else 0.0, cfg["seed"], cfg["site0"] + i, L.ptr(res),
-                             L.ptr(z), L.ptr(st[0]), L.ptr(st[1]), L.ptr(st[2]), L.ptr(y), L.ptr(ws), ws.numel())
+                             L.ptr(z), L.ptr(st[0]), L.ptr(st[1]), L.ptr(st[2]), L.ptr(y), L.ptr(ws), ws.numel(),
+                             L.ptr(cur16), L.ptr(y16), int(handoff))
             L.check(L.lib().t2_conv_bn_forward(C.byref(a), L.stream()))
-            saved.append((cur, z, st))
-            cur = y
-        ctx.cfg, ctx.saved_acts, ctx.params = cfg, saved, [p.detach() for p in params]
+            saved.append((cur, z, st, cur16))
+            cur, cur16 = y, y16
+        ctx.cfg, ctx.saved_acts, ctx.params, ctx.handoff = cfg, saved, [p.detach() for p in params], handoff
         return cur
 
     @staticmethod
@@ -142,7 +146,7 @@
         grads = [None] * (4 * n)
         for i in range(n - 1, -1, -1):
             w, bias, gamma, beta = params[4 * i:4 * i + 4]
-            xin, z, st = ctx.saved_acts[i]
+            xin, z, st, xin16 = ctx.saved_acts[i]
             B, T, Cin = xin.shape
             Cout, _, K = w.shape
             M = B * T
@@ -155,7 +159,7 @@
             a = L.ConvBnBwdArgs(B, T, Cin, Cout, K, L.ptr(xin), L.ptr(w), L.ptr(gamma), L.ptr(beta), L.ptr(z), L.ptr(st[0]), L.ptr(st[1]),
                                 int(cfg["training"]), 1e-5, cfg["acts"][i], cfg["drop_p"] if cfg["training"] else 0.0, cfg["seed"],
                                 cfg["site0"] + i, L.ptr(dy), L.ptr(dw), L.ptr(db), L.ptr(dg), L.ptr(dbt), L.ptr(dx), 0,
-                                L.ptr(ws), ws.numel())
+                                L.ptr(ws), ws.numel(), L.ptr(xin16), int(ctx.handoff and L.get_precision() == "bf16"))
             L.check(L.lib().t2_conv_bn_backward(C.byref(a), L.stream()))
             grads[4 * i:4 * i + 4] = [dw, db, dg, dbt]
             dy = dx
diff --git a/tacotron2_subword_amd/csrc/c_api.hip b/tacotron2_subword_amd/csrc/c_api.hip
--- a/tacotron2_subword_amd/csrc/c_api.hip
+++ b/tacotron2_subword_amd/csrc/c_api.hip
@@ -1390,6 +1390,7 @@
     f.wperm = a->ws; f.scratch = a->ws + align4(nw);
     const size_t used = align4(nw) + 128 * (size_t)a->Cout;
     if (a->ws_floats > used) { f.gemm_ws = a->ws + used; f.gemm_ws_bytes = (a->ws_floats - used) * sizeof(float); }
+    f.handoff = a->handoff; f.x16 = static_cast<const __bf16*>(a->x16); f.y16 = static_cast<__bf16*>(a->y16);
     return conv_bn_fwd(f, (hipStream_t)stream);
 }
 
@@ -1405,6 +1406,7 @@
     f.dx = a->dx; f.dx_accumulate = a->dx_accumulate;
     f.dz = a->ws; f.wperm = a->ws + ndz; f.scratch = a->ws + ndz + nw;
     f.gemm_ws = a->ws + ndz + nw + nsc; f.gemm_ws_bytes = (a->ws_floats - (ndz + nw + nsc)) * sizeof(float);
+    f.handoff = a->handoff; f.x16 = static_cast<const __bf16*>(a->x16);
     return conv_bn_bwd(f, (hipStream_t)stream);
 }
 
@@ -1524,9 +1526,8 @@
     T2_REQUIRE(a, "null argument");
     return gemm(desc_of(*a), (hipStream_t)stream);
 }
-int t2_gemm_plan(const t2_gemm_args* a, const t2_gemm_plan_opts* o, t2_gemm_plan_info* out) {
-    T2_REQUIRE(a && out, "null argument");
-    GemmDesc g = desc_of(*a);
+static GemmDesc desc_of(const t2_gemm_args& a, const t2_gemm_plan_opts* o) {
+    GemmDesc g = desc_of(a);
     if (o) {
         g.conv_a = o->conv_a; g.conv_b = o->conv_b; g.conv_T = o->conv_T; g.conv_C = o->conv_C; g.fp32_only = o->fp32_only;
         const __bf16* copy = reinterpret_cast<const __bf16*>(uintptr_t(256));
@@ -1534,9 +1535,27 @@
         if (o->b16) { g.B16 = copy; g.ldb16 = o->ldb16; g.b16_kmajor = o->b16_kmajor; }
         g.split16 = o->split16;
     }
+    return g;
+}
+static t2_gemm_plan_info info_of(const GemmPlan& p) {
+    return t2_gemm_plan_info{(int)p.kernel, gemm_plan_name(p), p.split, p.splitk, p.kchunks, (int)p.a.src, (int)p.b.src, p.a.bytes, p.b.bytes};
+}
+int t2_gemm_plan(const t2_gemm_args* a, const t2_gemm_plan_opts* o, t2_gemm_plan_info* out) {
+    T2_REQUIRE(a && out, "null argument");
     GemmPlan p;
-    T2_TRY(gemm_plan(g, &p));
-    *out = t2_gemm_plan_info{(int)p.kernel, gemm_plan_name(p), p.split, p.splitk, p.kchunks, (int)p.a.src, (int)p.b.src, p.a.bytes, p.b.bytes};
+    T2_TRY(gemm_plan(desc_of(*a, o), &p));
+    *out = info_of(p);
+    return 0;
+}
+int t2_conv_handoff_plan(const t2_gemm_args* a, const t2_gemm_plan_opts* o, int* taken, t2_gemm_plan_info* out) {
+    T2_REQUIRE(a && taken && out, "null argument");
+    const GemmDesc offered = desc_of(*a, o);
+    GemmDesc plain = offered;
+    plain.A16 = plain.B16 = nullptr; plain.a16_kmajor = plain.b16_kmajor = 0; plain.lda16 = plain.ldb16 = 0;
+    GemmPlan p;
+    T2_TRY(gemm_plan(plain, &p));
+    *taken = gemm_handoff(plain, offered, &p);
+    *out = info_of(p);
     return 0;
 }
 static int time_gemm(const GemmDesc& g, int reps, float* ms, hipStream_t s) {
diff --git a/tacotron2_subword_amd/csrc/common.h b/tacotron2_subword_amd/csrc/common.h
--- a/tacotron2_subword_amd/csrc/common.h
+++ b/tacotron2_subword_amd/csrc/common.h
@@ -51,6 +51,57 @@
     return v;
 }
 
+constexpr int kColLanes = 32;
+constexpr int kColThreads = 4 * kColLanes;
+
+template <int V> struct ColVec { float v[V]; };
+template <int V> __device__ __forceinline__ ColVec<V> load_cols(const float* p) {
+    static_assert(V == 1 || V == 4, "one column or one 16-byte group per lane");
+    ColVec<V> r;
+    if constexpr (V == 4) {
+        const f32x4 t = *reinterpret_cast<const f32x4*>(p);
+        r.v[0] = t.x; r.v[1] = t.y; r.v[2] = t.z; r.v[3] = t.w;
+    } else r.v[0] = *p;
+    return r;
+}
+template <int V> __device__ __forceinline__ void store_cols(float* p, const ColVec<V>& r) {
+    if constexpr (V == 4) { f32x4 t; t.x = r.v[0]; t.y = r.v[1]; t.z = r.v[2]; t.w = r.v[3]; *reinterpret_cast<f32x4*>(p) = t; }
+    else *p = r.v[0];
+}
+template <int R, class Row, class Load, class Use>
+__device__ __forceinline__ void rows_in_flight(int m, const int m1, Load load, Use use) {
+    int left = m < m1 ? (m1 - m + 3) / 4 : 0;
+    Row a[R], b[R];
+    auto request = [&](Row (&x)[R], int mm) {
+#pragma unroll
+        for (int j = 0; j < R; ++j) x[j] = load(mm + 4 * j);
+    };
+    auto consume = [&](const Row (&x)[R]) {
+#pragma unroll
+        for (int j = 0; j < R; ++j) use(m + 4 * j, x[j]);
+        m += 4 * R;
+        left -= R;
+    };
+    if (left >= R) request(a, m);
+    while (left >= R) {
+        if (left >= 2 * R) request(b, m + 4 * R);
+        consume(a);
+        if (left < R) break;
+        if (left >= 2 * R) request(a, m + 4 * R);
+        consume(b);
+    }
+    if (left > 0) {
+#pragma unroll
+        for (int j = 0; j < R; ++j) a[j] = load(m + 4 * (j < left ? j : left - 1));
+#pragma unroll
+        for (int j = 0; j < R; ++j) if (j < left) use(m + 4 * j, a[j]);
+    }
+}
+__host__ __device__ inline int col_slabs(int M) { return M >= 64 * 64 ? 64 : (M >= 64 ? M / 64 : 1); }
+inline bool cols_vectorisable(const void* p, long ld, int N) {
+    return N % 4 == 0 && ld % 4 == 0 && (reinterpret_cast<uintptr_t>(p) & 15) == 0;
+}
+
 }
 
 void t2_set_error(const char* fmt, ...);
diff --git a/tacotron2_subword_amd/csrc/conv.hip b/tacotron2_subword_amd/csrc/conv.hip
--- a/tacotron2_subword_amd/csrc/conv.hip
+++ b/tacotron2_subword_amd/csrc/conv.hip
@@ -9,18 +9,20 @@
     return (int)(g < 1 ? 1 : (g > (size_t)cap ? cap : g));
 }
 
-__global__ void permute_w_fwd_kernel(const float* __restrict__ w, float* __restrict__ wp, int Co, int Ci, int K) {
+template <class OUT>
+__global__ void permute_w_fwd_kernel(const float* __restrict__ w, OUT* __restrict__ wp, int Co, int Ci, int K) {
     const size_t n = (size_t)Co * Ci * K;
     for (size_t i = blockIdx.x * (size_t)blockDim.x + threadIdx.x; i < n; i += (size_t)gridDim.x * blockDim.x) {
         const int ci = (int)(i % Ci); const size_t r = i / Ci; const int dk = (int)(r % K), co = (int)(r / K);
-        wp[i] = w[((size_t)co * Ci + ci) * K + dk];
-    }
-}
-__global__ void permute_w_bwd_kernel(const float* __restrict__ w, float* __restrict__ wt, int Co, int Ci, int K) {
+        wp[i] = (OUT)w[((size_t)co * Ci + ci) * K + dk];
+    }
+}
+template <class OUT>
+__global__ void permute_w_bwd_kernel(const float* __restrict__ w, OUT* __restrict__ wt, int Co, int Ci, int K) {
     const size_t n = (size_t)Co * Ci * K;
     for (size_t i = blockIdx.x * (size_t)blockDim.x + threadIdx.x; i < n; i += (size_t)gridDim.x * blockDim.x) {
         const int co = (int)(i % Co); const size_t r = i / Co; const int dk = (int)(r % K), ci = (int)(r / K);
-        wt[i] = w[((size_t)co * Ci + ci) * K + (K - 1 - dk)];
+        wt[i] = (OUT)w[((size_t)co * Ci + ci) * K + (K - 1 - dk)];
     }
 }
 __global__ void unpermute_dw_kernel(const float* __restrict__ dwp, float* __restrict__ dw, int Co, int Ci, int K) {
@@ -39,42 +41,70 @@
     return act == ACT_RELU ? fmaxf(u, 0.f) : (act == ACT_TANH ? tanhf(u) : u);
 }
 
+struct BnCol { float mean, inv, ga, be; };
 template <int MODE>
-__global__ void colreduce_stage1_kernel(BnElem e, const float* __restrict__ dy, float* __restrict__ du, int M, int slabs,
-                                        float* __restrict__ scratch) {
+__device__ __forceinline__ float colreduce_term(const BnElem& e, const BnCol& k, float scale, float z, float g, uint32_t i,
+                                                float& a0, float& a1) {
+#pragma clang fp contract(off)
+    if (MODE == 0) a0 += z;
+    else if (MODE == 1) { const float d = z - k.mean; a0 = fmaf(d, d, a0); }
+    else {
+        const float xh = (z - k.mean) * k.inv, u = fmaf(xh, k.ga, k.be);
+        if (e.drop_p > 0.f) g = rng_keep(e.key, i, e.drop_p) ? g * scale : 0.f;
+        if (e.act == ACT_RELU) g = u > 0.f ? g : 0.f;
+        else if (e.act == ACT_TANH) { const float t = tanhf(u); g *= fmaf(-t, t, 1.0f); }
+        const float gx = g * xh;
+        a0 += g; a1 += gx;
+    }
+    return g;
+}
+template <int MODE, int V>
+__global__ void __launch_bounds__(kColThreads) colreduce_stage1_kernel(BnElem e, const float* __restrict__ dy, float* __restrict__ du,
+                                                                       int M, int slabs, float* __restrict__ scratch) {
+    constexpr int R = MODE == 2 ? 8 : 16;
     const int C = e.C;
-    const int c = blockIdx.x * 64 + (threadIdx.x & 63);
-    const int sub = threadIdx.x >> 6;
+    const int lane = threadIdx.x % kColLanes, sub = threadIdx.x / kColLanes;
+    const int c = (blockIdx.x * kColLanes + lane) * V;
     const int rows = (M + slabs - 1) / slabs;
     const int m0 = blockIdx.y * rows, m1 = min(M, m0 + rows);
-    __shared__ float p0[4][64], p1[4][64];
-    float a0 = 0.f, a1 = 0.f;
+    __shared__ float p0[4][kColLanes * V], p1[4][kColLanes * V];
+    float a0[V] = {}, a1[V] = {};
     if (c < C) {
-        const float mean = MODE >= 1 ? e.mean[c] : 0.f;
-        const float inv = MODE == 2 ? e.invstd[c] : 0.f, ga = MODE == 2 ? e.gamma[c] : 0.f, be = MODE == 2 ? e.beta[c] : 0.f;
+        BnCol col[V];
+#pragma unroll
+        for (int k = 0; k < V; ++k) {
+            col[k].mean = MODE >= 1 ? e.mean[c + k] : 0.f;
+            col[k].inv = MODE == 2 ? e.invstd[c + k] : 0.f; col[k].ga = MODE == 2 ? e.gamma[c + k] : 0.f; col[k].be = MODE == 2 ? e.beta[c + k] : 0.f;
+        }
         const float scale = e.drop_p > 0.f ? 1.0f / (1.0f - e.drop_p) : 1.0f;
-        for (int m = m0 + sub; m < m1; m += 4) {
-            const size_t i = (size_t)m * C + c;
-            const float z = e.z[i];
-            if (MODE == 0) a0 += z;
-            else if (MODE == 1) { const float d = z - mean; a0 += d * d; }
-            else {
-                const float xh = (z - mean) * inv, u = xh * ga + be;
-                float g = dy[i];
-                if (e.drop_p > 0.f) g = rng_keep(e.key, (uint32_t)i, e.drop_p) ? g * scale : 0.f;
-                if (e.act == ACT_RELU) g = u > 0.f ? g : 0.f;
-                else if (e.act == ACT_TANH) { const float t = tanhf(u); g *= 1.0f - t * t; }
-                du[i] = g;
-                a0 += g; a1 += g * xh;
-            }
-        }
-    }
-    p0[sub][threadIdx.x & 63] = a0; p1[sub][threadIdx.x & 63] = a1;
+        struct Row { ColVec<V> z, g; };
+        rows_in_flight<R, Row>(m0 + sub, m1,
+            [&](int m) {
+                const size_t i = (size_t)m * C + c;
+                Row r;
+                r.z = load_cols<V>(e.z + i);
+                if (MODE == 2) r.g = load_cols<V>(dy + i);
+                return r;
+            },
+            [&](int m, const Row& r) {
+                const size_t i = (size_t)m * C + c;
+                ColVec<V> g;
+#pragma unroll
+                for (int k = 0; k < V; ++k)
+                    g.v[k] = colreduce_term<MODE>(e, col[k], scale, r.z.v[k], MODE == 2 ? r.g.v[k] : 0.f, (uint32_t)(i + k), a0[k], a1[k]);
+                if (MODE == 2) store_cols<V>(du + i, g);
+            });
+    }
+#pragma unroll
+    for (int k = 0; k < V; ++k) { p0[sub][lane * V + k] = a0[k]; p1[sub][lane * V + k] = a1[k]; }
     __syncthreads();
     if (sub == 0 && c < C) {
-        const int l = threadIdx.x;
-        scratch[(size_t)blockIdx.y * C + c] = p0[0][l] + p0[1][l] + p0[2][l] + p0[3][l];
-        if (MODE == 2) scratch[(size_t)(slabs + blockIdx.y) * C + c] = p1[0][l] + p1[1][l] + p1[2][l] + p1[3][l];
+#pragma unroll
+        for (int k = 0; k < V; ++k) {
+            const int l = lane * V + k;
+            scratch[(size_t)blockIdx.y * C + c + k] = p0[0][l] + p0[1][l] + p0[2][l] + p0[3][l];
+            if (MODE == 2) scratch[(size_t)(slabs + blockIdx.y) * C + c + k] = p1[0][l] + p1[1][l] + p1[2][l] + p1[3][l];
+        }
     }
 }
 __global__ void colreduce_stage2_kernel(const float* __restrict__ scratch, int C, int slabs, int M, int mode, float eps,
@@ -101,28 +131,69 @@
     else { out0[c] = s0; out1[c] = s1; }
 }
 
-__global__ void bn_apply_kernel(BnElem e, const float* __restrict__ residual, float* __restrict__ y, size_t n) {
+typedef __bf16 bf16x4 __attribute__((ext_vector_type(4)));
+template <int V> __device__ __forceinline__ void store_cols16(__bf16* p, const ColVec<V>& r) {
+    if constexpr (V == 4) { bf16x4 t; t[0] = (__bf16)r.v[0]; t[1] = (__bf16)r.v[1]; t[2] = (__bf16)r.v[2]; t[3] = (__bf16)r.v[3]; *reinterpret_cast<bf16x4*>(p) = t; }
+    else *p = (__bf16)r.v[0];
+}
+__device__ __forceinline__ float bn_apply_term(const BnElem& e, float scale, float z, float mean, float inv, float ga, float be, uint32_t i) {
+#pragma clang fp contract(off)
+    float v = act_fwd(fmaf((z - mean) * inv, ga, be), e.act);
+    if (e.drop_p > 0.f) v = rng_keep(e.key, i, e.drop_p) ? v * scale : 0.f;
+    return v;
+}
+template <int V>
+__global__ void bn_apply_kernel(BnElem e, const float* __restrict__ residual, float* __restrict__ y, __bf16* __restrict__ y16, size_t n) {
     const float scale = e.drop_p > 0.f ? 1.0f / (1.0f - e.drop_p) : 1.0f;
-    for (size_t i = blockIdx.x * (size_t)blockDim.x + threadIdx.x; i < n; i += (size_t)gridDim.x * blockDim.x) {
-        const int c = (int)(i % e.C);
-        float v = act_fwd((e.z[i] - e.mean[c]) * e.invstd[c] * e.gamma[c] + e.beta[c], e.act);
-        if (e.drop_p > 0.f) v = rng_keep(e.key, (uint32_t)i, e.drop_p) ? v * scale : 0.f;
-        if (residual) v += residual[i];
-        y[i] = v;
-    }
-}
-__global__ void bn_bwd_dz_kernel(BnElem e, const float* __restrict__ du, const float* __restrict__ sdu, const float* __restrict__ sduxh,
-                                 int M, int training, float* __restrict__ dz, size_t n) {
+    const size_t stride = (size_t)gridDim.x * blockDim.x * V;
+    size_t i = (blockIdx.x * (size_t)blockDim.x + threadIdx.x) * V;
+    int c = (int)(i % e.C);
+    const int cstep = (int)(stride % e.C);
+    for (; i < n; i += stride) {
+        const ColVec<V> z = load_cols<V>(e.z + i), mean = load_cols<V>(e.mean + c), inv = load_cols<V>(e.invstd + c),
+                        ga = load_cols<V>(e.gamma + c), be = load_cols<V>(e.beta + c);
+        ColVec<V> v;
+#pragma unroll
+        for (int k = 0; k < V; ++k) v.v[k] = bn_apply_term(e, scale, z.v[k], mean.v[k], inv.v[k], ga.v[k], be.v[k], (uint32_t)(i + k));
+        if (residual) {
+            const ColVec<V> r = load_cols<V>(residual + i);
+#pragma unroll
+            for (int k = 0; k < V; ++k) v.v[k] += r.v[k];
+        }
+        store_cols<V>(y + i, v);
+        if (y16) store_cols16<V>(y16 + i, v);
+        c += cstep;
+        if (c >= e.C) c -= e.C;
+    }
+}
+__device__ __forceinline__ float bn_bwd_dz_term(float g, float z, float mean, float inv, float ga, float sdu, float sduxh, float invM, int training) {
+#pragma clang fp contract(off)
+    if (training) {
+        const float xh = (z - mean) * inv;
+        g = fmaf(-invM, sdu, g);
+        g = fmaf(-invM, xh * sduxh, g);
+    }
+    return g * ga * inv;
+}
+template <int V>
+__global__ void bn_bwd_dz_kernel(BnElem e, const float* du, const float* __restrict__ sdu, const float* __restrict__ sduxh,
+                                 int M, int training, float* dz, __bf16* __restrict__ dz16, size_t n) {
     const float invM = 1.0f / (float)M;
-    for (size_t i = blockIdx.x * (size_t)blockDim.x + threadIdx.x; i < n; i += (size_t)gridDim.x * blockDim.x) {
-        const int c = (int)(i % e.C);
-        const float inv = e.invstd[c], ga = e.gamma[c];
-        float g = du[i];
-        if (training) {
-            const float xh = (e.z[i] - e.mean[c]) * inv;
-            g = g - sdu[c] * invM - xh * sduxh[c] * invM;
-        }
-        dz[i] = g * ga * inv;
+    const size_t stride = (size_t)gridDim.x * blockDim.x * V;
+    size_t i = (blockIdx.x * (size_t)blockDim.x + threadIdx.x) * V;
+    int c = (int)(i % e.C);
+    const int cstep = (int)(stride % e.C);
+    for (; i < n; i += stride) {
+        const ColVec<V> g = load_cols<V>(du + i), inv = load_cols<V>(e.invstd + c), ga = load_cols<V>(e.gamma + c);
+        ColVec<V> z{}, mean{}, s0{}, s1{};
+        if (training) { z = load_cols<V>(e.z + i); mean = load_cols<V>(e.mean + c); s0 = load_cols<V>(sdu + c); s1 = load_cols<V>(sduxh + c); }
+        ColVec<V> o;
+#pragma unroll
+        for (int k = 0; k < V; ++k) o.v[k] = bn_bwd_dz_term(g.v[k], z.v[k], mean.v[k], inv.v[k], ga.v[k], s0.v[k], s1.v[k], invM, training);
+        store_cols<V>(dz + i, o);
+        if (dz16) store_cols16<V>(dz16 + i, o);
+        c += cstep;
+        if (c >= e.C) c -= e.C;
     }
 }
 __global__ void bn_running_kernel(const float* mean, const float* var, int C, int M, float momentum, float* rm, float* rv) {
@@ -182,10 +253,22 @@
     }
 }
 
+bool bn_vectorisable(const BnElem& e, const void* p, const void* q) {
+    for (const void* a : {(const void*)e.z, (const void*)e.mean, (const void*)e.invstd, (const void*)e.gamma, (const void*)e.beta, p, q})
+        if (!cols_vectorisable(a, e.C, e.C)) return false;
+    return true;
+}
+inline bool aligned8(const void* p) { return (reinterpret_cast<uintptr_t>(p) & 7) == 0; }
+inline size_t round256(size_t n) { return (n + 255) & ~(size_t)255; }
+inline bool same_route(const GemmPlan& p, const GemmPlan& q) { return p.kernel == q.kernel && p.split == q.split && p.splitk == q.splitk && p.kchunks == q.kchunks; }
+
 template <int MODE>
 int colreduce(const BnElem& e, const float* dy, float* du, int M, float eps, float* out0, float* out1, float* scratch, hipStream_t s) {
-    const int slabs = M >= 64 * 64 ? 64 : (M >= 64 ? M / 64 : 1);
-    hipLaunchKernelGGL(colreduce_stage1_kernel<MODE>, dim3((e.C + 63) / 64, slabs), dim3(256), 0, s, e, dy, du, M, slabs, scratch);
+    const int slabs = col_slabs(M);
+    if (cols_vectorisable(e.z, e.C, e.C) && cols_vectorisable(dy, e.C, e.C) && cols_vectorisable(du, e.C, e.C))
+        hipLaunchKernelGGL((colreduce_stage1_kernel<MODE, 4>), dim3((e.C + 4 * kColLanes - 1) / (4 * kColLanes), slabs), dim3(kColThreads), 0, s, e, dy, du, M, slabs, scratch);
+    else
+        hipLaunchKernelGGL((colreduce_stage1_kernel<MODE, 1>), dim3((e.C + kColLanes - 1) / kColLanes, slabs), dim3(kColThreads), 0, s, e, dy, du, M, slabs, scratch);
     T2_LAUNCH_CHECK();
     hipLaunchKernelGGL(colreduce_stage2_kernel, dim3((e.C + 255) / 256), dim3(256), 0, s, scratch, e.C, slabs, M, MODE, eps, out0, out1);
     T2_LAUNCH_CHECK();
@@ -199,13 +282,20 @@
     T2_REQUIRE(a.Cin % 4 == 0 && a.K % 2 == 1, "conv_bn_fwd: Cin=%d must be a multiple of 4 and the kernel size odd (%d)", a.Cin, a.K);
     T2_REQUIRE((size_t)M * a.Cout < (1ull << 32), "conv_bn_fwd: B*T*Cout too large for 32-bit RNG indices");
     const size_t nw = (size_t)a.Cout * a.Cin * a.K;
-    hipLaunchKernelGGL(permute_w_fwd_kernel, dim3(grid_for(nw)), dim3(256), 0, s, a.w, a.wperm, a.Cout, a.Cin, a.K);
-    T2_LAUNCH_CHECK();
     GemmDesc g = gemm_desc();
     g.A = a.x; g.conv_a = 1; g.conv_T = a.T; g.conv_C = a.Cin; g.conv_pad = (a.K - 1) / 2;
     g.B = a.wperm; g.sbn = (long)a.K * a.Cin; g.sbk = 1;
     g.C = a.z; g.ldc = a.Cout; g.M = M; g.N = a.Cout; g.K = a.K * a.Cin; g.bias1 = a.bias;
     g.ws = a.gemm_ws; g.ws_bytes = a.gemm_ws_bytes;
+    GemmDesc g16 = g;
+    g16.A16 = a.x16; g16.lda16 = a.Cin;
+    g16.B16 = reinterpret_cast<const __bf16*>(a.wperm); g16.ldb16 = (long)a.K * a.Cin;
+    if (a.handoff && gemm_handoff(g, g16)) {
+        g = g16;
+        hipLaunchKernelGGL(permute_w_fwd_kernel<__bf16>, dim3(grid_for(nw)), dim3(256), 0, s, a.w, reinterpret_cast<__bf16*>(a.wperm), a.Cout, a.Cin, a.K);
+    } else
+        hipLaunchKernelGGL(permute_w_fwd_kernel<float>, dim3(grid_for(nw)), dim3(256), 0, s, a.w, a.wperm, a.Cout, a.Cin, a.K);
+    T2_LAUNCH_CHECK();
     T2_TRY_RC(gemm(g, s));
     BnElem e{a.z, a.mean, a.invstd, a.gamma, a.beta, a.Cout, a.act, a.drop_p, rng_key(a.seed, a.site)};
     if (a.training) {
@@ -221,7 +311,10 @@
         T2_LAUNCH_CHECK();
     }
     const size_t n = (size_t)M * a.Cout;
-    hipLaunchKernelGGL(bn_apply_kernel, dim3(grid_for(n)), dim3(256), 0, s, e, a.residual, a.y, n);
+    if (bn_vectorisable(e, a.residual, a.y) && aligned8(a.y16))
+        hipLaunchKernelGGL(bn_apply_kernel<4>, dim3(grid_for(n / 4)), dim3(256), 0, s, e, a.residual, a.y, a.y16, n);
+    else
+        hipLaunchKernelGGL(bn_apply_kernel<1>, dim3(grid_for(n)), dim3(256), 0, s, e, a.residual, a.y, a.y16, n);
     T2_LAUNCH_CHECK();
     return 0;
 }
@@ -230,29 +323,55 @@
     const int M = a.B * a.T;
     const size_t n = (size_t)M * a.Cout;
     BnElem e{a.z, a.mean, a.invstd, a.gamma, a.beta, a.Cout, a.act, a.drop_p, rng_key(a.seed, a.site)};
-    T2_TRY_RC(colreduce<2>(e, a.dy, a.dz, M, a.eps, a.dbeta, a.dgamma, a.scratch, s));
-    hipLaunchKernelGGL(bn_bwd_dz_kernel, dim3(grid_for(n)), dim3(256), 0, s, e, a.dz, a.dbeta, a.dgamma, M, a.training, a.dz, n);
-    T2_LAUNCH_CHECK();
-    T2_TRY_RC(colsum(a.dz, a.Cout, M, a.Cout, a.dbias, nullptr, a.scratch, s));
     GemmDesc g = gemm_desc();
     g.A = a.dz; g.sam = 1; g.sak = a.Cout;
     g.B = a.x; g.conv_b = 1; g.conv_T = a.T; g.conv_C = a.Cin; g.conv_pad = (a.K - 1) / 2;
     g.C = a.wperm; g.ldc = (long)a.K * a.Cin; g.M = a.Cout; g.N = a.K * a.Cin; g.K = M;
     g.ws = a.gemm_ws; g.ws_bytes = a.gemm_ws_bytes;
+    GemmDesc h = gemm_desc();
+    h.A = a.dz; h.conv_a = 1; h.conv_T = a.T; h.conv_C = a.Cout; h.conv_pad = (a.K - 1) / 2;
+    h.B = a.wperm; h.sbn = (long)a.K * a.Cout; h.sbk = 1;
+    h.C = a.dx; h.ldc = a.Cin; h.M = M; h.N = a.Cin; h.K = a.K * a.Cout;
+    h.beta = a.dx_accumulate ? 1.f : 0.f;
+    h.ws = a.gemm_ws; h.ws_bytes = a.gemm_ws_bytes;
+    if (a.dx) T2_REQUIRE(a.Cout % 4 == 0, "conv_bn_bwd: Cout=%d must be a multiple of 4", a.Cout);
+    __bf16* dz16 = nullptr;
+    bool w16 = false;
+    const size_t dz16_bytes = round256(n * sizeof(__bf16));
+    if (a.handoff && a.gemm_ws && (reinterpret_cast<uintptr_t>(a.gemm_ws) & 15) == 0 && a.gemm_ws_bytes >= dz16_bytes) {
+        float* behind = a.gemm_ws + dz16_bytes / sizeof(float);
+        GemmDesc g16 = g, h16 = h;
+        g16.ws = h16.ws = behind; g16.ws_bytes = h16.ws_bytes = a.gemm_ws_bytes - dz16_bytes;
+        g16.A16 = h16.A16 = reinterpret_cast<const __bf16*>(a.gemm_ws);
+        g16.lda16 = a.Cout; g16.a16_kmajor = 1; h16.lda16 = a.Cout;
+        g16.B16 = a.x16; g16.ldb16 = a.Cin; g16.b16_kmajor = 1;
+        h16.B16 = reinterpret_cast<const __bf16*>(a.wperm); h16.ldb16 = (long)a.K * a.Cout;
+        const bool tw = gemm_handoff(g, g16);
+        bool tx = a.dx && gemm_handoff(h, h16);
+        if (tx && !tw) {
+            GemmDesc gb = g;
+            gb.ws = behind; gb.ws_bytes = g16.ws_bytes;
+            if (same_route(plan_gemm(g), plan_gemm(gb))) g = gb; else tx = false;
+        }
+        if (tw) g = g16;
+        if (tx) { h = h16; w16 = true; }
+        if (tw || tx) dz16 = reinterpret_cast<__bf16*>(a.gemm_ws);
+    }
+    T2_TRY_RC(colreduce<2>(e, a.dy, a.dz, M, a.eps, a.dbeta, a.dgamma, a.scratch, s));
+    if (bn_vectorisable(e, a.dz, a.dbeta) && cols_vectorisable(a.dgamma, e.C, e.C))
+        hipLaunchKernelGGL(bn_bwd_dz_kernel<4>, dim3(grid_for(n / 4)), dim3(256), 0, s, e, a.dz, a.dbeta, a.dgamma, M, a.training, a.dz, dz16, n);
+    else
+        hipLaunchKernelGGL(bn_bwd_dz_kernel<1>, dim3(grid_for(n)), dim3(256), 0, s, e, a.dz, a.dbeta, a.dgamma, M, a.training, a.dz, dz16, n);
+    T2_LAUNCH_CHECK();
+    T2_TRY_RC(colsum(a.dz, a.Cout, M, a.Cout, a.dbias, nullptr, a.scratch, s));
     T2_TRY_RC(gemm(g, s));
     const size_t nw = (size_t)a.Cout * a.Cin * a.K;
     hipLaunchKernelGGL(unpermute_dw_kernel, dim3(grid_for(nw)), dim3(256), 0, s, a.wperm, a.dw, a.Cout, a.Cin, a.K);
     T2_LAUNCH_CHECK();
     if (a.dx) {
-        T2_REQUIRE(a.Cout % 4 == 0, "conv_bn_bwd: Cout=%d must be a multiple of 4", a.Cout);
-        hipLaunchKernelGGL(permute_w_bwd_kernel, dim3(grid_for(nw)), dim3(256), 0, s, a.w, a.wperm, a.Cout, a.Cin, a.K);
+        if (w16) hipLaunchKernelGGL(permute_w_bwd_kernel<__bf16>, dim3(grid_for(nw)), dim3(256), 0, s, a.w, reinterpret_cast<__bf16*>(a.wperm), a.Cout, a.Cin, a.K);
+        else hipLaunchKernelGGL(permute_w_bwd_kernel<float>, dim3(grid_for(nw)), dim3(256), 0, s, a.w, a.wperm, a.Cout, a.Cin, a.K);
         T2_LAUNCH_CHECK();
-        GemmDesc h = gemm_desc();
-        h.A = a.dz; h.conv_a = 1; h.conv_T = a.T; h.conv_C = a.Cout; h.conv_pad = (a.K - 1) / 2;
-        h.B = a.wperm; h.sbn = (long)a.K * a.Cout; h.sbk = 1;
-        h.C = a.dx; h.ldc = a.Cin; h.M = M; h.N = a.Cin; h.K = a.K * a.Cout;
-        h.beta = a.dx_accumulate ? 1.f : 0.f;
-        h.ws = a.gemm_ws; h.ws_bytes = a.gemm_ws_bytes;
         T2_TRY_RC(gemm(h, s));
     }
     return 0;
diff --git a/tacotron2_subword_amd/csrc/elementwise.hip b/tacotron2_subword_amd/csrc/elementwise.hip
--- a/tacotron2_subword_amd/csrc/elementwise.hip
+++ b/tacotron2_subword_amd/csrc/elementwise.hip
@@ -87,17 +87,31 @@
         dz[i] = y[i] > 0.f ? dy[i] * scale : 0.f;
 }
 
-__global__ void colsum_stage1_kernel(const float* __restrict__ X, long ld, int M, int N, int slabs, float* scratch) {
-    const int n = blockIdx.x * 64 + (threadIdx.x & 63);
-    const int sub = threadIdx.x >> 6;
+template <int V>
+__global__ void __launch_bounds__(kColThreads) colsum_stage1_kernel(const float* __restrict__ X, long ld, int M, int N, int slabs,
+                                                                    float* __restrict__ scratch) {
+    const int lane = threadIdx.x % kColLanes, sub = threadIdx.x / kColLanes;
+    const int n = (blockIdx.x * kColLanes + lane) * V;
     const int rows = (M + slabs - 1) / slabs;
     const int m0 = blockIdx.y * rows, m1 = min(M, m0 + rows);
-    __shared__ float part[4][64];
-    float acc = 0.f;
-    if (n < N) for (int m = m0 + sub; m < m1; m += 4) acc += X[(long)m * ld + n];
-    part[sub][threadIdx.x & 63] = acc;
+    __shared__ float part[4][kColLanes * V];
+    ColVec<V> acc{};
+    if (n < N)
+        rows_in_flight<16, ColVec<V>>(m0 + sub, m1, [&](int m) { return load_cols<V>(X + (long)m * ld + n); },
+                                      [&](int, const ColVec<V>& x) {
+#pragma unroll
+                                          for (int k = 0; k < V; ++k) acc.v[k] += x.v[k];
+                                      });
+#pragma unroll
+    for (int k = 0; k < V; ++k) part[sub][lane * V + k] = acc.v[k];
     __syncthreads();
-    if (sub == 0 && n < N) scratch[(long)blockIdx.y * N + n] = part[0][threadIdx.x] + part[1][threadIdx.x] + part[2][threadIdx.x] + part[3][threadIdx.x];
+    if (sub == 0 && n < N) {
+#pragma unroll
+        for (int k = 0; k < V; ++k) {
+            const int l = lane * V + k;
+            scratch[(long)blockIdx.y * N + n + k] = part[0][l] + part[1][l] + part[2][l] + part[3][l];
+        }
+    }
 }
 __device__ __forceinline__ float ordered_sum16(const float* __restrict__ p, int count, long stride) {
     float acc = 0.f;
@@ -146,8 +160,11 @@
     return 0;
 }
 int colsum(const float* X, long ld, int M, int N, float* out, float* out2, float* scratch, hipStream_t s) {
-    const int slabs = M >= 64 * 64 ? 64 : (M >= 64 ? M / 64 : 1);
-    hipLaunchKernelGGL(colsum_stage1_kernel, dim3((N + 63) / 64, slabs), dim3(256), 0, s, X, ld, M, N, slabs, scratch);
+    const int slabs = col_slabs(M);
+    if (cols_vectorisable(X, ld, N))
+        hipLaunchKernelGGL(colsum_stage1_kernel<4>, dim3((N + 4 * kColLanes - 1) / (4 * kColLanes), slabs), dim3(kColThreads), 0, s, X, ld, M, N, slabs, scratch);
+    else
+        hipLaunchKernelGGL(colsum_stage1_kernel<1>, dim3((N + kColLanes - 1) / kColLanes, slabs), dim3(kColThreads), 0, s, X, ld, M, N, slabs, scratch);
     T2_LAUNCH_CHECK();
     hipLaunchKernelGGL(colsum_stage2_kernel, dim3((N + 255) / 256), dim3(256), 0, s, scratch, N, slabs, out, out2);
     T2_LAUNCH_CHECK();
diff --git a/tacotron2_subword_amd/csrc/gemm.hip b/tacotron2_subword_amd/csrc/gemm.hip
--- a/tacotron2_subword_amd/csrc/gemm.hip
+++ b/tacotron2_subword_amd/csrc/gemm.hip
@@ -1231,7 +1231,9 @@
     const bool km = shape256 && !akc && !bkc && !d.conv_a && (!d.conv_b || d.conv_C % 256 == 0) && (long)d.K * kmul * ld_km * 2 < (1l << 31);
     a_caller = a_caller && (d.a16_kmajor != 0) == km;
     b_caller = b_caller && (d.b16_kmajor != 0) == km;
-    const bool conv_ok = !conv_any || (d.conv_a && d.conv_C % 64 == 0 && !a_caller && !b_caller) || (d.conv_b && km && (!want_split || d.K % d.conv_T == 0));
+    a_caller = a_caller && (!d.conv_a || d.lda16 == d.conv_C);
+    const bool conv_ok = !conv_any || (d.conv_a && d.conv_C % 64 == 0 && (!want_split || (!a_caller && !b_caller))) ||
+                         (d.conv_b && km && (!want_split || d.K % d.conv_T == 0));
     bool staged = false;
     size_t ws_bytes = d.ws_bytes;
     if ((use_bf16 || want_split) && g_stage && conv_ok && d.batch == 1 && d.M % 128 == 0 && d.N % 128 == 0 && d.K % 64 == 0) {
@@ -1289,6 +1291,18 @@
     return 0;
 }
 
+bool gemm_handoff(const GemmDesc& plain, const GemmDesc& offered, GemmPlan* plan) {
+    const GemmPlan p0 = plan_gemm(plain);
+    if (plan) *plan = p0;
+    if (g_precision != 1 || !gemm_reads_bf16_copies(p0.kernel) || !(offered.A16 || offered.B16)) return false;
+    if ((offered.A16 && p0.a.src != GemmSrc::staged) || (offered.B16 && p0.b.src != GemmSrc::staged)) return false;
+    const GemmPlan p1 = plan_gemm(offered);
+    if (p1.kernel != p0.kernel || p1.split != p0.split || p1.splitk != p0.splitk || p1.kchunks != p0.kchunks) return false;
+    if ((offered.A16 && p1.a.src != GemmSrc::caller) || (offered.B16 && p1.b.src != GemmSrc::caller)) return false;
+    if (plan) *plan = p1;
+    return true;
+}
+
 int gemm(const GemmDesc& d, hipStream_t s) {
     GemmPlan p;
     T2_TRY_RC(gemm_plan(d, &p));
diff --git a/tacotron2_subword_amd/csrc/kernels.h b/tacotron2_subword_amd/csrc/kernels.h
--- a/tacotron2_subword_amd/csrc/kernels.h
+++ b/tacotron2_subword_amd/csrc/kernels.h
@@ -57,6 +57,7 @@
 };
 GemmPlan plan_gemm(const GemmDesc& d);
 int gemm_plan(const GemmDesc& d, GemmPlan* out);
+bool gemm_handoff(const GemmDesc& plain, const GemmDesc& offered, GemmPlan* plan = nullptr);
 const char* gemm_plan_name(const GemmPlan& p);
 int stage_planned(const float* src, const GemmOperandPlan& o, bool split, __bf16* dst, hipStream_t s);
 int stage_bf16(const float* src, bool kc, long ld, __bf16* dst, int rows, int K, hipStream_t s);
@@ -328,6 +329,8 @@
     float* y;
     float* wperm; float* scratch;
     float* gemm_ws; size_t gemm_ws_bytes;
+    int handoff;
+    const __bf16* x16; __bf16* y16;
 };
 int conv_bn_fwd(const ConvBnFwd& a, hipStream_t s);
 struct ConvBnBwd {
@@ -340,6 +343,8 @@
     float* dw; float* dbias; float* dgamma; float* dbeta;
     float* dx; int dx_accumulate;
     float* wperm; float* scratch; float* gemm_ws; size_t gemm_ws_bytes;
+    int handoff;
+    const __bf16* x16;
 };
 int conv_bn_bwd(const ConvBnBwd& a, hipStream_t s);
 int embedding_fwd(const long* ids, const float* table, float* out, int rows, int D, hipStream_t s);
```
